# wildltr/ptranking

Hardware: AMD Instinct MI355X
Metric: queries/sec fwd+bwd LambdaRank, MSLR-WEB30K-shaped list_len=128 (higher is better)
Workload: dtype f32

## Files before the change

### include/ptranking_amd.h

```cpp
#ifndef PTRANKING_AMD_H
#define PTRANKING_AMD_H

#include <stddef.h>
#include <stdint.h>

#ifdef __cplusplus
extern "C" {
#endif

#define PTR_ABI_VERSION 8
#define PTR_MAX_LIST_LEN 4096
#define PTR_MAX_CUTOFFS 32
#define PTR_MAX_SUBTOPICS 32
#define PTR_MLP_ACT_LD 112

#define PTR_ERR_INVALID_ARG 1001
#define PTR_ERR_UNSUPPORTED 1002

#define PTR_LAMBDALOSS_NDCG_LOSS1 0
#define PTR_LAMBDALOSS_NDCG_LOSS2 1
#define PTR_LAMBDALOSS_NDCG_LOSS2PP 2

int ptr_abi_version(void);
const char *ptr_last_error(void);

int ptr_ranknet_fwd_bwd(const float *preds, const float *labels, const int32_t *lens, int B, int L, float sigma,
                        float *loss_out, float *loss_q, float *grad, void *stream);

int ptr_lambdarank_fwd_bwd(const float *preds, const float *labels, const int32_t *lens, int B, int L, float sigma,
                           float *loss_out, float *loss_q, float *grad, void *stream);

int ptr_lambdaloss_fwd_bwd(const float *preds, const float *labels, const int32_t *lens, int B, int L, int k,
                           float sigma, float mu, int loss_type, int presort, float *loss_out, float *loss_q,
                           float *grad, void *stream);

int ptr_softrank_fwd_bwd(const float *preds, const float *labels, const int32_t *lens, int B, int L, float delta, int top_k,
                         float *loss_out, float *loss_q, float *grad, void *stream);

int ptr_approxndcg_fwd_bwd(const float *preds, const float *labels, const int32_t *lens, int B, int L, float alpha,
                           int presort, int couple_batch, float grad_scale_override, float *loss_out, float *dcg_q,
                           float *inv_idcg_q, float *scale_out, float *grad, void *stream);

int ptr_listnet_fwd_bwd(const float *preds, const float *labels, const int32_t *lens, int B, int L, float *loss_out,
                        float *loss_q, float *grad, void *stream);

int ptr_stlistnet_fwd_bwd(const float *preds, const float *labels, const float *unif, const int32_t *lens, int B, int L,
                          float temperature, float *loss_out, float *loss_q, float *grad, void *stream);
int ptr_rankmse_fwd_bwd(const float *preds, const float *labels, const int32_t *lens, int B, int L, float *loss_out,
                        float *loss_q, float *grad, void *stream);
int ptr_rankcosine_fwd_bwd(const float *preds, const float *labels, const int32_t *lens, int B, int L, float *loss_out,
                           float *loss_q, float *grad, void *stream);

int ptr_listmle_fwd_bwd(const float *preds, const int64_t *perm, const int32_t *lens, int B, int L, float *loss_out,
                        float *loss_q, float *grad, void *stream);

int ptr_mdprank_fwd_bwd(const float *preds, const float *labels, const int64_t *perm, const int32_t *lens, int B, int L, int top_k,
                        float gamma, float *loss_out, float *loss_q, float *grad, void *stream);

#define PTR_WASS_COST_P1 0
#define PTR_WASS_COST_P2 1
#define PTR_WASS_COST_EG 2
#define PTR_WASS_COST_DG 3
#define PTR_WASS_COST_DDG 4

int ptr_wassrank_fwd_bwd(const float *preds, const float *labels, const int32_t *lens, int B, int L, int cost_type,
                         float gain_base, float non_rele_gap, float var_penalty, float lam, int sh_itr,
                         int scale_by_max_label, float *loss_out, float *loss_q, float *grad, void *stream);

#define PTR_ADCG_TOPK_SUBTOPICS 0
#define PTR_ADCG_TOPK_DOCUMENTS 1
int ptr_alphadcg_fwd_bwd(const float *preds, const float *rele, const int32_t *lens, const int32_t *ntopics, int B, int T, int L, float rt,
                         float alpha, int top_k, int top_k_axis, float *loss_out, float *loss_q, float *grad, void *stream);
int ptr_div_metrics_at_ks(const float *preds, const float *rele, const int32_t *lens, const int32_t *ntopics, int B, int T, int L,
                          const int32_t *ks, int nk, float alpha, float max_label, float *andcg, float *err_ia, float *nerr_ia,
                          int32_t *valid, void *stream);

#define PTR_DIVPROB_ANDCG 0
#define PTR_DIVPROB_ERRIA 1
#define PTR_DIVPROB_PAIRCLS 2
#define PTR_DIVPROB_LAMBDAPAIRCLS 3
int ptr_divprob_fwd_bwd(const float *mus, const float *vars, const float *rele, const int32_t *lens, const int32_t *ntopics, int B, int T, int L,
                        int objective, float beta, int top_k, int top_k_axis, float max_label, int norm, float *loss_out, float *loss_q,
                        float *grad_mu, float *grad_var, void *stream);
int ptr_divprob_expected_ranks(const float *mus, const float *vars, const int32_t *lens, int B, int L, float *ranks, void *stream);

#define PTR_NDEVAL_DEPTH 20
int ptr_ndeval_measures(const float *preds, const float *rele, const int32_t *lens, const int32_t *ntopics, int B, int T, int L,
                        const int32_t *ks, int nk, double alpha, double beta, int depth_m, double *per_k, double *per_q,
                        int32_t *actual_subtopics, int32_t *ideal_order, void *stream);

#define PTR_TREE_PAIRS_ALL 0
#define PTR_TREE_PAIRS_NOTIES 1
#define PTR_TREE_PAIRS_NO00 2
#define PTR_TREE_PAIRS_00 3
#define PTR_TREE_W_NONE 0
#define PTR_TREE_W_DELTA_NDCG 1
#define PTR_TREE_W_DELTA_GAIN 2
#define PTR_TREE_HESS_REFERENCE 0
#define PTR_TREE_HESS_SUM 1
#define PTR_TREE_HESS_CONSTANT 2
#define PTR_TREE_GAIN_POWER 0
#define PTR_TREE_GAIN_LABEL 1
int ptr_tree_pair_grad_hess(const float *preds, const float *labels, const int64_t *offsets, int B, const int32_t *queries, int nq, int max_len,
                            int pair_type, int weighting, float epsilon, int hessian, float *grad, float *hess, void *stream);
int ptr_tree_listnet_grad_hess(const float *preds, const float *labels, const int64_t *offsets, int B, const int32_t *queries, int nq, int max_len,
                               int gain_type, int hessian, float *grad, float *hess, void *stream);

#define PTR_SMOOTH_P 0
#define PTR_SMOOTH_AP 1
#define PTR_SMOOTH_NERR 2
#define PTR_SMOOTH_NDCG 3
int ptr_smoothmetric_fwd_bwd(const float *preds, const float *labels, const int32_t *lens, int B, int L, int metric, int opt_ideal, int top_k,
                             float alpha, float max_label, float *loss_out, float *loss_q, float *valid_q, float *ranks, float *max_label_ws,
                             float *grad, void *stream);

int ptr_gaussmetric_fwd_bwd(const float *mus, const float *vars, const float *labels, const int32_t *lens, int B, int L, int metric,
                            int opt_ideal, int top_k, float const_std, float max_label, float *loss_out, float *loss_q, float *valid_q,
                            float *ranks, int32_t *pos, float *max_label_ws, float *grad_mu, float *grad_var, void *stream);

#define PTR_PL_DIST_PL 0
#define PTR_PL_DIST_STPL 1
int ptr_pl_uniforms(int B, int L, int S, uint64_t seed, int64_t q0, float *unif, void *stream);
int ptr_pl_sample(const float *preds, const int32_t *lens, int B, int L, int S, float temperature, int distribution, uint64_t seed, int64_t q0,
                  const float *unif, int64_t *perm, float *action, void *stream);
int ptr_mdprank_sample_fwd_bwd(const float *preds, const float *labels, const int32_t *lens, int B, int L, int S, int top_k, float gamma,
                               float temperature, int distribution, uint64_t seed, int64_t q0, const float *unif, float *loss_out,
                               float *loss_q, float *grad, int64_t *perm_out, void *stream);

#define PTR_IRGAN_MAX_SAMPLES 64
#define PTR_IRGAN_MAX_DRAWS_PER_POS 64
#define PTR_IRGAN_POINT_D 0
#define PTR_IRGAN_PAIR_D 1
#define PTR_IRGAN_PAIR_G 2
#define PTR_IRGAN_SEL_POINT_D 0
#define PTR_IRGAN_SEL_PAIR_D_SVM 1
#define PTR_IRGAN_SEL_PAIR_D_LOG 2
#define PTR_IRGAN_SEL_PAIR_G_SVM 3
#define PTR_IRGAN_SEL_PAIR_G_LOG 4
int ptr_irgan_sample(const float *preds, const int32_t *lens, const int32_t *num_pos, int B, int L, int S, int mode, float temperature,
                     uint64_t seed, int64_t q0, const float *unif, int64_t *pos_idx, int64_t *neg_idx, int32_t *nsel, void *stream);
int ptr_irgan_point_gen_fwd_bwd(const float *g_preds, const float *d_preds, const int32_t *lens, const int32_t *num_pos, int B, int L,
                                float temperature, float lambda, int draws_per_pos, uint64_t seed, int64_t q0, const float *unif,
                                float *loss_out, float *loss_q, float *valid_q, float *grad, int32_t *counts, void *stream);
int ptr_irgan_sel_fwd_bwd(const float *x, const float *d_sel, const int64_t *neg_idx, const int32_t *nsel, const int32_t *lens, int B, int L,
                          int S, int mode, float temperature, float *loss_out, float *loss_q, float *valid_q, float *grad, void *stream);

#define PTR_IRFGAN_POINT_D 0
#define PTR_IRFGAN_PAIR_D 1
#define PTR_IRFGAN_POINT_G 2
#define PTR_IRFGAN_PAIR_G 3
#define PTR_FDIV_TVAR 0
#define PTR_FDIV_KL 1
#define PTR_FDIV_RKL 2
#define PTR_FDIV_PC 3
#define PTR_FDIV_NC 4
#define PTR_FDIV_SH 5
#define PTR_FDIV_JS 6
#define PTR_FDIV_GAN 7
int ptr_irfgan_point_sample(const float *preds, const int32_t *lens, const int32_t *num_pos, int B, int L, int S, uint64_t seed, int64_t q0,
                            const float *unif, int64_t *pos_idx, int64_t *neg_idx, int32_t *nsel, void *stream);
int ptr_irfgan_pair_sample(const float *preds, const float *labels, const int32_t *lens, const int32_t *num_pos, int B, int L, int S,
                           uint64_t seed, int64_t q0, const float *unif_draw, const float *unif_bern, int64_t *true_head, int64_t *true_tail,
                           int64_t *fake_head, int64_t *fake_tail, int32_t *nsel, int32_t *bern_count, void *stream);
int ptr_irfgan_fwd_bwd(const float *x, const float *d_fake, const int64_t *idx_a, const int64_t *idx_b, const int32_t *nsel, const int32_t *lens,
                       int B, int L, int S, int mode, int f_div, float *loss_out, float *loss_q, float *valid_q, float *grad, void *stream);

int ptr_shuffle_ties_order(const float *labels, const int32_t *lens, int B, int L, uint64_t seed, int64_t *perm,
                           void *stream);

int ptr_sort_desc(const float *preds, const int32_t *lens, int B, int L, float *vals, int64_t *idx, void *stream);

#define PTR_LABEL_MULTILABEL 0
#define PTR_LABEL_PERMUTATION 1
int ptr_metrics_at_ks(const float *preds, const float *labels, const int32_t *lens, int B, int L, const int32_t *ks,
                      int nk, int presort, int label_type, float max_label, float *max_label_ws, float *ndcg, float *nerr,
                      float *ap, float *prec, void *stream);

int ptr_sum_f32(const float *x, int n, float scale, float *out, void *stream);

size_t ptr_mlp_num_params(int F, int NL);
size_t ptr_mlp_backward_ws_floats(int F, int NL);
size_t ptr_mlp_backward_dz_floats(int R, int F, int NL);
size_t ptr_mlp_acts_floats(int R, int NL);
int ptr_mlp_forward(const float *X, const float *params, int R, int F, int NL, int train, float p_drop, uint64_t seed,
                    float *preds, float *acts, void *stream);
int ptr_mlp_backward(const float *X, const float *params, const float *acts, const float *dpreds, int R, int F, int NL,
                     float p_drop, uint64_t seed, float *dz, float *ws, float *grad, void *stream);
#define PTR_OPT_ADAM 1
#define PTR_OPT_ADAGRAD 2
#define PTR_OPT_RMSPROP 3
int ptr_mlp_backward_step(const float *X, float *params, const float *acts, const float *dpreds, int R, int F, int NL, float p_drop,
                          uint64_t seed, float *dz, float *ws, float *grad, int opt_kind, float lr, float hyper1, float hyper2, float eps,
                          float weight_decay, int step, float *state1, float *state2, const float *loss_q, int nq, float *loss_out,
                          void *stream);
int ptr_opt_step_loss(float *params, const float *grad, int64_t n, int opt_kind, float lr, float hyper1, float hyper2, float eps,
                      float weight_decay, int step, float *state1, float *state2, const float *loss_q, int nq, float *loss_out, void *stream);
int ptr_adam_step(float *param, const float *grad, float *exp_avg, float *exp_avg_sq, int64_t n, float lr, float beta1,
                  float beta2, float eps, float weight_decay, int step, void *stream);
int ptr_adagrad_step(float *param, const float *grad, float *state_sum, int64_t n, float lr, float lr_decay, float eps,
                     float weight_decay, int step, void *stream);
int ptr_rmsprop_step(float *param, const float *grad, float *square_avg, int64_t n, float lr, float alpha, float eps,
                     float weight_decay, void *stream);
size_t ptr_mlp_x6_ws_bytes(int F, int NL);
int ptr_mlp_forward_x6(const float *X, const float *params, int R, int F, int NL, int train, float p_drop, uint64_t seed,
                       float *preds, float *acts, void *wimg, void *stream);
#define PTR_LOSS_RANKNET 1
#define PTR_LOSS_LAMBDARANK 2
#define PTR_LOSS_LAMBDALOSS 3
#define PTR_LOSS_LISTNET 4
typedef struct ptr_train_step_desc {
    int32_t struct_bytes;
    int32_t loss_kind;
    int32_t B, L, F, NL;
    int32_t opt_kind, step;
    int32_t loss_i[4];
    float loss_f[4];
    float p_drop, lr, hyper1, hyper2, eps, weight_decay;
    uint64_t seed;
    const float *X, *labels;
    const int32_t *lens;
    float *params, *grad, *state1, *state2;
    float *preds, *acts, *loss_q, *dpreds, *dz, *ws;
    void *wimg;
    float *loss_out;
    void *events[4];
    int32_t wimg_current;
    int32_t reserved;
} ptr_train_step_desc;
int ptr_train_step(const ptr_train_step_desc *d, void *stream);
int ptr_mlp_dropout_mask(int R, int n_feat, int site, float p_drop, uint64_t seed, float *out, void *stream);

#define PTR_LINEAR_NONE 0
#define PTR_LINEAR_RELU 1
#define PTR_LINEAR_RELU_DROPOUT 2
#define PTR_LINEAR_GATE 3
int ptr_linear_forward(const float *X, int ldx, const float *W, const float *bias, int R, int K, int N, int act, float p_drop,
                       uint64_t seed, int site, float *Y, int ldy, void *stream);
int ptr_linear_backward_input(const float *dY, int ldy, const float *W, int R, int K, int N, const float *gate, int ldg, float p_drop,
                              float *dX, int ldx, void *stream);
size_t ptr_linear_backward_weight_ws_floats(int R, int K, int N);
int ptr_linear_backward_weight(const float *X, int ldx, const float *dY, int ldy, int R, int K, int N, float *ws, float *dW, float *db,
                               void *stream);
int ptr_dropout_apply(const float *x, int ldx, int R, int C, float p_drop, uint64_t seed, int site, float *out, int ldo, void *stream);
int ptr_relu_gate(const float *dy, const float *y, int64_t n, float *out, void *stream);

#define PTR_AF_NONE 0
#define PTR_AF_RELU 1
#define PTR_AF_LEAKY 2
#define PTR_AF_ELU 3
#define PTR_AF_SELU 4
#define PTR_AF_GELU 5
#define PTR_AF_SIGMOID 6
#define PTR_AF_TANH 7
size_t ptr_bn_ws_floats(int R, int N, int group_rows);
int ptr_bn_stats(const float *z, int ld, int R, int N, int group_rows, const int32_t *lens, int rows_per_query, float eps, float *ws,
                 float *mean, float *rstd, void *stream);
int ptr_bnact_forward(const float *z, int ld, int R, int N, int group_rows, const int32_t *lens, int rows_per_query, const float *mean,
                      const float *rstd, const float *gamma, const float *beta, int af, float p_drop, uint64_t seed, int site, float *out,
                      void *stream);
int ptr_bnact_backward(const float *z, const float *da, int ld, int R, int N, int group_rows, const int32_t *lens, int rows_per_query,
                       const float *mean, const float *rstd, const float *gamma, const float *beta, int af, float p_drop, uint64_t seed,
                       int site, float *ws, float *dz, float *dgamma, float *dbeta, void *stream);

size_t ptr_bn_slot_floats(int N);
int ptr_bn_stats_partial(const float *z, int ld, int R, int N, int group_rows, const int32_t *lens, int rows_per_query, float *ws,
                         float *slot, void *stream);
int ptr_bn_stats_combine(const float *slots, int W, int slot_stride, int N, float eps, float *mean, float *rstd, float *total_count,
                         void *stream);
int ptr_bnact_backward_sums(const float *z, const float *da, int ld, int R, int N, int group_rows, const int32_t *lens, int rows_per_query,
                            const float *mean, const float *rstd, const float *gamma, const float *beta, int af, float p_drop,
                            uint64_t seed, int site, float *ws, float *sums, void *stream);
int ptr_bnact_backward_apply(const float *z, const float *da, int ld, int R, int N, int group_rows, const int32_t *lens, int rows_per_query,
                             const float *mean, const float *rstd, const float *gamma, const float *beta, int af, float p_drop,
                             uint64_t seed, int site, const float *sums, int W, const float *total_count, float *ws, float *dz,
                             void *stream);

#define PTR_MHSA_MAX_HEAD_DIM 352
int ptr_mhsa_forward(const float *Q, const float *K, const float *V, int ld_qkv, const int32_t *lens, int B, int L, int F,
                     int n_heads, float p_drop, uint64_t seed, int site, float *O, float *lse, void *stream);
int ptr_mhsa_backward(const float *Q, const float *K, const float *V, int ld_qkv, const float *O, const float *dO, const float *lse,
                      const int32_t *lens, int B, int L, int F, int n_heads, float p_drop, uint64_t seed, int site, float *dvec,
                      float *dQ, float *dK, float *dV, float *ds_ws, void *stream);
int ptr_mhsa_dropout_mask(int B, int L, int n_heads, float p_drop, uint64_t seed, int site, float *out, void *stream);
int ptr_layernorm_forward(const float *X, const float *a2, const float *b2, int64_t R, int F, float eps, float *Y, float *stats,
                          void *stream);
size_t ptr_layernorm_backward_ws_floats(int F);
int ptr_layernorm_backward(const float *X, const float *a2, const float *dY, const float *stats, int64_t R, int F, float *ws,
                           float *dX, float *da2, float *db2, void *stream);

int ptr_launch_form(const char *entry, const int64_t *args, int nargs, int32_t *form, int nform);

#define PTR_GBDT_MAX_BIN 256
int ptr_gbdt_bin(const float *X, int64_t n, int F, const float *edges, const int32_t *nbins, int max_bin, int stride, uint8_t *bins,
                 void *stream);
int ptr_gbdt_quantize(const float *g, const float *h, int64_t n, int32_t *qg, int32_t *qh, int32_t *expo, int32_t *flag, uint32_t *state,
                      void *stream);
int ptr_gbdt_histogram(const uint8_t *bins, int stride, int64_t n, const int32_t *qg, const int32_t *qh, const int32_t *rows, int64_t m,
                       int F, int max_bin, int64_t *hist, void *stream);
int ptr_gbdt_hist_sub(const int64_t *parent, const int64_t *child, int F, int max_bin, int64_t *out, void *stream);
int ptr_gbdt_best_split(const int64_t *hist, int nleaf, int F, int max_bin, const int32_t *nbins, const int32_t *expo, double lambda_l2,
                        int64_t min_data_in_leaf, double min_sum_hessian_in_leaf, double min_gain_to_split, int64_t *ws, int64_t *rec,
                        void *stream);
size_t ptr_gbdt_partition_ws_ints(int64_t m);
int ptr_gbdt_partition(const uint8_t *bins, int stride, int64_t n, int F, const int32_t *rows, int64_t m, int feature, int bin,
                       int32_t *out, int32_t *left_count, int32_t *ws, void *stream);
int ptr_gbdt_add_leaf_values(float *scores, int64_t n, const int32_t *rows, const int32_t *offsets, const float *values, int nleaves,
                             int64_t total, void *stream);
int ptr_gbdt_predict(const float *X, int64_t n, int F, const int32_t *feature, const float *threshold, const int32_t *left,
                     const int32_t *right, const float *value, const int32_t *tree_offsets, int ntrees, float *out, void *stream);

int ptr_gbdt_histogram_segments(const uint8_t *bins, int stride, int64_t n, const int32_t *qg, const int32_t *qh, const int32_t *rows,
                                int64_t nrows, const int32_t *segs, int K, const int32_t *items, int n_direct, int n_lds, int F, int max_bin,
                                int64_t *pool, int nslots, void *stream);
int ptr_gbdt_hist_sub_segments(int64_t *pool, int nslots, int F, int max_bin, const int32_t *trips, int K, void *stream);
int ptr_gbdt_best_split_slots(const int64_t *pool, int nslots, const int32_t *slots, int K, int F, int max_bin, const int32_t *nbins,
                              const int32_t *expo, double lambda_l2, int64_t min_data_in_leaf, double min_sum_hessian_in_leaf,
                              double min_gain_to_split, int64_t *ws, int64_t *rec, void *stream);
size_t ptr_gbdt_partition_segments_ws_ints(int64_t nblocks);
int ptr_gbdt_partition_segments(const uint8_t *bins, int stride, int64_t n, int F, const int32_t *rows, int64_t nrows, const int32_t *segs, int K,
                                const int32_t *blocks, int nblocks, int32_t *out, int32_t *left_counts, int32_t *ws, int64_t ws_ints,
                                void *stream);

int ptr_letor_scan(const char *path, int one_indexed, int64_t *n_docs, int32_t *n_features, int64_t *n_queries);
int ptr_letor_load(const char *path, int one_indexed, float missing, int64_t n_docs, int32_t n_features, int64_t n_queries,
                   void *X, int x_is_f64, float *y, int64_t *qids, int64_t *qoff);

#ifdef __cplusplus
}
#endif
#endif
```

### ptranking_amd/_lib.py

```python
import ctypes as C
import os

import torch

_PKG = os.path.dirname(os.path.abspath(__file__))
LIB_PATH = os.environ.get("PTR_LIB") or os.path.join(_PKG, "libptranking_amd.so")

ABI_VERSION = 8
MAX_LIST_LEN = 4096
MAX_CUTOFFS = 32
MAX_SUBTOPICS = 32

_vp, _i, _f, _u64 = C.c_void_p, C.c_int, C.c_float, C.c_uint64

SIGNATURES = {
    "ptr_abi_version": [],
    "ptr_last_error": [],
    "ptr_ranknet_fwd_bwd": [_vp, _vp, _vp, _i, _i, _f, _vp, _vp, _vp, _vp],
    "ptr_lambdarank_fwd_bwd": [_vp, _vp, _vp, _i, _i, _f, _vp, _vp, _vp, _vp],
    "ptr_lambdaloss_fwd_bwd": [_vp, _vp, _vp, _i, _i, _i, _f, _f, _i, _i, _vp, _vp, _vp, _vp],
    "ptr_approxndcg_fwd_bwd": [_vp, _vp, _vp, _i, _i, _f, _i, _i, _f, _vp, _vp, _vp, _vp, _vp, _vp],
    "ptr_softrank_fwd_bwd": [_vp, _vp, _vp, _i, _i, _f, _i, _vp, _vp, _vp, _vp],
    "ptr_listnet_fwd_bwd": [_vp, _vp, _vp, _i, _i, _vp, _vp, _vp, _vp],
    "ptr_mdprank_fwd_bwd": [_vp, _vp, _vp, _vp, _i, _i, _i, _f, _vp, _vp, _vp, _vp],
    "ptr_listmle_fwd_bwd": [_vp, _vp, _vp, _i, _i, _vp, _vp, _vp, _vp],
    "ptr_stlistnet_fwd_bwd": [_vp, _vp, _vp, _vp, _i, _i, _f, _vp, _vp, _vp, _vp],
    "ptr_rankmse_fwd_bwd": [_vp, _vp, _vp, _i, _i, _vp, _vp, _vp, _vp],
    "ptr_rankcosine_fwd_bwd": [_vp, _vp, _vp, _i, _i, _vp, _vp, _vp, _vp],
    "ptr_wassrank_fwd_bwd": [_vp, _vp, _vp, _i, _i, _i, _f, _f, _f, _f, _i, _i, _vp, _vp, _vp, _vp],
    "ptr_alphadcg_fwd_bwd": [_vp, _vp, _vp, _vp, _i, _i, _i, _f, _f, _i, _i, _vp, _vp, _vp, _vp],
    "ptr_div_metrics_at_ks": [_vp, _vp, _vp, _vp, _i, _i, _i, C.POINTER(C.c_int32), _i, _f, _f, _vp, _vp, _vp, _vp, _vp],
    "ptr_divprob_fwd_bwd": [_vp, _vp, _vp, _vp, _vp, _i, _i, _i, _i, _f, _i, _i, _f, _i, _vp, _vp, _vp, _vp, _vp],
    "ptr_divprob_expected_ranks": [_vp, _vp, _vp, _i, _i, _vp, _vp],
    "ptr_ndeval_measures": [_vp, _vp, _vp, _vp, _i, _i, _i, C.POINTER(C.c_int32), _i, C.c_double, C.c_double, _i, _vp, _vp, _vp, _vp, _vp],
    "ptr_tree_pair_grad_hess": [_vp, _vp, _vp, _i, _vp, _i, _i, _i, _i, _f, _i, _vp, _vp, _vp],
    "ptr_tree_listnet_grad_hess": [_vp, _vp, _vp, _i, _vp, _i, _i, _i, _i, _vp, _vp, _vp],
    "ptr_smoothmetric_fwd_bwd": [_vp, _vp, _vp, _i, _i, _i, _i, _i, _f, _f, _vp, _vp, _vp, _vp, _vp, _vp, _vp],
    "ptr_gaussmetric_fwd_bwd": [_vp, _vp, _vp, _vp, _i, _i, _i, _i, _i, _f, _f, _vp, _vp, _vp, _vp, _vp, _vp, _vp, _vp, _vp],
    "ptr_pl_uniforms": [_i, _i, _i, _u64, C.c_int64, _vp, _vp],
    "ptr_pl_sample": [_vp, _vp, _i, _i, _i, _f, _i, _u64, C.c_int64, _vp, _vp, _vp, _vp],
    "ptr_mdprank_sample_fwd_bwd": [_vp, _vp, _vp, _i, _i, _i, _i, _f, _f, _i, _u64, C.c_int64, _vp, _vp, _vp, _vp, _vp, _vp],
    "ptr_irgan_sample": [_vp, _vp, _vp, _i, _i, _i, _i, _f, _u64, C.c_int64, _vp, _vp, _vp, _vp, _vp],
    "ptr_irgan_point_gen_fwd_bwd": [_vp, _vp, _vp, _vp, _i, _i, _f, _f, _i, _u64, C.c_int64, _vp, _vp, _vp, _vp, _vp, _vp, _vp],
    "ptr_irgan_sel_fwd_bwd": [_vp, _vp, _vp, _vp, _vp, _i, _i, _i, _i, _f, _vp, _vp, _vp, _vp, _vp],
    "ptr_irfgan_point_sample": [_vp, _vp, _vp, _i, _i, _i, _u64, C.c_int64, _vp, _vp, _vp, _vp, _vp],
    "ptr_irfgan_pair_sample": [_vp, _vp, _vp, _vp, _i, _i, _i, _u64, C.c_int64, _vp, _vp, _vp, _vp, _vp, _vp, _vp, _vp, _vp],
    "ptr_irfgan_fwd_bwd": [_vp, _vp, _vp, _vp, _vp, _vp, _i, _i, _i, _i, _i, _vp, _vp, _vp, _vp, _vp],
    "ptr_shuffle_ties_order": [_vp, _vp, _i, _i, _u64, _vp, _vp],
    "ptr_sort_desc": [_vp, _vp, _i, _i, _vp, _vp, _vp],
    "ptr_metrics_at_ks": [_vp, _vp, _vp, _i, _i, C.POINTER(C.c_int32), _i, _i, _i, _f, _vp, _vp, _vp, _vp, _vp, _vp],
    "ptr_sum_f32": [_vp, _i, _f, _vp, _vp],
    "ptr_mlp_num_params": [_i, _i],
    "ptr_mlp_backward_ws_floats": [_i, _i],
    "ptr_mlp_backward_dz_floats": [_i, _i, _i],
    "ptr_mlp_acts_floats": [_i, _i],
    "ptr_mlp_forward": [_vp, _vp, _i, _i, _i, _i, _f, _u64, _vp, _vp, _vp],
    "ptr_mlp_backward": [_vp, _vp, _vp, _vp, _i, _i, _i, _f, _u64, _vp, _vp, _vp, _vp],
    "ptr_mlp_backward_step": [_vp, _vp, _vp, _vp, _i, _i, _i, _f, _u64, _vp, _vp, _vp, _i, _f, _f, _f, _f, _f, _i, _vp, _vp, _vp, _i, _vp, _vp],
    "ptr_opt_step_loss": [_vp, _vp, C.c_int64, _i, _f, _f, _f, _f, _f, _i, _vp, _vp, _vp, _i, _vp, _vp],
    "ptr_train_step": [_vp, _vp],
    "ptr_mlp_x6_ws_bytes": [_i, _i],
    "ptr_mlp_forward_x6": [_vp, _vp, _i, _i, _i, _i, _f, _u64, _vp, _vp, _vp, _vp],
    "ptr_adam_step": [_vp, _vp, _vp, _vp, C.c_int64, _f, _f, _f, _f, _f, _i, _vp],
    "ptr_adagrad_step": [_vp, _vp, _vp, C.c_int64, _f, _f, _f, _f, _i, _vp],
    "ptr_rmsprop_step": [_vp, _vp, _vp, C.c_int64, _f, _f, _f, _f, _vp],
    "ptr_mlp_dropout_mask": [_i, _i, _i, _f, _u64, _vp, _vp],
    "ptr_linear_forward": [_vp, _i, _vp, _vp, _i, _i, _i, _i, _f, _u64, _i, _vp, _i, _vp],
    "ptr_linear_backward_input": [_vp, _i, _vp, _i, _i, _i, _vp, _i, _f, _vp, _i, _vp],
    "ptr_linear_backward_weight_ws_floats": [_i, _i, _i],
    "ptr_linear_backward_weight": [_vp, _i, _vp, _i, _i, _i, _i, _vp, _vp, _vp, _vp],
    "ptr_bn_ws_floats": [_i, _i, _i],
    "ptr_bn_stats": [_vp, _i, _i, _i, _i, _vp, _i, _f, _vp, _vp, _vp, _vp],
    "ptr_bnact_forward": [_vp, _i, _i, _i, _i, _vp, _i, _vp, _vp, _vp, _vp, _i, _f, _u64, _i, _vp, _vp],
    "ptr_bnact_backward": [_vp, _vp, _i, _i, _i, _i, _vp, _i, _vp, _vp, _vp, _vp, _i, _f, _u64, _i, _vp, _vp, _vp, _vp, _vp],
    "ptr_bn_slot_floats": [_i],
    "ptr_bn_stats_partial": [_vp, _i, _i, _i, _i, _vp, _i, _vp, _vp, _vp],
    "ptr_bn_stats_combine": [_vp, _i, _i, _i, _f, _vp, _vp, _vp, _vp],
    "ptr_bnact_backward_sums": [_vp, _vp, _i, _i, _i, _i, _vp, _i, _vp, _vp, _vp, _vp, _i, _f, _u64, _i, _vp, _vp, _vp],
    "ptr_bnact_backward_apply": [_vp, _vp, _i, _i, _i, _i, _vp, _i, _vp, _vp, _vp, _vp, _i, _f, _u64, _i, _vp, _i, _vp, _vp, _vp, _vp],
    "ptr_dropout_apply": [_vp, _i, _i, _i, _f, _u64, _i, _vp, _i, _vp],
    "ptr_relu_gate": [_vp, _vp, C.c_int64, _vp, _vp],
    "ptr_mhsa_forward": [_vp, _vp, _vp, _i, _vp, _i, _i, _i, _i, _f, _u64, _i, _vp, _vp, _vp],
    "ptr_mhsa_backward": [_vp, _vp, _vp, _i, _vp, _vp, _vp, _vp, _i, _i, _i, _i, _f, _u64, _i, _vp, _vp, _vp, _vp, _vp, _vp],
    "ptr_mhsa_dropout_mask": [_i, _i, _i, _f, _u64, _i, _vp, _vp],
    "ptr_layernorm_forward": [_vp, _vp, _vp, C.c_int64, _i, _f, _vp, _vp, _vp],
    "ptr_layernorm_backward_ws_floats": [_i],
    "ptr_layernorm_backward": [_vp, _vp, _vp, _vp, C.c_int64, _i, _vp, _vp, _vp, _vp, _vp],
    "ptr_launch_form": [C.c_char_p, C.POINTER(C.c_int64), _i, C.POINTER(C.c_int32), _i],
    "ptr_gbdt_bin": [_vp, C.c_int64, _i, _vp, _vp, _i, _i, _vp, _vp],
    "ptr_gbdt_quantize": [_vp, _vp, C.c_int64, _vp, _vp, _vp, _vp, _vp, _vp],
    "ptr_gbdt_histogram": [_vp, _i, C.c_int64, _vp, _vp, _vp, C.c_int64, _i, _i, _vp, _vp],
    "ptr_gbdt_hist_sub": [_vp, _vp, _i, _i, _vp, _vp],
    "ptr_gbdt_best_split": [_vp, _i, _i, _i, _vp, _vp, C.c_double, C.c_int64, C.c_double, C.c_double, _vp, _vp, _vp],
    "ptr_gbdt_partition_ws_ints": [C.c_int64],
    "ptr_gbdt_partition": [_vp, _i, C.c_int64, _i, _vp, C.c_int64, _i, _i, _vp, _vp, _vp, _vp],
    "ptr_gbdt_add_leaf_values": [_vp, C.c_int64, _vp, _vp, _vp, _i, C.c_int64, _vp],
    "ptr_gbdt_predict": [_vp, C.c_int64, _i, _vp, _vp, _vp, _vp, _vp, _vp, _i, _vp, _vp],
    "ptr_gbdt_histogram_segments": [_vp, _i, C.c_int64, _vp, _vp, _vp, C.c_int64, _vp, _i, _vp, _i, _i, _i, _i, _vp, _i, _vp],
    "ptr_gbdt_hist_sub_segments": [_vp, _i, _i, _i, _vp, _i, _vp],
    "ptr_gbdt_best_split_slots": [_vp, _i, _vp, _i, _i, _i, _vp, _vp, C.c_double, C.c_int64, C.c_double, C.c_double, _vp, _vp, _vp],
    "ptr_gbdt_partition_segments_ws_ints": [C.c_int64],
    "ptr_gbdt_partition_segments": [_vp, _i, C.c_int64, _i, _vp, C.c_int64, _vp, _i, _vp, _i, _vp, _vp, _vp, C.c_int64, _vp],
    "ptr_letor_scan":[C.c_char_p, _i, _vp, _vp, _vp],
    "ptr_letor_load": [C.c_char_p, _i, _f, C.c_int64, C.c_int32, C.c_int64, _vp, _i, _vp, _vp, _vp],
}
_RESTYPES = {"ptr_last_error": C.c_char_p, "ptr_mlp_num_params": C.c_size_t, "ptr_mlp_backward_ws_floats": C.c_size_t,
             "ptr_mlp_backward_dz_floats": C.c_size_t, "ptr_mlp_acts_floats": C.c_size_t, "ptr_mlp_x6_ws_bytes": C.c_size_t, "ptr_linear_backward_weight_ws_floats": C.c_size_t, "ptr_bn_ws_floats": C.c_size_t,
             "ptr_bn_slot_floats": C.c_size_t, "ptr_gbdt_partition_ws_ints": C.c_size_t,
             "ptr_gbdt_partition_segments_ws_ints": C.c_size_t,
             "ptr_layernorm_backward_ws_floats": C.c_size_t}
OPTIONAL = set()

_lib = None


class Loss:

    def __init__(self, entry, kind, params=()):
        self.entry, self.kind, self.params = entry, kind, tuple(params)

    def c_args(self, **values):
        return [C.c_float(float(values[n])) if t is _f else int(values[n]) for n, t in self.params]

    def desc_arrays(self, **values):
        return (tuple(int(values[n]) for n, t in self.params if t is _i), tuple(C.c_float(float(values[n])).value for n, t in self.params if t is _f))


LOSSES = {
    "ranknet": Loss("ptr_ranknet_fwd_bwd", 1, [("sigma", _f)]),
    "lambdarank": Loss("ptr_lambdarank_fwd_bwd", 2, [("sigma", _f)]),
    "lambdaloss": Loss("ptr_lambdaloss_fwd_bwd", 3, [("k", _i), ("sigma", _f), ("mu", _f), ("loss_type", _i), ("presort", _i)]),
    "listnet": Loss("ptr_listnet_fwd_bwd", 4),
}


class TrainStepDesc(C.Structure):
    _fields_ = [("struct_bytes", C.c_int32), ("loss_kind", C.c_int32),
                ("B", C.c_int32), ("L", C.c_int32), ("F", C.c_int32), ("NL", C.c_int32),
                ("opt_kind", C.c_int32), ("step", C.c_int32),
                ("loss_i", C.c_int32 * 4), ("loss_f", C.c_float * 4),
                ("p_drop", C.c_float), ("lr", C.c_float), ("hyper1", C.c_float), ("hyper2", C.c_float), ("eps", C.c_float), ("weight_decay", C.c_float),
                ("seed", C.c_uint64),
                ("X", C.c_void_p), ("labels", C.c_void_p), ("lens", C.c_void_p),
                ("params", C.c_void_p), ("grad", C.c_void_p), ("state1", C.c_void_p), ("state2", C.c_void_p),
                ("preds", C.c_void_p), ("acts", C.c_void_p), ("loss_q", C.c_void_p), ("dpreds", C.c_void_p), ("dz", C.c_void_p), ("ws", C.c_void_p),
                ("wimg", C.c_void_p), ("loss_out", C.c_void_p), ("events", C.c_void_p * 4), ("wimg_current", C.c_int32), ("reserved", C.c_int32)]


class NativeLibraryError(RuntimeError):
    pass


def load():
    global _lib
    if _lib is not None:
        return _lib
    if not os.path.exists(LIB_PATH):
        raise NativeLibraryError(
            f"{LIB_PATH} is missing: build the HIP extension first (python -m ptranking_amd.build, or "
            f"__graft_entry__.build()).  ptranking_amd has no CPU / eager fallback by design.")
    lib = C.CDLL(LIB_PATH, mode=C.RTLD_GLOBAL)
    for name, argtypes in SIGNATURES.items():
        try:
            fn = getattr(lib, name)
        except AttributeError:
            if name in OPTIONAL:
                continue
            raise NativeLibraryError(f"{LIB_PATH} does not export {name}; rebuild it")
        fn.argtypes = argtypes
        fn.restype = _RESTYPES.get(name, C.c_int)
    v = lib.ptr_abi_version()
    if v != ABI_VERSION:
        raise NativeLibraryError(f"ABI version mismatch: library {v}, binding {ABI_VERSION}")
    _lib = lib
    return lib


def has(name):
    return hasattr(load(), name)


TIMING = None


def query(name, *args):
    return getattr(load(), name)(*args)


def call(name, *args):
    lib = load()
    if TIMING is not None:
        ev0, ev1 = torch.cuda.Event(enable_timing=True), torch.cuda.Event(enable_timing=True)
        ev0.record()
        rc = getattr(lib, name)(*args)
        ev1.record()
        TIMING.setdefault(name, []).append((ev0, ev1))
    else:
        rc = getattr(lib, name)(*args)
    if rc != 0:
        msg = lib.ptr_last_error()
        raise RuntimeError(f"{name} failed (code {rc}): {msg.decode() if msg else ''}")


def ptr(t):
    return None if t is None else C.c_void_p(t.data_ptr())


def current_stream(device):
    return C.c_void_p(torch.cuda.current_stream(device).cuda_stream)
```

### ptranking_amd/csrc/optim.hip

```cpp
#include "ptr_mlp.h"
#include "ptr_optim.h"

namespace ptr {

constexpr int kRedElems = 128;
inline unsigned reduce_grid(size_t n, bool loss_block) { return (unsigned)((n + kRedElems - 1) / kRedElems) + (loss_block ? 1u : 0u); }
__global__ void __launch_bounds__(1024)
reduce_partials_kernel(const float *__restrict__ ws, int nblk, int nblk_tail, size_t tail_begin, size_t stride, size_t n,
                       float *__restrict__ grad, OptStep o) {
    __shared__ float part[16][kRedElems];
    const int lane = threadIdx.x & 63, w = threadIdx.x >> 6;
    if (o.loss_out && blockIdx.x == gridDim.x - 1) {
        const float tot = block1024_sum(o.loss_q, o.nq, &part[0][0]);
        if (threadIdx.x == 0) o.loss_out[0] = tot;
        return;
    }
    const size_t ia = (size_t)blockIdx.x * kRedElems + lane, ib = ia + 64;
    const size_t ica = ia < n ? ia : n - 1, icb = ib < n ? ib : n - 1;
    const int nba = ica >= tail_begin ? nblk_tail : nblk, nbb = icb >= tail_begin ? nblk_tail : nblk;
    const int nbc = nba < nbb ? nba : nbb;
    float a0 = 0.f, a1 = 0.f, a2 = 0.f, a3 = 0.f, b0 = 0.f, b1 = 0.f, b2 = 0.f, b3 = 0.f;
    int b = w;
    for (; b + 48 < nbc; b += 64) {
        a0 += ws[(size_t)b * stride + ica];
        a1 += ws[(size_t)(b + 16) * stride + ica];
        a2 += ws[(size_t)(b + 32) * stride + ica];
        a3 += ws[(size_t)(b + 48) * stride + ica];
        b0 += ws[(size_t)b * stride + icb];
        b1 += ws[(size_t)(b + 16) * stride + icb];
        b2 += ws[(size_t)(b + 32) * stride + icb];
        b3 += ws[(size_t)(b + 48) * stride + icb];
    }
    int ba = b, bb = b;
    for (; ba + 48 < nba; ba += 64) {
        a0 += ws[(size_t)ba * stride + ica];
        a1 += ws[(size_t)(ba + 16) * stride + ica];
        a2 += ws[(size_t)(ba + 32) * stride + ica];
        a3 += ws[(size_t)(ba + 48) * stride + ica];
    }
    for (; bb + 48 < nbb; bb += 64) {
        b0 += ws[(size_t)bb * stride + icb];
        b1 += ws[(size_t)(bb + 16) * stride + icb];
        b2 += ws[(size_t)(bb + 32) * stride + icb];
        b3 += ws[(size_t)(bb + 48) * stride + icb];
    }
    for (; ba < nba; ba += 16) a0 += ws[(size_t)ba * stride + ica];
    for (; bb < nbb; bb += 16) b0 += ws[(size_t)bb * stride + icb];
    part[w][lane] = (a0 + a1) + (a2 + a3);
    part[w][64 + lane] = (b0 + b1) + (b2 + b3);
    __syncthreads();
    const int col = 64 * w + lane;
    const size_t i = (size_t)blockIdx.x * kRedElems + col;
    if (w < 2 && i < n) {
        float s = part[0][col];
#pragma unroll
        for (int k = 1; k < 16; ++k) s += part[k][col];
        if (grad) grad[i] = s;
        if (o.kind) {
            const float pn = opt_update(o, i, s);
            if (o.wimg) x6_img_put(o.wimg, o.F, o.NL, i, pn);
        }
    }
}

int launch_reduce_partials(const float *ws, int nblk, int nblk_tail, size_t tail_begin, size_t stride, size_t n, float *grad, const OptStep &o,
                           hipStream_t st, const char *who) {
    hipLaunchKernelGGL(reduce_partials_kernel, dim3(reduce_grid(n, o.loss_out != nullptr)), dim3(1024), 0, st, ws, nblk, nblk_tail, tail_begin,
                       stride, n, grad, o);
    return check_hip(hipGetLastError(), who);
}

__global__ void __launch_bounds__(256)
opt_step_kernel(const float *__restrict__ grad, size_t n, OptStep o) {
    const size_t i = (size_t)blockIdx.x * 256 + threadIdx.x;
    if (i < n) opt_update(o, i, grad[i]);
}

static int opt_step_alone(const char *who, int opt_kind, float *param, const float *grad, float *state1, float *state2, int64_t n, float lr, float hyper1,
                          float hyper2, float eps, float weight_decay, int step, void *stream) {
    if (n < 0 || (n > 0 && (!param || !grad))) { set_error("%s: bad arguments", who); return PTR_ERR_INVALID_ARG; }
    OptStep o;
    if (int rc = make_opt_step(o, who, opt_kind, lr, hyper1, hyper2, eps, weight_decay, step, param, state1, state2, n > 0, nullptr, 0, nullptr)) return rc;
    if (n == 0) return 0;
    hipLaunchKernelGGL(opt_step_kernel, dim3((unsigned)((n + 255) / 256)), dim3(256), 0, as_stream(stream), grad, (size_t)n, o);
    return check_hip(hipGetLastError(), who);
}

}

extern "C" int ptr_adam_step(float *param, const float *grad, float *exp_avg, float *exp_avg_sq, int64_t n, float lr, float beta1,
                             float beta2, float eps, float weight_decay, int step, void *stream) {
    return ptr::opt_step_alone("ptr_adam_step", PTR_OPT_ADAM, param, grad, exp_avg, exp_avg_sq, n, lr, beta1, beta2, eps, weight_decay, step, stream);
}

extern "C" int ptr_adagrad_step(float *param, const float *grad, float *state_sum, int64_t n, float lr, float lr_decay, float eps,
                                float weight_decay, int step, void *stream) {
    return ptr::opt_step_alone("ptr_adagrad_step", PTR_OPT_ADAGRAD, param, grad, state_sum, nullptr, n, lr, lr_decay, 0.0f, eps, weight_decay, step, stream);
}

extern "C" int ptr_rmsprop_step(float *param, const float *grad, float *square_avg, int64_t n, float lr, float alpha, float eps,
                                float weight_decay, void *stream) {
    return ptr::opt_step_alone("ptr_rmsprop_step", PTR_OPT_RMSPROP, param, grad, square_avg, nullptr, n, lr, alpha, 0.0f, eps, weight_decay, 1, stream);
}

extern "C" int ptr_opt_step_loss(float *params, const float *grad, int64_t n, int opt_kind, float lr, float hyper1, float hyper2, float eps,
                                 float weight_decay, int step, float *state1, float *state2, const float *loss_q, int nq, float *loss_out,
                                 void *stream) {
    using namespace ptr;
    const char *who = "ptr_opt_step_loss";
    OptStep o;
    if (int rc = make_opt_step(o, who, opt_kind, lr, hyper1, hyper2, eps, weight_decay, step, params, state1, state2, n > 0, loss_q, nq, loss_out)) return rc;
    if (n < 0 || (n > 0 && (!params || !grad))) { set_error("%s: bad optimiser / loss arguments", who); return PTR_ERR_INVALID_ARG; }
    if (n == 0 && !loss_out) return 0;
    const size_t nn = (size_t)n;
    return launch_reduce_partials(grad, 1, 1, nn, nn, nn, nullptr, o, as_stream(stream), who);
}
```

### ptranking_amd/csrc/ptr_mlp.h

```cpp
#pragma once
#include <stdlib.h>
#include <utility>

#include "ptr_device.h"
#include "ptr_dropout.h"
#include "ptr_x6.h"

namespace ptr {

constexpr int kH = 100;
constexpr int kHP = 112;
constexpr int kMT = 7;
constexpr int kMaxLayers = 8;
constexpr int kAL = 112;
constexpr int kActTile = 16 * kAL;
__host__ __device__ inline int act_row_tiles(int R) { return (R + 15) >> 4; }
__host__ __device__ inline size_t act_layer_floats(int R) { return (size_t)act_row_tiles(R) * kActTile; }
__host__ __device__ inline size_t act_off(int row, int col) {
    return (size_t)(row >> 4) * kActTile + (size_t)(((col >> 4) << 8) + ((row & 15) << 4) + (col & 15));
}

__host__ __device__ inline size_t off_W(int l, int F) { return l == 0 ? 0 : (size_t)kH * F + kH + (size_t)(l - 1) * (kH * kH + kH); }
__host__ __device__ inline size_t off_b(int l, int F) { return off_W(l, F) + (l == 0 ? (size_t)kH * F : (size_t)kH * kH); }
__host__ __device__ inline size_t off_wout(int NL, int F) { return off_W(NL, F); }
__host__ __device__ inline size_t n_params(int NL, int F) { return off_wout(NL, F) + kH + 1; }

struct MlpArgs {
    int R, F, NL;
    float p_drop;
    uint32_t seed_lo, seed_hi;
};

constexpr int kX6Rows = kHP;
constexpr int kX6PlaneBytes = kX6Rows * 32 * 2;
constexpr int kX6SliceBytes = 3 * kX6PlaneBytes;
__host__ __device__ inline int x6_n1(int F) { return (F + 31) / 32; }
__host__ __device__ inline int x6_nslices(int F, int NL) { return x6_n1(F) + 4 * (NL - 1); }
#if defined(__HIPCC__)
__device__ __forceinline__ void x6_img_put(uint8_t *__restrict__ img, int F, int NL, size_t i, float x) {
    const size_t w1 = (size_t)kH * F;
    int sl, row, g, e;
    if (i < w1) {
        row = (int)(i / F);
        const int k = (int)(i - (size_t)row * F), kk = k & 31;
        sl = k >> 5; g = kk >> 3; e = kk & 7;
    } else {
        if (i < w1 + kH) return;
        const size_t jv = i - (w1 + kH);
        const int l = 1 + (int)(jv / (kH * kH + kH));
        if (l > NL - 1) return;
        const int jj = (int)(jv - (size_t)(l - 1) * (kH * kH + kH));
        int k;
        if (jj < kH * kH) { row = jj / kH; k = jj - row * kH; } else { row = jj - kH * kH; k = kH; }
        const int kk = k & 31;
        sl = x6_n1(F) + 4 * (l - 1) + (k >> 5);
        g = (kk & 15) >> 2; e = 4 * (kk >> 4) + (kk & 3);
    }
    uint16_t p1, p2, p3;
    split_pack1(x, p1, p2, p3);
    uint8_t *at = img + (size_t)sl * kX6SliceBytes + (size_t)(row >> 4) * 1024 + g * 256 + (row & 15) * 16 + e * 2;
    *reinterpret_cast<uint16_t *>(at) = p1;
    *reinterpret_cast<uint16_t *>(at + kX6PlaneBytes) = p2;
    *reinterpret_cast<uint16_t *>(at + 2 * kX6PlaneBytes) = p3;
}
#endif

template <int N, class Fn> __device__ __forceinline__ void static_for(Fn &&f) {
    [&]<int... I>(std::integer_sequence<int, I...>) { (f(std::integral_constant<int, I>{}), ...); }(std::make_integer_sequence<int, N>{});
}

bool bwd_fused_supported(int F, int NL, const void *X, const void *acts);
int bwd_fused_grid(int R);
int launch_bwd_fused(const float *X, const float *params, const float *acts, const float *dpreds, const MlpArgs &a, float *ws,
                     hipStream_t st, const char *who);

bool bwd_tail_supported(int NL, const void *acts);
int launch_bwd_tail(const float *params, const float *acts, const float *dpreds, const MlpArgs &a, float *ws, float *dz0, hipStream_t st,
                    const char *who);

bool bwd_x6_supported(int R, int F, int NL, const void *X, const void *acts);
int launch_bwd_x6(const float *X, const float *params, const float *acts, const float *dpreds, const MlpArgs &a, float *ws, hipStream_t st,
                  const char *who);

bool bwd_x6_tail_supported(int R, int NL, const void *acts);
int launch_bwd_x6_tail(const float *params, const float *acts, const float *dpreds, const MlpArgs &a, float *ws, float *dz0, hipStream_t st,
                       const char *who);

bool dw_x6_supported(int R, int K, int lda, const void *A);
int launch_dw_x6(const float *A, int lda, const float *dZ, int K, int ntk, const MlpArgs &a, float *ws, size_t np_stride, size_t w_off, size_t b_off,
                 int nblk, hipStream_t st, const char *who);

int mlp_forward_x6_impl(const float *X, const float *params, int R, int F, int NL, int train, float p_drop, uint64_t seed, float *preds, float *acts,
                        void *wimg, bool prep, void *stream);
int mlp_backward_step_impl(const float *X, float *params, const float *acts, const float *dpreds, int R, int F, int NL, float p_drop, uint64_t seed, float *dz,
                           float *ws, float *grad, int opt_kind, float lr, float hyper1, float hyper2, float eps, float weight_decay, int step, float *state1,
                           float *state2, const float *loss_q, int nq, float *loss_out, void *wimg, void *stream);

}
```

### ptranking_amd/csrc/ptr_optim.h

```cpp
#pragma once
#include <math.h>

#include "ptr_device.h"

namespace ptr {

struct OptStep {
    int kind;
    float lr, h1, h2, eps, wd, bc1, bc2_sqrt;
    float *param, *s1, *s2;
    const float *loss_q; int nq; float *loss_out;
    uint8_t *wimg; int F, NL;
};

inline int make_opt_step(OptStep &o, const char *who, int opt_kind, float lr, float hyper1, float hyper2, float eps, float weight_decay, int step,
                         float *params, float *state1, float *state2, bool need_state, const float *loss_q, int nq, float *loss_out) {
    if (opt_kind < PTR_OPT_ADAM || opt_kind > PTR_OPT_RMSPROP) { set_error("%s: unknown optimiser %d", who, opt_kind); return PTR_ERR_INVALID_ARG; }
    if (step < 1 || nq < 0 || (need_state && (!state1 || (opt_kind == PTR_OPT_ADAM && !state2))) || (loss_out && nq > 0 && !loss_q)) {
        set_error("%s: bad optimiser / loss arguments", who);
        return PTR_ERR_INVALID_ARG;
    }
    o = OptStep{};
    o.kind = opt_kind; o.lr = lr; o.h1 = hyper1; o.h2 = hyper2; o.eps = eps; o.wd = weight_decay;
    o.param = params; o.s1 = state1; o.s2 = state2; o.loss_q = loss_q; o.nq = nq; o.loss_out = loss_out;
    if (opt_kind == PTR_OPT_ADAM) { o.bc1 = 1.0f - powf(hyper1, (float)step); o.bc2_sqrt = sqrtf(1.0f - powf(hyper2, (float)step)); }
    else if (opt_kind == PTR_OPT_ADAGRAD) o.lr = lr / (1.0f + (float)(step - 1) * hyper1);
    return 0;
}

int launch_reduce_partials(const float *ws, int nblk, int nblk_tail, size_t tail_begin, size_t stride, size_t n, float *grad, const OptStep &o,
                           hipStream_t st, const char *who);

#if defined(__HIPCC__)
__device__ __forceinline__ float opt_update(const OptStep &o, size_t i, float g) {
    const float pi = o.param[i];
    const float gi = g + o.wd * pi;
    float upd;
    if (o.kind == PTR_OPT_ADAM) {
        const float mi = o.h1 * o.s1[i] + (1.0f - o.h1) * gi;
        const float vi = o.h2 * o.s2[i] + (1.0f - o.h2) * gi * gi;
        o.s1[i] = mi; o.s2[i] = vi;
        const float denom = sqrtf(vi) / o.bc2_sqrt + o.eps;
        upd = (o.lr / o.bc1) * (mi / denom);
    } else {
        const float si = o.kind == PTR_OPT_ADAGRAD ? o.s1[i] + gi * gi : o.h1 * o.s1[i] + (1.0f - o.h1) * gi * gi;
        o.s1[i] = si;
        upd = o.lr * (gi / (sqrtf(si) + o.eps));
    }
    const float pn = pi - upd;
    o.param[i] = pn;
    return pn;
}
#endif

}
```

### ptranking_amd/csrc/scorer.hip

```cpp
#include "ptr_mlp.h"
#include "ptr_optim.h"

namespace ptr {

__host__ __device__ inline int ld_w1(int F) { return (F + 3) / 4 * 4 + 4; }


constexpr int kTailNone = 0, kTailSpread = 1, kTailReplicate = 2;
__device__ __forceinline__ void stage_matrix(float *dst, int ld, const float *src, int rows, int cols, bool transpose, int tid, int nthr,
                                             int tail = kTailNone) {
    constexpr int U = 8;
    const int n = rows * cols;
    const bool vec = ((cols & 3) == 0) && ((reinterpret_cast<uintptr_t>(src) & 15) == 0);
    const int reps = tail == kTailReplicate ? 4 : 1;
    if (vec) {
        const int n4 = n >> 2;
        for (int base = tid; base < n4; base += U * nthr) {
            f32x4 v[U];
#pragma unroll
            for (int u = 0; u < U; ++u) {
                const int i4 = base + u * nthr;
                v[u] = *reinterpret_cast<const f32x4 *>(src + 4 * (size_t)(i4 < n4 ? i4 : n4 - 1));
            }
#pragma unroll
            for (int u = 0; u < U; ++u) {
                const int i4 = base + u * nthr;
                if (i4 < n4) {
                    const int idx = 4 * i4, r = idx / cols, c = idx - r * cols;
                    if (!transpose) {
                        for (int rep = 0; rep < (r >= 96 ? reps : 1); ++rep) *reinterpret_cast<f32x4 *>(dst + (size_t)(r + 4 * rep) * ld + c) = v[u];
                    } else {
#pragma unroll
                        for (int e = 0; e < 4; ++e) dst[(size_t)(c + e) * ld + r] = v[u][e];
                    }
                }
            }
        }
    } else {
        for (int base = tid; base < n; base += U * nthr) {
            float v[U];
#pragma unroll
            for (int u = 0; u < U; ++u) { const int idx = base + u * nthr; v[u] = src[idx < n ? idx : n - 1]; }
#pragma unroll
            for (int u = 0; u < U; ++u) {
                const int idx = base + u * nthr;
                if (idx < n) {
                    const int r = idx / cols, c = idx - r * cols;
                    if (transpose) dst[(size_t)c * ld + r] = v[u];
                    else for (int rep = 0; rep < (r >= 96 ? reps : 1); ++rep) dst[(size_t)(r + 4 * rep) * ld + c] = v[u];
                }
            }
        }
    }
    const int vr = transpose ? cols : rows, vc = transpose ? rows : cols;
    for (int idx = tid; idx < kHP * ld; idx += nthr) {
        const int r = idx / ld, c = idx - r * ld;
        const bool real_row = (tail == kTailReplicate && r >= 96) ? 96 + ((r - 96) & 3) < vr : r < vr;
        if (!real_row || c >= vc) dst[idx] = 0.0f;
    }
}
__device__ __forceinline__ void stage_vector(float *dst, const float *src, int n, int tid, int nthr, int tail = kTailNone) {
    for (int i = tid; i < kHP; i += nthr) {
        if (tail != kTailSpread || i < 96) dst[i] = i < n ? src[i] : 0.0f;
        else dst[i] = (((i - 96) & 3) == 0 && 96 + ((i - 96) >> 2) < n) ? src[96 + ((i - 96) >> 2)] : 0.0f;
    }
}

constexpr int kSlabK = 48, kSlabLd = kSlabK + 4;
__host__ __device__ inline size_t fwd_lds_floats(int F, int NL, int w1_mode) {
    const size_t w1 = w1_mode == 0 ? (size_t)kHP * ld_w1(F) : (w1_mode == 2 ? (size_t)2 * kHP * kSlabLd : 0);
    return w1 + (size_t)(NL - 1) * kHP * kH + (size_t)NL * kHP + kHP + 16;
}
__host__ __device__ inline int fwd_w1_mode(int F, int NL) {
    if (fwd_lds_floats(F, NL, 0) * sizeof(float) <= 160 * 1024) return 0;
    return fwd_lds_floats(F, NL, 2) * sizeof(float) <= 160 * 1024 ? 2 : 1;
}

#ifdef PTR_FWD_TRACE
#define FWD_STAMP(i) do { if (blockIdx.x == 0 && lane == 0 && ntile_done < 8) { unsigned long long *tr_ = reinterpret_cast<unsigned long long *>(preds + ((R + 3) & ~3) + 4) + (ntile_done * 16 + wave) * 8; tr_[(i)] = clock64(); if ((i) == 0) tr_[4] = wall_clock64(); if ((i) == 3) tr_[5] = wall_clock64(); } } while (0)
#else
#define FWD_STAMP(i) do { } while (0)
#endif

template <int RT, int NTHR, bool TRAIN, bool VEC, int W1G>
__global__ void __launch_bounds__(NTHR)
mlp_fwd_kernel(const float *__restrict__ X, const float *__restrict__ P, MlpArgs a, float *__restrict__ preds,
               float *__restrict__ acts) {
    extern __shared__ __attribute__((aligned(16))) float smem[];
    const int F = a.F, NL = a.NL, R = a.R, ld1 = ld_w1(F), R16 = act_row_tiles(a.R) * 16;
    float *W1s = smem;
    float *Wh = W1s + (W1G == 0 ? (size_t)kHP * ld1 : (W1G == 2 ? (size_t)2 * kHP * kSlabLd : 0));
    float *Bs = Wh + (size_t)(NL - 1) * kHP * kH;
    float *Wo = Bs + (size_t)NL * kHP;
    const int tid = threadIdx.x, nthr = blockDim.x;
    if constexpr (W1G == 0) stage_matrix(W1s, ld1, P + off_W(0, F), kH, F, false, tid, nthr, kTailReplicate);
    for (int l = 1; l < NL; ++l) stage_matrix(Wh + (size_t)(l - 1) * kHP * kH, kH, P + off_W(l, F), kH, kH, false, tid, nthr, kTailReplicate);
    for (int l = 0; l < NL; ++l) stage_vector(Bs + (size_t)l * kHP, P + off_b(l, F), kH, tid, nthr);
    stage_vector(Wo, P + off_wout(NL, F), kH, tid, nthr, kTailSpread);
    if (tid < 16) Wo[kHP + tid] = tid == 0 ? P[off_wout(NL, F) + kH] : 0.0f;
    __syncthreads();
    const float b_out = Wo[kHP];

    const int lane = tid & 63, j = lane & 15, g = lane >> 4;
    const int wpb = nthr >> 6, wave = tid >> 6;
    const int rows_per_tile = 16 * RT;
    const int ntiles = (R + rows_per_tile - 1) / rows_per_tile;
    const uint32_t thr = drop_thr(a.p_drop);
    const float scale = TRAIN ? 1.0f / (1.0f - a.p_drop) : 1.0f;
    const int nS1 = (F + 15) >> 4;

    int ntile_done = 0;
    (void)ntile_done;
    auto prefetch_first = [&](int t, f32x4 (&xb)[RT]) {
        const int tt = t < ntiles ? t : ntiles - 1;
        const int k0 = 4 * g;
#pragma unroll
        for (int rt = 0; rt < RT; ++rt) {
            const int r = tt * rows_per_tile + 16 * rt + j;
            const float *xr = X + (size_t)(r < R ? r : R - 1) * F;
            if constexpr (VEC) {
                xb[rt] = *reinterpret_cast<const f32x4 *>(xr + (k0 < F ? k0 : 0));
            } else {
#pragma unroll
                for (int c = 0; c < 4; ++c) xb[rt][c] = xr[k0 + c < F ? k0 + c : 0];
            }
        }
    };
    f32x4 xpre[RT];
    constexpr bool kQueue = W1G != 2;
    const int tiles_per_block = (ntiles + gridDim.x - 1) / gridDim.x;
    const int tile_lo = kQueue ? blockIdx.x * tiles_per_block : 0, tile_hi = kQueue ? min(ntiles, tile_lo + tiles_per_block) : ntiles;
    int *queue = reinterpret_cast<int *>(Wo + kHP + 8);
    int tile = blockIdx.x * wpb + wave;
    if constexpr (kQueue) {
        if (tid == 0) *queue = tile_lo + wpb;
        __syncthreads();
        tile = tile_lo + wave;
    }
    constexpr int kSlabV = kHP * (kSlabK / 4);
    constexpr int kSlabU = (kSlabV + NTHR - 1) / NTHR;
    f32x4 slab_r[W1G == 2 ? kSlabU : 1];
    int slab_buf = 0;
    auto slab_load = [&](int sl) {
        if constexpr (W1G == 2) {
#pragma unroll
            for (int u = 0; u < kSlabU; ++u) {
                const int i4 = tid + u * NTHR, r = i4 / (kSlabK / 4), c = 4 * (i4 - r * (kSlabK / 4));
                const int wr = r < 96 ? r : 96 + ((r - 96) & 3), k = kSlabK * sl + c;
                slab_r[u] = *reinterpret_cast<const f32x4 *>(P + (size_t)(wr < kHP ? wr : 0) * F + (k < F ? k : 0));
            }
        }
    };
    auto slab_store = [&](int sl, int buf) {
        if constexpr (W1G == 2) {
#pragma unroll
            for (int u = 0; u < kSlabU; ++u) {
                const int i4 = tid + u * NTHR, r = i4 / (kSlabK / 4), c = 4 * (i4 - r * (kSlabK / 4));
                const bool real = kSlabK * sl + c < F;
                f32x4 v = slab_r[u];
                if (!real) v = f32x4{0.f, 0.f, 0.f, 0.f};
                if (i4 < kSlabV) *reinterpret_cast<f32x4 *>(W1s + (size_t)buf * kHP * kSlabLd + (size_t)r * kSlabLd + c) = v;
            }
        }
    };
    if constexpr (W1G == 2) { slab_load(0); slab_store(0, 0); }
    prefetch_first(tile, xpre);
    for (; (kQueue ? tile : tile - wave) < tile_hi; ++ntile_done) {
        int next_tile = tile_hi;
        auto advance = [&]() {
            if constexpr (kQueue) {
                int nxt = 0;
                if (lane == 0) nxt = atomicAdd(queue, 1);
                next_tile = __builtin_amdgcn_readfirstlane(nxt);
            } else {
                next_tile = tile + gridDim.x * wpb;
            }
            prefetch_first(next_tile, xpre);
        };
        const int row0 = tile * rows_per_tile;
        const bool tile_full = row0 + rows_per_tile <= R;
        int row[RT];
#pragma unroll
        for (int rt = 0; rt < RT; ++rt) row[rt] = row0 + 16 * rt + j;
        FWD_STAMP(0);

        const float *xrow[RT];
        bool rok[RT];
#pragma unroll
        for (int rt = 0; rt < RT; ++rt) {
            rok[rt] = row[rt] < R;
            xrow[rt] = X + (size_t)(rok[rt] ? row[rt] : R - 1) * F;
        }
        auto load_raw = [&](int S, f32x4 (&xb)[RT]) {
            const int k0 = 16 * S + 4 * g;
#pragma unroll
            for (int rt = 0; rt < RT; ++rt) {
                if constexpr (VEC) {
                    xb[rt] = *reinterpret_cast<const f32x4 *>(xrow[rt] + (k0 < F ? k0 : 0));
                } else {
#pragma unroll
                    for (int c = 0; c < 4; ++c) xb[rt][c] = xrow[rt][k0 + c < F ? k0 + c : 0];
                }
            }
        };
        auto finish_x = [&](int S, f32x4 (&xb)[RT]) {
            const int k0 = 16 * S + 4 * g;
#pragma unroll
            for (int rt = 0; rt < RT; ++rt) {
                f32x4 v = xb[rt];
                if (16 * S + 16 > F || !tile_full) {
#pragma unroll
                    for (int c = 0; c < 4; ++c) v[c] *= ((k0 + c < F) && rok[rt]) ? 1.0f : 0.0f;
                }
                if constexpr (TRAIN) {
                    uint32_t w0, w1;
                    drop_bits(a.seed_lo, a.seed_hi, 0, row[rt], k0 >> 2, w0, w1);
                    v = drop4(v, w0, w1, thr, scale);
                }
                xb[rt] = v;
            }
        };

        auto tail_store = [&](float v, float ones) -> f32x4 {
            const float h1 = __shfl(v, j + 16, 64), h2 = __shfl(v, j + 32, 64), h3 = __shfl(v, j + 48, 64);
            f32x4 o = f32x4{g == 1 ? ones : 0.0f, 0.0f, 0.0f, 0.0f};
            if (g == 0) o = f32x4{v, h1, h2, h3};
            return o;
        };
        auto mma = [&](auto mt_, float aop, float bop, f32x4 c) -> f32x4 {
            if constexpr (decltype(mt_)::value == kMT - 1) return __builtin_amdgcn_mfma_f32_4x4x1f32(aop, bop, c, 0, 0, 0);
            else return __builtin_amdgcn_mfma_f32_16x16x4f32(aop, bop, c, 0, 0, 0);
        };
        f32x4 acc[kMT][RT];
        auto tile6_finish = [&]() {
#pragma unroll
            for (int rt = 0; rt < RT; ++rt) {
                f32x4 t = acc[kMT - 1][rt];
#pragma unroll
                for (int c = 0; c < 4; ++c) { t[c] += __shfl_xor(t[c], 16, 64); t[c] += __shfl_xor(t[c], 32, 64); }
                acc[kMT - 1][rt][0] = g == 0 ? t[0] : (g == 1 ? t[1] : (g == 2 ? t[2] : t[3]));
            }
        };
        auto mma_tiles = [&](const f32x4 (&wa)[kMT], const f32x4 (&b)[RT], int nc) {
            auto one = [&]<int MT>(std::integral_constant<int, MT> mt_, int c) {
#pragma unroll
                for (int rt = 0; rt < RT; ++rt) acc[MT][rt] = mma(mt_, wa[MT][c], b[rt][c], acc[MT][rt]);
            };
            using std::integral_constant;
#pragma unroll
            for (int c = 0; c < 4; ++c) if (c < nc) { one(integral_constant<int, 0>{}, c); one(integral_constant<int, 1>{}, c); }
#pragma unroll
            for (int c = 0; c < 4; ++c) if (c < nc) { one(integral_constant<int, 2>{}, c); one(integral_constant<int, 3>{}, c); }
#pragma unroll
            for (int c = 0; c < 4; ++c) if (c < nc) { one(integral_constant<int, 4>{}, c); one(integral_constant<int, 5>{}, c); one(integral_constant<int, 6>{}, c); }
        };
        auto bias_init = [&](const float *b) {
#pragma unroll
            for (int mt = 0; mt < kMT; ++mt) {
                f32x4 b4 = *reinterpret_cast<const f32x4 *>(b + (mt < kMT - 1 ? 16 * mt + 4 * g : 96));
                if (mt == kMT - 1) { const float on = g == 0 ? 1.0f : 0.0f; b4 = b4 * on; }
#pragma unroll
                for (int rt = 0; rt < RT; ++rt) acc[mt][rt] = b4;
            }
        };
        bias_init(Bs);
        f32x4 xa[RT], xb[RT], xc[RT];
#pragma unroll
        for (int rt = 0; rt < RT; ++rt) xa[rt] = xpre[rt];
        if (NL == 1) advance();
        finish_x(0, xa);
        auto read_w1 = [&](int S, int sin, int mt) -> f32x4 {
            const int k0 = 16 * S + 4 * g;
            if constexpr (W1G == 2) {
                return *reinterpret_cast<const f32x4 *>(W1s + (size_t)slab_buf * kHP * kSlabLd + (size_t)(16 * mt + j) * kSlabLd + 16 * sin + 4 * g);
            } else if constexpr (W1G == 1) {
                const int wr = mt < kMT - 1 ? 16 * mt + j : 96 + (j & 3);
                return *reinterpret_cast<const f32x4 *>(P + (size_t)wr * F + (k0 < F ? k0 : 0));
            } else {
                return *reinterpret_cast<const f32x4 *>(W1s + (size_t)(16 * mt + j) * ld1 + k0);
            }
        };
        auto l1_step = [&](int S, int sin, f32x4 (&cur)[RT], f32x4 (&nxt)[RT], f32x4 (&nn)[RT]) {
            load_raw(S + 2 < nS1 ? S + 2 : 0, nn);
            __builtin_amdgcn_sched_barrier(0);
            f32x4 wa[kMT];
#pragma unroll
            for (int mt = 0; mt < kMT; ++mt) wa[mt] = read_w1(S, sin, mt);
            if constexpr (RT > 1) __builtin_amdgcn_sched_barrier(0);
            mma_tiles(wa, cur, 4);
            finish_x(S + 1, nxt);
        };
        auto slab_enter = [&](int S) {
            if constexpr (W1G == 2) {
                __syncthreads();
                slab_load(S + 3 < nS1 ? S / 3 + 1 : 0);
            }
        };
        auto slab_leave = [&](int S) {
            if constexpr (W1G == 2) {
                slab_store(S + 3 < nS1 ? S / 3 + 1 : 0, slab_buf ^ 1);
                slab_buf ^= 1;
            }
        };
        load_raw(nS1 > 1 ? 1 : 0, xb);
        int S1 = 0;
        for (; S1 + 3 <= nS1; S1 += 3) {
            slab_enter(S1);
            l1_step(S1, 0, xa, xb, xc);
            l1_step(S1 + 1, 1, xb, xc, xa);
            l1_step(S1 + 2, 2, xc, xa, xb);
            slab_leave(S1);
        }
        const int left = nS1 - S1;
        if (left == 0) {
        } else if (left == 1) {
            slab_enter(S1);
            l1_step(S1, 0, xa, xb, xc);
            slab_leave(S1);
        } else {
            slab_enter(S1);
            l1_step(S1, 0, xa, xb, xc);
            l1_step(S1 + 1, 1, xb, xc, xa);
            slab_leave(S1);
        }
        tile6_finish();

        FWD_STAMP(1);
        for (int l = 1; l < NL; ++l) {
            f32x4 hin[kMT][RT];
#pragma unroll
            for (int mt = 0; mt < kMT; ++mt)
#pragma unroll
                for (int rt = 0; rt < RT; ++rt) {
                    f32x4 h = acc[mt][rt];
#pragma unroll
                    for (int c = 0; c < 4; ++c) h[c] = fmaxf(h[c], 0.0f);
                    if constexpr (TRAIN) {
                        if (mt < kMT - 1) {
                            uint32_t w0, w1;
                            drop_bits(a.seed_lo, a.seed_hi, l, row[rt], 4 * mt + g, w0, w1);
                            h = drop4(h, w0, w1, thr, scale);
                        } else {
                            h[0] *= drop_keep1(a.seed_lo, a.seed_hi, l, row[rt], 96 + g, thr) ? scale : 0.0f;
                        }
                    }
                    hin[mt][rt] = h;
                }
            if (l == NL - 1) advance();
            const float *Wl = Wh + (size_t)(l - 1) * kHP * kH;
            bias_init(Bs + (size_t)l * kHP);
#pragma unroll
            for (int S = 0; S < kMT; ++S) {
                constexpr int kLast = kMT - 1;
                f32x4 wa[kMT];
#pragma unroll
                for (int mt = 0; mt < kMT; ++mt) {
                    const float *wp = Wl + (size_t)(16 * mt + j) * kH;
                    if (S < kLast) wa[mt] = *reinterpret_cast<const f32x4 *>(wp + 16 * S + 4 * g);
                    else wa[mt] = f32x4{wp[96 + g], 0.0f, 0.0f, 0.0f};
                }
                if constexpr (RT > 1) __builtin_amdgcn_sched_barrier(0);
                if constexpr (TRAIN) {
#pragma unroll
                    for (int rt = 0; rt < RT; ++rt) {
                        if (row[rt] < R16) {
                            float *arow = acts + (size_t)(l - 1) * act_layer_floats(R) + act_off(row[rt], 0);
                            *reinterpret_cast<f32x4 *>(arow + 256 * S + 4 * g) = S < kLast ? hin[S][rt] : tail_store(hin[S][rt][0], 1.0f);
                        }
                    }
                    if constexpr (RT > 1) __builtin_amdgcn_sched_barrier(0);
                }
                mma_tiles(wa, hin[S], S < kLast ? 4 : 1);
            }
            tile6_finish();
        }

        FWD_STAMP(2);
        float sc[RT];
#pragma unroll
        for (int rt = 0; rt < RT; ++rt) sc[rt] = 0.0f;
#pragma unroll
        for (int mt = 0; mt < kMT; ++mt) {
            const f32x4 w4 = *reinterpret_cast<const f32x4 *>(Wo + 16 * mt + 4 * g);
#pragma unroll
            for (int rt = 0; rt < RT; ++rt) {
                f32x4 h = acc[mt][rt];
#pragma unroll
                for (int c = 0; c < (mt == kMT - 1 ? 1 : 4); ++c) { h[c] = fmaxf(h[c], 0.0f); sc[rt] = fmaf(h[c], w4[c], sc[rt]); }
                if constexpr (TRAIN) {
                    if (row[rt] < R16) {
                        float *arow = acts + (size_t)(NL - 1) * act_layer_floats(R) + act_off(row[rt], 0);
                        *reinterpret_cast<f32x4 *>(arow + 256 * mt + 4 * g) = mt < kMT - 1 ? h : tail_store(h[0], 0.0f);
                    }
                }
            }
        }
#pragma unroll
        for (int rt = 0; rt < RT; ++rt) {
            float s = sc[rt];
            s += __shfl_xor(s, 16, 64);
            s += __shfl_xor(s, 32, 64);
            if (g == 0 && row[rt] < R) preds[row[rt]] = s + b_out;
        }
        FWD_STAMP(3);
        tile = next_tile;
    }
}

__host__ __device__ inline size_t dz_lds_floats(int NL) { return (size_t)(NL - 1) * kHP * kH + (kHP + 16) + 16 * (kHP + 16); }

template <int RT, int NTHR>
__global__ void __launch_bounds__(NTHR)
mlp_bwd_dz_kernel(const float *__restrict__ P, const float *__restrict__ acts, const float *__restrict__ dpreds, MlpArgs a,
                  float *__restrict__ dz, float *__restrict__ ws, size_t np_stride, size_t wout_off) {
    extern __shared__ __attribute__((aligned(16))) float smem[];
    const int F = a.F, NL = a.NL, R = a.R;
    float *WT = smem;
    float *Wo = WT + (size_t)(NL - 1) * kHP * kH;
    float *wrow = Wo + kHP + 16;
    const int tid = threadIdx.x, nthr = blockDim.x;
    for (int l = 1; l < NL; ++l) stage_matrix(WT + (size_t)(l - 1) * kHP * kH, kH, P + off_W(l, F), kH, kH, true, tid, nthr);
    stage_vector(Wo, P + off_wout(NL, F), kH, tid, nthr);
    if (tid < 16) Wo[kHP + tid] = 0.0f;
    __syncthreads();

    const int lane = tid & 63, j = lane & 15, g = lane >> 4;
    const int wpb = nthr >> 6, wave = tid >> 6;
    const int rows_per_tile = 16 * RT;
    const int ntiles = (R + rows_per_tile - 1) / rows_per_tile;
    const float inv_keep = a.p_drop > 0.0f ? 1.0f / (1.0f - a.p_drop) : 1.0f;

    f32x4 dwo[kMT];
#pragma unroll
    for (int mt = 0; mt < kMT; ++mt) dwo[mt] = f32x4{0.f, 0.f, 0.f, 0.f};
    float dbo = 0.0f;

    f32x4 hpf[kMT][RT];
    float dspf[RT];
    auto prefetch_top = [&](int tile) {
#pragma unroll
        for (int rt = 0; rt < RT; ++rt) {
            const int r = tile * rows_per_tile + 16 * rt + j;
            const int rc = r < R ? r : R - 1;
            dspf[rt] = dpreds[rc];
#pragma unroll
            for (int mt = 0; mt < kMT; ++mt)
                hpf[mt][rt] = *reinterpret_cast<const f32x4 *>(acts + (size_t)(NL - 1) * act_layer_floats(R) + act_off(rc, 16 * mt + 4 * g));
        }
    };
    const int tile_first = blockIdx.x * wpb + wave, tile_step = gridDim.x * wpb;
    if (tile_first < ntiles) prefetch_top(tile_first);
    for (int tile = tile_first; tile < ntiles; tile += tile_step) {
        const int row0 = tile * rows_per_tile;
        int row[RT];
        float ds[RT];
        f32x4 htop[kMT][RT];
#pragma unroll
        for (int rt = 0; rt < RT; ++rt) {
            row[rt] = row0 + 16 * rt + j;
            ds[rt] = dspf[rt] * (row[rt] < R ? 1.0f : 0.0f);
            if (g == 0) dbo += ds[rt];
#pragma unroll
            for (int mt = 0; mt < kMT; ++mt) htop[mt][rt] = hpf[mt][rt];
        }
        if (tile + tile_step < ntiles) prefetch_top(tile + tile_step);
        f32x4 cur[kMT][RT];
#pragma unroll
        for (int mt = 0; mt < kMT; ++mt) {
            const f32x4 w4 = *reinterpret_cast<const f32x4 *>(Wo + 16 * mt + 4 * g);
#pragma unroll
            for (int rt = 0; rt < RT; ++rt) {
                const bool ok = row[rt] < R;
                const size_t o = ((size_t)(NL - 1) * R + row[rt]) * kAL + 16 * mt + 4 * g;
                f32x4 h = htop[mt][rt];
                const float okf = ok ? 1.0f : 0.0f;
#pragma unroll
                for (int c = 0; c < 4; ++c) h[c] *= okf;
                f32x4 d;
#pragma unroll
                for (int c = 0; c < 4; ++c) { d[c] = (ds[rt] * w4[c]) * (h[c] > 0.0f ? 1.0f : 0.0f); dwo[mt][c] = fmaf(h[c], ds[rt], dwo[mt][c]); }
                if (ok) *reinterpret_cast<f32x4 *>(dz + o) = d;
                cur[mt][rt] = d;
            }
        }
        for (int l = NL - 1; l >= 1; --l) {
            const float *Wl = WT + (size_t)(l - 1) * kHP * kH;
            f32x4 gate[kMT][RT];
#pragma unroll
            for (int mt = 0; mt < kMT; ++mt)
#pragma unroll
                for (int rt = 0; rt < RT; ++rt) {
                    const bool ok = row[rt] < R;
                    const size_t o = (size_t)(l - 1) * act_layer_floats(R) + act_off(row[rt], 16 * mt + 4 * g);
                    gate[mt][rt] = *reinterpret_cast<const f32x4 *>(acts + (ok ? o : 0));
                }
            f32x4 acc[kMT][RT];
#pragma unroll
            for (int mt = 0; mt < kMT; ++mt)
#pragma unroll
                for (int rt = 0; rt < RT; ++rt) acc[mt][rt] = f32x4{0.f, 0.f, 0.f, 0.f};
#pragma unroll
            for (int S = 0; S < kMT; ++S) {
                f32x4 wa[kMT];
#pragma unroll
                for (int mt = 0; mt < kMT; ++mt) wa[mt] = *reinterpret_cast<const f32x4 *>(Wl + (size_t)(16 * mt + j) * kH + 16 * S + 4 * g);
                auto group = [&](int m0, int m1) {
#pragma unroll
                    for (int c = 0; c < 4; ++c)
#pragma unroll
                        for (int mt = m0; mt < m1; ++mt)
#pragma unroll
                            for (int rt = 0; rt < RT; ++rt)
                                acc[mt][rt] = __builtin_amdgcn_mfma_f32_16x16x4f32(wa[mt][c], cur[S][rt][c], acc[mt][rt], 0, 0, 0);
                };
                group(0, 2); group(2, 4); group(4, kMT);
            }
#pragma unroll
            for (int mt = 0; mt < kMT; ++mt)
#pragma unroll
                for (int rt = 0; rt < RT; ++rt) {
                    const bool ok = row[rt] < R;
                    const size_t o = ((size_t)(l - 1) * R + row[rt]) * kAL + 16 * mt + 4 * g;
                    f32x4 d;
#pragma unroll
                    for (int c = 0; c < 4; ++c) d[c] = acc[mt][rt][c] * ((ok && gate[mt][rt][c] > 0.0f) ? inv_keep : 0.0f);
                    if (ok) *reinterpret_cast<f32x4 *>(dz + o) = d;
                    cur[mt][rt] = d;
                }
        }
    }
#pragma unroll
    for (int mt = 0; mt < kMT; ++mt)
#pragma unroll
        for (int c = 0; c < 4; ++c) {
            float v = dwo[mt][c];
            v += __shfl_xor(v, 1, 64); v += __shfl_xor(v, 2, 64); v += __shfl_xor(v, 4, 64); v += __shfl_xor(v, 8, 64);
            if (j == 0) wrow[(size_t)wave * (kHP + 16) + 16 * mt + 4 * g + c] = v;
        }
    {
        float v = dbo;
        v += __shfl_xor(v, 1, 64); v += __shfl_xor(v, 2, 64); v += __shfl_xor(v, 4, 64); v += __shfl_xor(v, 8, 64);
        if (lane == 0) wrow[(size_t)wave * (kHP + 16) + kHP] = v;
    }
    __syncthreads();
    for (int i = tid; i < kH + 1; i += nthr) {
        const int src = i < kH ? i : kHP;
        float s = 0.0f;
        for (int w = 0; w < wpb; ++w) s += wrow[(size_t)w * (kHP + 16) + src];
        ws[(size_t)blockIdx.x * np_stride + wout_off + i] = s;
    }
}

template <int NTW, bool SITE0, int NWV>
__global__ void __launch_bounds__(NWV * 64)
mlp_bwd_dw_kernel(const float *__restrict__ A, int lda, const float *__restrict__ dZ, int K, int nt_base, MlpArgs a,
                  float *__restrict__ ws, size_t np_stride, size_t w_off, size_t b_off) {
    const int R = a.R;
    const int tid = threadIdx.x, lane = tid & 63, j = lane & 15, g = lane >> 4, wave = tid >> 6;
    constexpr int U = 4;
    const int chunk = ((R + gridDim.x - 1) / gridDim.x + 4 * U - 1) / (4 * U) * (4 * U);
    const int r_begin = blockIdx.x * chunk, r_end = min(R, r_begin + chunk);
    const uint32_t thr = drop_thr(a.p_drop);
    const float scale = (SITE0 && a.p_drop > 0.0f) ? 1.0f / (1.0f - a.p_drop) : 1.0f;
    const int ntk = (K + 15) >> 4;
    (void)ntk;

    f32x4 acc[NTW][kMT];
#pragma unroll
    for (int t = 0; t < NTW; ++t)
#pragma unroll
        for (int mt = 0; mt < kMT; ++mt) acc[t][mt] = f32x4{0.f, 0.f, 0.f, 0.f};
    float dbv[kMT];
#pragma unroll
    for (int mt = 0; mt < kMT; ++mt) dbv[mt] = 0.0f;

    int fa[kMT], kb[NTW];
    bool fa_ok[kMT], kb_ok[NTW];
#pragma unroll
    for (int mt = 0; mt < kMT; ++mt) { const int f = 16 * mt + j; fa_ok[mt] = true; fa[mt] = f; }
#pragma unroll
    for (int t = 0; t < NTW; ++t) { const int k = 16 * (nt_base + wave + NWV * t) + j; kb_ok[t] = k < K; kb[t] = kb_ok[t] ? k : 0; }
    float av[U][kMT], bv[U][NTW], avn[U][kMT], bvn[U][NTW];
    auto load = [&](int r0, bool guard, float (&pa)[U][kMT], float (&pb)[U][NTW]) {
#pragma unroll
        for (int u = 0; u < U; ++u) {
            const int r = r0 + 4 * u + g;
            const bool rok = !guard || r < r_end;
            const int rc = rok ? r : r_end - 1;
            const float *dzr = dZ + (size_t)rc * kAL;
            const float *ar = SITE0 ? A + (size_t)rc * lda : A + act_off(rc, 0);
#pragma unroll
            for (int mt = 0; mt < kMT; ++mt) pa[u][mt] = dzr[fa[mt]] * ((rok & fa_ok[mt]) ? 1.0f : 0.0f);
#pragma unroll
            for (int t = 0; t < NTW; ++t) {
                float v = SITE0 ? ar[kb[t]] : ar[((kb[t] >> 4) << 8) + (kb[t] & 15)];
                bool keep = rok & kb_ok[t];
                if constexpr (SITE0) keep = keep & drop_keep1(a.seed_lo, a.seed_hi, 0, rc, kb[t], thr);
                pb[u][t] = v * (keep ? scale : 0.0f);
            }
        }
    };
    auto mma = [&]() {
#pragma unroll
        for (int u = 0; u < U; ++u) {
#pragma unroll
            for (int mt = 0; mt < kMT; ++mt) dbv[mt] += av[u][mt];
#pragma unroll
            for (int t = 0; t < NTW; ++t)
#pragma unroll
                for (int mt = 0; mt < kMT; ++mt)
                    acc[t][mt] = __builtin_amdgcn_mfma_f32_16x16x4f32(av[u][mt], bv[u][t], acc[t][mt], 0, 0, 0);
        }
    };
    const int n_full = r_end > r_begin ? (r_end - r_begin) / (4 * U) : 0;
    int r0 = r_begin;
    if (n_full > 0) {
        load(r0, false, av, bv);
        for (int it = 0; it < n_full; ++it, r0 += 4 * U) {
            if (it + 1 < n_full) load(r0 + 4 * U, false, avn, bvn);
            mma();
#pragma unroll
            for (int u = 0; u < U; ++u) {
#pragma unroll
                for (int mt = 0; mt < kMT; ++mt) av[u][mt] = avn[u][mt];
#pragma unroll
                for (int t = 0; t < NTW; ++t) bv[u][t] = bvn[u][t];
            }
        }
    }
    if (r0 < r_end) { load(r0, true, av, bv); mma(); }
    float *out = ws + (size_t)blockIdx.x * np_stride + w_off;
    float *outb = ws + (size_t)blockIdx.x * np_stride + b_off;
#pragma unroll
    for (int t = 0; t < NTW; ++t) {
        const int nt = nt_base + wave + NWV * t, k = 16 * nt + j;
#pragma unroll
        for (int mt = 0; mt < kMT; ++mt)
#pragma unroll
            for (int c = 0; c < 4; ++c) {
                const int o = 16 * mt + 4 * g + c;
                if (nt < ntk && k < K && o < kH) out[(size_t)o * K + k] = acc[t][mt][c];
            }
    }
    if (wave == 0 && nt_base == 0) {
#pragma unroll
        for (int mt = 0; mt < kMT; ++mt) {
            float v = dbv[mt];
            v += __shfl_xor(v, 16, 64);
            v += __shfl_xor(v, 32, 64);
            const int f = 16 * mt + j;
            if (g == 0 && f < kH) outb[f] = v;
        }
    }
}

template <int NTW, bool SITE0, int RB>
__global__ void __launch_bounds__(256)
mlp_bwd_dw_lds_kernel(const float *__restrict__ A, int lda, const float *__restrict__ dZ, int K, int nt_base, MlpArgs a,
                      float *__restrict__ ws, size_t np_stride, size_t w_off, size_t b_off) {
    constexpr int WA4 = 16 * NTW;
    constexpr int LDA = 64 * NTW + 16;
    constexpr int LDZ = kAL;
    constexpr int SA = RB * WA4 / 256;
    constexpr int SZ = (RB * (kAL / 4) + 255) / 256;
    extern __shared__ __attribute__((aligned(16))) float smem[];
    auto zb = [&](int b) -> float * { return smem + b * (RB * LDZ); };
    auto ab = [&](int b) -> float * { return smem + 2 * RB * LDZ + b * (RB * LDA); };

    const int R = a.R;
    const int tid = threadIdx.x, lane = tid & 63, j = lane & 15, g = lane >> 4, wave = tid >> 6;
    const int chunk = ((R + gridDim.x - 1) / gridDim.x + RB - 1) / RB * RB;
    const int r_begin = blockIdx.x * chunk, r_end = min(R, r_begin + chunk);
    const uint32_t thr = drop_thr(a.p_drop);
    const float scale = (SITE0 && a.p_drop > 0.0f) ? 1.0f / (1.0f - a.p_drop) : 1.0f;
    const int col0 = 16 * nt_base;

    int a_row[SA], a_col[SA], z_row[SZ], z_col[SZ];
    bool a_ok[SA], z_ok[SZ];
#pragma unroll
    for (int s_ = 0; s_ < SA; ++s_) {
        const int idx = s_ * 256 + tid;
        a_row[s_] = idx / WA4;
        a_col[s_] = col0 + 4 * (idx % WA4);
        a_ok[s_] = a_col[s_] < K;
    }
#pragma unroll
    for (int s_ = 0; s_ < SZ; ++s_) {
        const int idx = s_ * 256 + tid;
        z_ok[s_] = idx < RB * (kAL / 4);
        z_row[s_] = z_ok[s_] ? idx / (kAL / 4) : 0;
        z_col[s_] = z_ok[s_] ? 4 * (idx % (kAL / 4)) : 0;
    }
    f32x4 ra[SA], rz[SZ];
    auto gload = [&](int r0) {
#pragma unroll
        for (int s_ = 0; s_ < SA; ++s_) {
            const int r = r0 + a_row[s_];
            const int rc = r < r_end ? r : r_end - 1;
            const int cc = a_ok[s_] ? a_col[s_] : 0;
            ra[s_] = *reinterpret_cast<const f32x4 *>(SITE0 ? A + (size_t)rc * lda + cc : A + act_off(rc, cc));
        }
#pragma unroll
        for (int s_ = 0; s_ < SZ; ++s_) {
            const int r = r0 + z_row[s_];
            const int rc = r < r_end ? r : r_end - 1;
            rz[s_] = *reinterpret_cast<const f32x4 *>(dZ + (size_t)rc * kAL + z_col[s_]);
        }
    };
    auto lstore = [&](int buf, int r0) {
#pragma unroll
        for (int s_ = 0; s_ < SA; ++s_) {
            const int r = r0 + a_row[s_];
            const bool rok = r < r_end;
            f32x4 v = ra[s_];
            if constexpr (SITE0) {
                uint32_t w0, w1;
                drop_bits(a.seed_lo, a.seed_hi, 0, rok ? r : r_end - 1, a_col[s_] >> 2, w0, w1);
                v = drop4(v, w0, w1, thr, scale);
            }
            const float okf = (rok & a_ok[s_]) ? 1.0f : 0.0f;
#pragma unroll
            for (int c = 0; c < 4; ++c) v[c] *= okf;
            *reinterpret_cast<f32x4 *>(ab(buf) + a_row[s_] * LDA + (a_col[s_] - col0)) = v;
        }
#pragma unroll
        for (int s_ = 0; s_ < SZ; ++s_) {
            if (z_ok[s_]) {
                const float okf = (r0 + z_row[s_] < r_end) ? 1.0f : 0.0f;
                f32x4 v = rz[s_];
#pragma unroll
                for (int c = 0; c < 4; ++c) v[c] *= okf;
                *reinterpret_cast<f32x4 *>(zb(buf) + z_row[s_] * LDZ + z_col[s_]) = v;
            }
        }
    };

    f32x4 acc[NTW][kMT];
#pragma unroll
    for (int t = 0; t < NTW; ++t)
#pragma unroll
        for (int mt = 0; mt < kMT; ++mt) acc[t][mt] = f32x4{0.f, 0.f, 0.f, 0.f};
    float dbv[kMT];
#pragma unroll
    for (int mt = 0; mt < kMT; ++mt) dbv[mt] = 0.0f;

    if (r_begin < r_end) {
        gload(r_begin);
        lstore(0, r_begin);
    }
    __syncthreads();
    int buf = 0;
    for (int r0 = r_begin; r0 < r_end; r0 += RB, buf ^= 1) {
        const bool more = r0 + RB < r_end;
        if (more) gload(r0 + RB);
        const float *zs = zb(buf), *as = ab(buf);
#pragma unroll
        for (int u = 0; u < RB / 4; ++u) {
            float av[kMT], bv[NTW];
#pragma unroll
            for (int mt = 0; mt < kMT; ++mt) { av[mt] = zs[(4 * u + g) * LDZ + 16 * mt + j]; dbv[mt] += av[mt]; }
#pragma unroll
            for (int t = 0; t < NTW; ++t) bv[t] = as[(4 * u + g) * LDA + 16 * (wave + 4 * t) + j];
#pragma unroll
            for (int t = 0; t < NTW; ++t)
#pragma unroll
                for (int mt = 0; mt < kMT; ++mt)
                    acc[t][mt] = __builtin_amdgcn_mfma_f32_16x16x4f32(av[mt], bv[t], acc[t][mt], 0, 0, 0);
        }
        if (more) lstore(buf ^ 1, r0 + RB);
        __syncthreads();
    }
    float *out = ws + (size_t)blockIdx.x * np_stride + w_off;
    float *outb = ws + (size_t)blockIdx.x * np_stride + b_off;
#pragma unroll
    for (int t = 0; t < NTW; ++t) {
        const int k = col0 + 16 * (wave + 4 * t) + j;
#pragma unroll
        for (int mt = 0; mt < kMT; ++mt)
#pragma unroll
            for (int c = 0; c < 4; ++c) {
                const int o = 16 * mt + 4 * g + c;
                if (k < K && o < kH) out[(size_t)o * K + k] = acc[t][mt][c];
            }
    }
    if (wave == 0 && nt_base == 0) {
#pragma unroll
        for (int mt = 0; mt < kMT; ++mt) {
            float v = dbv[mt];
            v += __shfl_xor(v, 16, 64);
            v += __shfl_xor(v, 32, 64);
            const int f = 16 * mt + j;
            if (g == 0 && f < kH) outb[f] = v;
        }
    }
}
__host__ __device__ constexpr size_t dw_lds_bytes(int NTW, int RB) { return (size_t)(2 * RB * kAL + 2 * RB * (64 * NTW + 16)) * sizeof(float); }

__global__ void __launch_bounds__(256)
dropout_mask_kernel(MlpArgs a, int site, int n_feat, float *__restrict__ out) {
    const size_t i = (size_t)blockIdx.x * 256 + threadIdx.x;
    if (i >= (size_t)a.R * n_feat) return;
    const int row = (int)(i / n_feat), k = (int)(i % n_feat);
    out[i] = drop_keep1(a.seed_lo, a.seed_hi, site, row, k, drop_thr(a.p_drop)) ? 1.0f : 0.0f;
}

static int check_mlp(const char *who, int R, int F, int NL, float p) {
    if (R < 0 || F <= 0 || NL < 1 || NL > kMaxLayers) { set_error("%s: bad shape R=%d F=%d NL=%d", who, R, F, NL); return PTR_ERR_INVALID_ARG; }
    if (!(p >= 0.0f && p < 1.0f)) { set_error("%s: dropout p=%g out of [0,1)", who, (double)p); return PTR_ERR_INVALID_ARG; }
    const int w1g = fwd_w1_mode(F, NL);
    if (fwd_lds_floats(F, NL, w1g) * sizeof(float) > 160 * 1024 || (w1g && F % 4 != 0) || (F + 15) / 16 > 48) {
        set_error("%s: F=%d with %d hidden layers is outside the fused scorer's range (LDS %zu KB, max 160; F %% 4 == 0 needed "
                  "above ~157 features; F <= 768)", who, F, NL, fwd_lds_floats(F, NL, w1g) * sizeof(float) / 1024);
        return PTR_ERR_UNSUPPORTED;
    }
    return 0;
}

constexpr int kDwBlocksPerCu = 2;
constexpr int kDwRB = 16;

}

extern "C" size_t ptr_mlp_num_params(int F, int NL) { return ptr::n_params(NL, F); }

extern "C" size_t ptr_mlp_backward_ws_floats(int F, int NL) {
    return (size_t)ptr::kDwBlocksPerCu * ptr::num_cus() * ptr::n_params(NL, F);
}

extern "C" size_t ptr_mlp_acts_floats(int R, int NL) { return R > 0 && NL > 0 ? (size_t)NL * ptr::act_layer_floats(R) : 0; }
extern "C" size_t ptr_mlp_backward_dz_floats(int R, int F, int NL) {
    return ptr::bwd_fused_supported(F, NL, nullptr, nullptr) ? 0 : (size_t)NL * (size_t)R * ptr::kAL;
}

extern "C" int ptr_mlp_forward(const float *X, const float *params, int R, int F, int NL, int train, float p_drop, uint64_t seed,
                               float *preds, float *acts, void *stream) {
    using namespace ptr;
    const char *who = "ptr_mlp_forward";
    if (int rc = check_mlp(who, R, F, NL, p_drop)) return rc;
    if (R > 0 && (!X || !params || !preds || (train && !acts))) { set_error("%s: NULL pointer", who); return PTR_ERR_INVALID_ARG; }
    if (R == 0) return 0;
    MlpArgs a{R, F, NL, train ? p_drop : 0.0f, (uint32_t)seed, (uint32_t)(seed >> 32)};
    const int w1g = fwd_w1_mode(F, NL);
    const size_t lds = fwd_lds_floats(F, NL, w1g) * sizeof(float);
    const bool vec = (F % 4 == 0) && ((reinterpret_cast<uintptr_t>(X) & 15) == 0);
    const bool wide = train && !w1g;
    const int rows_per_tile = wide ? 16 : 32, wpb = wide ? 16 : 8;
    const int ntiles = (R + rows_per_tile - 1) / rows_per_tile;
    const int grid = ntiles < num_cus() ? ntiles : num_cus();
    auto launch = [&](auto kern) -> int {
        if (int e = allow_lds(kern, lds)) return e;
        hipLaunchKernelGGL(kern, dim3(grid > 0 ? grid : 1), dim3(wpb * 64), lds, as_stream(stream), X, params, a, preds, acts);
        return check_hip(hipGetLastError(), who);
    };
    if (w1g) {
        if (!vec) { set_error("%s: X must be 16-byte aligned for F=%d", who, F); return PTR_ERR_INVALID_ARG; }
        if (w1g == 2 && !env_int("PTR_FWD_W1_STREAM", 0))
            return train ? launch(mlp_fwd_kernel<2, 512, true, true, 2>) : launch(mlp_fwd_kernel<2, 512, false, true, 2>);
        return train ? launch(mlp_fwd_kernel<2, 512, true, true, 1>) : launch(mlp_fwd_kernel<2, 512, false, true, 1>);
    }
    if (wide) return vec ? launch(mlp_fwd_kernel<1, 1024, true, true, 0>) : launch(mlp_fwd_kernel<1, 1024, true, false, 0>);
    return vec ? launch(mlp_fwd_kernel<2, 512, false, true, 0>) : launch(mlp_fwd_kernel<2, 512, false, false, 0>);
}

namespace ptr {
int mlp_backward_impl(const char *who, const float *X, const float *params, const float *acts, const float *dpreds, int R, int F, int NL,
                             float p_drop, uint64_t seed, float *dz, float *ws, float *grad, void *stream, const OptStep &opt);
}
extern "C" int ptr_mlp_backward(const float *X, const float *params, const float *acts, const float *dpreds, int R, int F, int NL,
                                float p_drop, uint64_t seed, float *dz, float *ws, float *grad, void *stream) {
    return ptr::mlp_backward_impl("ptr_mlp_backward", X, params, acts, dpreds, R, F, NL, p_drop, seed, dz, ws, grad, stream, ptr::OptStep{});
}

extern "C" int ptr_mlp_backward_step(const float *X, float *params, const float *acts, const float *dpreds, int R, int F, int NL, float p_drop,
                                     uint64_t seed, float *dz, float *ws, float *grad, int opt_kind, float lr, float hyper1, float hyper2,
                                     float eps, float weight_decay, int step, float *state1, float *state2, const float *loss_q, int nq,
                                     float *loss_out, void *stream) {
    return ptr::mlp_backward_step_impl(X, params, acts, dpreds, R, F, NL, p_drop, seed, dz, ws, grad, opt_kind, lr, hyper1, hyper2, eps, weight_decay, step, state1,
                                       state2, loss_q, nq, loss_out, nullptr, stream);
}

int ptr::mlp_backward_step_impl(const float *X, float *params, const float *acts, const float *dpreds, int R, int F, int NL, float p_drop, uint64_t seed,
                                float *dz, float *ws, float *grad, int opt_kind, float lr, float hyper1, float hyper2, float eps, float weight_decay, int step,
                                float *state1, float *state2, const float *loss_q, int nq, float *loss_out, void *wimg, void *stream) {
    using namespace ptr;
    const char *who = "ptr_mlp_backward_step";
    OptStep o;
    if (int rc = make_opt_step(o, who, opt_kind, lr, hyper1, hyper2, eps, weight_decay, step, params, state1, state2, true, loss_q, nq, loss_out)) return rc;
    o.wimg = reinterpret_cast<uint8_t *>(wimg); o.F = F; o.NL = NL;
    return mlp_backward_impl(who, X, params, acts, dpreds, R, F, NL, p_drop, seed, dz, ws, grad, stream, o);
}

int ptr::mlp_backward_impl(const char *who, const float *X, const float *params, const float *acts, const float *dpreds, int R, int F, int NL,
                                  float p_drop, uint64_t seed, float *dz, float *ws, float *grad, void *stream, const OptStep &opt) {
    using namespace ptr;
    if (int rc = check_mlp(who, R, F, NL, p_drop)) return rc;
    if (!X || !params || !acts || !dpreds || !ws || !grad) { set_error("%s: NULL pointer", who); return PTR_ERR_INVALID_ARG; }
    hipStream_t st = as_stream(stream);
    MlpArgs a{R, F, NL, p_drop, (uint32_t)seed, (uint32_t)(seed >> 32)};
    if (R > 0 && bwd_fused_supported(F, NL, X, acts)) {
        if (int e = bwd_x6_supported(R, F, NL, X, acts) ? launch_bwd_x6(X, params, acts, dpreds, a, ws, st, who)
                                                        : launch_bwd_fused(X, params, acts, dpreds, a, ws, st, who)) return e;
        const int nb = bwd_fused_grid(R);
        const size_t NPf = n_params(NL, F);
        return launch_reduce_partials(ws, nb, nb, NPf, NPf, NPf, grad, opt, st, who);
    }
    if (!dz) { set_error("%s: dz scratch is required for this configuration (ptr_mlp_backward_dz_floats)", who); return PTR_ERR_INVALID_ARG; }
    const int ncu = num_cus();
    const int nblk = kDwBlocksPerCu * ncu;
    const size_t NP = n_params(NL, F);
    constexpr int wpb = 8;
    const int ntiles = (R + 15) / 16;
    int grid_dz = ntiles < wpb * ncu ? (ntiles + wpb - 1) / wpb : ncu;
    if (grid_dz < 1) grid_dz = 1;
    const bool tail = R > 0 && bwd_tail_supported(NL, acts);
    if (tail) {
        if (int e = bwd_x6_tail_supported(R, NL, acts) ? launch_bwd_x6_tail(params, acts, dpreds, a, ws, dz, st, who)
                                                       : launch_bwd_tail(params, acts, dpreds, a, ws, dz, st, who)) return e;
    } else {
        const size_t lds = dz_lds_floats(NL) * sizeof(float);
        auto go = [&](auto kern) -> int {
            if (int e = allow_lds(kern, lds)) return e;
            hipLaunchKernelGGL(kern, dim3(grid_dz), dim3(wpb * 64), lds, st, params, acts, dpreds, a, dz, ws, NP, off_wout(NL, F));
            return check_hip(hipGetLastError(), who);
        };
        if (int e = go(mlp_bwd_dz_kernel<1, 512>)) return e;
    }
    for (int l = 0; l < (tail ? 1 : NL); ++l) {
        const int K = l == 0 ? F : kH;
        const float *A = l == 0 ? X : acts + (size_t)(l - 1) * act_layer_floats(R);
        const int lda = l == 0 ? F : kAL;
        const float *dZ = dz + (size_t)l * R * kAL;
        const int ntk = (K + 15) / 16;
        auto go = [&](auto kern, int nt_base) -> int {
            hipLaunchKernelGGL(kern, dim3(nblk), dim3(256), 0, st, A, lda, dZ, K, nt_base, a, ws, NP, off_W(l, F), off_b(l, F));
            return check_hip(hipGetLastError(), who);
        };
        auto go_lds = [&](auto kern, int ntw, int nt_base) -> int {
            if (int e0 = allow_lds(kern, dw_lds_bytes(ntw, kDwRB))) return e0;
            hipLaunchKernelGGL(kern, dim3(nblk), dim3(256), dw_lds_bytes(ntw, kDwRB), st, A, lda, dZ, K, nt_base, a, ws, NP, off_W(l, F),
                               off_b(l, F));
            return check_hip(hipGetLastError(), who);
        };
        const bool aligned = (lda % 4 == 0) && ((reinterpret_cast<uintptr_t>(A) & 15) == 0);
        int e = 0;
        if (l == 0) {
            if (aligned) {
                if (ntk <= 12) e = go_lds(mlp_bwd_dw_lds_kernel<3, true, kDwRB>, 3, 0);
                else if (dw_x6_supported(R, K, lda, A))
                    e = launch_dw_x6(A, lda, dZ, K, ntk, a, ws, NP, off_W(l, F), off_b(l, F), nblk, st, who);
                else for (int base = 0; base < ntk && !e; base += 24) e = go_lds(mlp_bwd_dw_lds_kernel<6, true, kDwRB>, 6, base);
            } else if (ntk <= 12) e = go(mlp_bwd_dw_kernel<3, true, 4>, 0);
            else if (ntk <= 24) e = go(mlp_bwd_dw_kernel<6, true, 4>, 0);
            else if (ntk <= 48) { e = go(mlp_bwd_dw_kernel<6, true, 4>, 0); if (!e) e = go(mlp_bwd_dw_kernel<6, true, 4>, 24); }
            else { set_error("%s: F=%d not supported by the dW kernel", who, F); return PTR_ERR_UNSUPPORTED; }
        } else {
            if (!aligned) e = go(mlp_bwd_dw_kernel<2, false, 4>, 0);
            else e = go_lds(mlp_bwd_dw_lds_kernel<2, false, kDwRB>, 2, 0);
        }
        if (e) return e;
    }
    return launch_reduce_partials(ws, nblk, tail ? bwd_fused_grid(R) : grid_dz, tail ? off_W(1, F) : off_wout(NL, F), NP, NP, grad, opt, st, who);
}

extern "C" int ptr_mlp_dropout_mask(int R, int n_feat, int site, float p_drop, uint64_t seed, float *out, void *stream) {
    using namespace ptr;
    if (R < 0 || n_feat <= 0 || !out) { set_error("ptr_mlp_dropout_mask: bad arguments"); return PTR_ERR_INVALID_ARG; }
    MlpArgs a{R, n_feat, 1, p_drop, (uint32_t)seed, (uint32_t)(seed >> 32)};
    const size_t n = (size_t)R * n_feat;
    if (n == 0) return 0;
    hipLaunchKernelGGL(dropout_mask_kernel, dim3((unsigned)((n + 255) / 256)), dim3(256), 0, as_stream(stream), a, site, n_feat, out);
    return check_hip(hipGetLastError(), "ptr_mlp_dropout_mask");
}
```

### ptranking_amd/csrc/scorer_bwd_x6.hip

```cpp
#include "ptr_mlp.h"

namespace ptr {

constexpr int kB6S = 32;
constexpr int kB6ZRS = 224, kB6ZPL = kB6S * kB6ZRS, kB6ZIMG = 3 * kB6ZPL;
constexpr int kB6XRS = 288, kB6XPL = kB6S * kB6XRS, kB6XIMG = 3 * kB6XPL;
constexpr int kB6STG = kB6S * kAL * 4;
constexpr int kB6_ZA = 0, kB6_ZB = kB6ZIMG, kB6_A1 = 2 * kB6ZIMG, kB6_A2 = 3 * kB6ZIMG, kB6_XI = 4 * kB6ZIMG, kB6_ST = kB6_XI + kB6XIMG;
constexpr int kB6_WO = kB6_ST + 3 * kB6STG;
constexpr int kB6Lds = kB6_WO + 512;
static_assert(kB6Lds <= 160 * 1024, "LDS budget");

using b6_srd = __attribute__((ext_vector_type(4))) int;
using b6_rsrc = __amdgpu_buffer_rsrc_t;
__device__ __forceinline__ b6_srd b6_make_srd(const void *p, uint32_t bytes) {
    const uint64_t a = reinterpret_cast<uint64_t>(p);
    return b6_srd{(int)(uint32_t)a, (int)((uint32_t)(a >> 32) & 0xffffu), (int)bytes, 0x00020000};
}
__device__ __forceinline__ void b6_bdma16(b6_srd srd, uint32_t voff, uint32_t soff, uint32_t lds_dst) {
    unsigned keep;
    asm volatile("s_mov_b32 %0, m0\n\ts_mov_b32 m0, %4\n\ts_nop 0\n\tbuffer_load_dwordx4 %1, %2, %3 offen lds\n\ts_mov_b32 m0, %0"
                 : "=&s"(keep) : "v"(voff), "s"(srd), "s"(soff), "s"(lds_dst) : "memory");
}
__device__ __forceinline__ uint32_t b6_opaque(uint32_t x) { asm volatile("" : "+s"(x)); return x; }

template <int NT1>
__global__ void __launch_bounds__(512, 2)
mlp_bwd_x6_kernel(const float *__restrict__ X, const float *__restrict__ P, const float *__restrict__ acts, const float *__restrict__ dpreds,
                  MlpArgs a, float *__restrict__ ws, size_t np_stride, float *__restrict__ dz0) {
    static_assert(NT1 == 9 || NT1 == 0, "the X image is laid out for nine in-feature tiles; NT1 = 0 is the TAIL form");
    constexpr bool TAIL = NT1 == 0;
    extern __shared__ __attribute__((aligned(16))) uint8_t smem_b6[];
    constexpr int NL = 3;
    const int F = a.F, R = a.R;
    const int tid = threadIdx.x, lane = tid & 63, j = lane & 15, g = lane >> 4, W = __builtin_amdgcn_readfirstlane(tid >> 6);
    const uint32_t lds0 = lds_byte_addr(smem_b6);
#ifdef PTR_B6_TRACE_EDGE
    unsigned long long *etrace = reinterpret_cast<unsigned long long *>(ws + (size_t)gridDim.x * np_stride) + 8 * 256 + W * 16;
    int nedge = 0;
#define B6_EDGE() do { if (blockIdx.x == 0 && lane == 0 && nedge < 16) etrace[nedge++] = clock64(); } while (0)
#else
#define B6_EDGE() do { } while (0)
#endif
    B6_EDGE();
    const int nslabs = (R + kB6S - 1) / kB6S;
    const uint32_t thr = a.p_drop > 0.0f ? drop_thr(a.p_drop) : 0u;
    const float scale = a.p_drop > 0.0f ? 1.0f / (1.0f - a.p_drop) : 1.0f;
    const bool chain = W < 7;
    B6_EDGE();

    f32x4 st[39];
#pragma unroll
    for (int i = 0; i < 39; ++i) st[i] = f32x4{0.0f, 0.0f, 0.0f, 0.0f};
    if (chain) {
#pragma unroll
        for (int c = 0; c < 2; ++c) {
            const float *Wl = P + off_W(2 - c, F);
            const int ri = 16 * W + j;
#pragma unroll
            for (int s = 0; s < 3; ++s) {
                float v[8];
#pragma unroll
                for (int e = 0; e < 8; ++e) {
                    const int k = 32 * s + 8 * g + e;
                    v[e] = ri < kH ? Wl[(size_t)k * kH + ri] : 0.0f;
                }
                Frag pl[3];
#pragma unroll
                for (int d = 0; d < 4; ++d) split_pack2(v[2 * d], v[2 * d + 1], pl[0].u[d], pl[1].u[d], pl[2].u[d]);
#pragma unroll
                for (int p = 0; p < 3; ++p) st[18 + 3 * (3 * c + s) + p] = __builtin_bit_cast(f32x4, pl[p].q);
            }
            {
                float v[4];
#pragma unroll
                for (int e = 0; e < 4; ++e) { const int k = 96 + 4 * g + e; v[e] = (ri < kH && k < kH) ? Wl[(size_t)k * kH + ri] : 0.0f; }
                uint32_t t0[3], t1[3];
                split_pack2(v[0], v[1], t0[0], t0[1], t0[2]);
                split_pack2(v[2], v[3], t1[0], t1[1], t1[2]);
#pragma unroll
                for (int p = 0; p < 3; ++p) {
                    const int d = 2 * (3 * c + p);
                    st[36 + d / 4][d % 4] = __uint_as_float(t0[p]);
                    st[36 + d / 4][d % 4 + 1] = __uint_as_float(t1[p]);
                }
            }
        }
    }
    B6_EDGE();
    if (tid < kHP) reinterpret_cast<float *>(smem_b6 + kB6_WO)[tid] = tid < kH ? P[off_wout(NL, F) + tid] : 0.0f;
    float awo[4] = {0.0f, 0.0f, 0.0f, 0.0f}, abo = 0.0f;

    const uint32_t swz = (uint32_t)((j >> 2) & 1);
    const uint32_t wr_z = (uint32_t)(j * kB6ZRS) + 8u * ((uint32_t)g ^ (2u * swz));
    const uint32_t wr_x = (uint32_t)(j * kB6XRS) + 8u * ((uint32_t)g ^ (2u * swz));
    const uint32_t rd_b = (uint32_t)(j * kB6ZRS + 32 * (g >> 1)) + 16u * (((uint32_t)g & 1u) ^ swz);
    const uint32_t tr_z = (uint32_t)((4 * g + (j >> 2)) * kB6ZRS) + 8u * (((uint32_t)j & 3u) ^ (2u * ((uint32_t)g & 1u)));
    const uint32_t tr_x = (uint32_t)((4 * g + (j >> 2)) * kB6XRS) + 8u * (((uint32_t)j & 3u) ^ (2u * ((uint32_t)g & 1u)));

    auto mma6w = [&](f32x4 &c, int w0, const Frag (&bf)[3]) __attribute__((always_inline)) {
        Frag af[3];
#pragma unroll
        for (int p = 0; p < 3; ++p) af[p].q = __builtin_bit_cast(u32x4, st[w0 + p]);
        mma6(c, af, bf);
    };
    auto mma6t = [&](f32x4 &c, int cl, const u32x2 (&bt)[3]) __attribute__((always_inline)) {
        i16x4 at[3], bb[3];
#pragma unroll
        for (int p = 0; p < 3; ++p) {
            const int d = 2 * (3 * cl + p);
            at[p] = __builtin_bit_cast(i16x4, u32x2{__float_as_uint(st[36 + d / 4][d % 4]), __float_as_uint(st[36 + d / 4][d % 4 + 1])});
            bb[p] = __builtin_bit_cast(i16x4, bt[p]);
        }
#pragma unroll
        for (int q = 0; q < 6; ++q) c = __builtin_amdgcn_mfma_f32_16x16x16bf16_1k(at[kSixA[q]], bb[kSixB[q]], c, 0, 0, 0);
    };
    auto dw_row = [&](auto nn_, auto pipe_, int acc0, uint32_t zimg, int mo, uint32_t aimg_lane, int a_plane, int a_row, int n0) __attribute__((always_inline)) {
        constexpr int NN = decltype(nn_)::value;
        constexpr bool PIPE = decltype(pipe_)::value;
        Frag za[3];
        read_tr(za, zimg + tr_z + (uint32_t)(32 * mo), kB6ZPL, kB6ZRS, 0);
        if constexpr (PIPE && NN > 1) {
            Frag ab[2][3];
            read_tr(ab[0], aimg_lane, a_plane, a_row, n0);
#pragma unroll
            for (int n = 0; n < NN; ++n) {
                if (n + 1 < NN) read_tr(ab[(n + 1) & 1], aimg_lane, a_plane, a_row, n0 + n + 1);
                __builtin_amdgcn_sched_barrier(0);
                mma6(st[acc0 + n], za, ab[n & 1]);
                __builtin_amdgcn_sched_barrier(0);
            }
        } else {
#pragma unroll
            for (int n = 0; n < NN; ++n) {
                Frag ab[3];
                read_tr(ab, aimg_lane, a_plane, a_row, n0 + n);
                mma6(st[acc0 + n], za, ab);
                __builtin_amdgcn_sched_barrier(0);
            }
        }
    };

    f32x4 xr[2][2];
    float dsv[2];
    const b6_rsrc xsrd = __builtin_amdgcn_make_buffer_rsrc(const_cast<float *>(X), 0, TAIL ? 0 : (int)((uint32_t)R * (uint32_t)(F * 4)), 0x00020000);
    const b6_rsrc zsrd = __builtin_amdgcn_make_buffer_rsrc(dz0, 0, TAIL ? (int)((uint32_t)R * (uint32_t)(kAL * 4)) : 0, 0x00020000);
    const b6_rsrc dsrd = __builtin_amdgcn_make_buffer_rsrc(const_cast<float *>(dpreds), 0, (int)((uint32_t)R * 4u), 0x00020000);
    const b6_srd asrd = b6_make_srd(acts, (uint32_t)NL * (uint32_t)(act_layer_floats(R) * 4));
    uint32_t jx = (uint32_t)j * (uint32_t)(F * 4) + (uint32_t)g * 16, j4 = (uint32_t)j * 4, l16 = (uint32_t)lane * 16;
    asm volatile("" : "+v"(jx), "+v"(j4), "+v"(l16));
    auto load_x = [&](int slab) __attribute__((always_inline)) {
        const int row0 = slab * kB6S;
#pragma unroll
        for (int dt = 0; dt < 2; ++dt)
#pragma unroll
            for (int sl = 0; sl < 2; ++sl) {
                const int t = chain ? W : 7 + sl;
                if (!(chain && sl == 1))
                    xr[sl][dt] = __builtin_bit_cast(f32x4, __builtin_amdgcn_raw_buffer_load_b128(xsrd, (int)jx, (int)((uint32_t)(row0 + 16 * dt) * (uint32_t)(F * 4) + (uint32_t)(64 * t)), 0));
            }
    };
    uint32_t jk = (uint32_t)j * kDropRowMul + (uint32_t)g * kDropFgMul + a.seed_lo;
    asm volatile("" : "+v"(jk));
    auto stage_x_tile = [&](int row0, int t_, const f32x4 (&x2)[2]) __attribute__((always_inline)) {
        const int t = (int)b6_opaque((uint32_t)t_);
        int col = 16 * t + 4 * g;
        asm volatile("" : "+v"(col));
#pragma unroll
        for (int dt = 0; dt < 2; ++dt) {
            uint32_t w0, w1;
            drop_bits_key(jk + ((uint32_t)(row0 + 16 * dt) * kDropRowMul + (uint32_t)(4 * t) * kDropFgMul), a.seed_hi, w0, w1);
            f32x4 v = drop4(x2[dt], w0, w1, thr, scale);
#pragma unroll
            for (int r = 0; r < 4; ++r) v[r] = col + r < F ? v[r] : (col + r == F ? 1.0f : 0.0f);
            split_write4(b6_opaque(lds0 + kB6_XI + (uint32_t)(32 * t)) + wr_x + (uint32_t)(16 * dt * kB6XRS), kB6XPL, v);
        }
    };
    auto stage_x = [&](int slab) __attribute__((always_inline)) {
        if (chain) stage_x_tile(slab * kB6S, W, xr[0]);
        else { stage_x_tile(slab * kB6S, 7, xr[0]); stage_x_tile(slab * kB6S, 8, xr[1]); }
    };
    auto prefetch = [&](int slab) __attribute__((always_inline)) {
        const int row0 = slab * kB6S;
#pragma unroll
        for (int q = 0; q < 6; ++q) {
            const int k = chain ? W + 7 * q : 3 * 14;
            if (k < 3 * 14) {
                const int layer = k / 14, ch = k - 14 * layer;
                b6_bdma16(asrd, l16, (uint32_t)layer * (uint32_t)(act_layer_floats(R) * 4) + (uint32_t)row0 * (kAL * 4) + (uint32_t)ch * 1024,
                          __builtin_amdgcn_readfirstlane(lds0 + (uint32_t)(kB6_ST + layer * kB6STG + ch * 1024)));
            }
        }
#pragma unroll
        for (int dt = 0; dt < 2; ++dt)
            dsv[dt] = __builtin_bit_cast(float, __builtin_amdgcn_raw_buffer_load_b32(dsrd, (int)j4, (int)((uint32_t)(row0 + 16 * dt) * 4u), 0));
    };
    uint32_t m2 = 0u, m1 = 0u;
    auto staging = [&](uint32_t zdst) __attribute__((always_inline)) {
        m2 = 0u; m1 = 0u;
        if (chain) {
            const f32x4 wo4 = *reinterpret_cast<lds_f32x4 *>((uintptr_t)(b6_opaque(lds0 + (uint32_t)(kB6_WO + 64 * W)) + (uint32_t)(16 * g)));
#pragma unroll
            for (int dt = 0; dt < 2; ++dt) {
                const uint32_t so = b6_opaque(lds0 + (uint32_t)(kB6_ST + 1024 * W)) + (uint32_t)(j * 64 + 16 * g) + (uint32_t)(dt * kActTile * 4);
                const f32x4 a1 = *reinterpret_cast<lds_f32x4 *>((uintptr_t)so);
                const f32x4 a2 = *reinterpret_cast<lds_f32x4 *>((uintptr_t)(so + kB6STG));
                const f32x4 a3 = *reinterpret_cast<lds_f32x4 *>((uintptr_t)(so + 2 * kB6STG));
                const float ds = dsv[dt];
                f32x4 z3;
#pragma unroll
                for (int r = 0; r < 4; ++r) {
                    z3[r] = a3[r] > 0.0f ? ds * wo4[r] : 0.0f;
                    awo[r] = fmaf(ds, a3[r], awo[r]);
                    m2 |= (a2[r] > 0.0f ? 1u : 0u) << (4 * dt + r);
                    m1 |= (a1[r] > 0.0f ? 1u : 0u) << (4 * dt + r);
                }
                if (W == 0 && g == 0) abo += ds;
                const uint32_t wo = wr_z + b6_opaque(lds0 + (uint32_t)(32 * W)) + (uint32_t)(16 * dt * kB6ZRS);
                split_write4(wo + b6_opaque(zdst), kB6ZPL, z3);
                split_write4(wo + kB6_A2, kB6ZPL, a2);
                split_write4(wo + kB6_A1, kB6ZPL, a1);
            }
        }
    };
    const int slab0 = blockIdx.x;
    prefetch(slab0 < nslabs ? slab0 : nslabs - 1);
    asm volatile("s_waitcnt vmcnt(0)" ::: "memory");
    __syncthreads();
    B6_EDGE();

#ifdef PTR_B6_TRACE
    unsigned long long *trace = reinterpret_cast<unsigned long long *>(ws + (size_t)gridDim.x * np_stride) + W * 256;
    int nstamp = 0;
#define B6_STAMP() do { if (blockIdx.x == 0 && lane == 0 && nstamp < 256) trace[nstamp++] = clock64(); } while (0)
#else
#define B6_STAMP() do { } while (0)
#endif
#if defined(PTR_B6_TRACE) && defined(PTR_B6_TRACE2)
#define B6_STAMP2() B6_STAMP()
#else
#define B6_STAMP2() do { } while (0)
#endif
    uint32_t zi = kB6_ZA, zo = kB6_ZB;
    staging(zi);
    wg_barrier();
    {
        const int nxt = slab0 + (int)gridDim.x;
        prefetch(nxt < nslabs ? nxt : nslabs - 1);
    }
    for (int slab = slab0; slab < nslabs; slab += gridDim.x) {
        B6_STAMP();
#pragma unroll
        for (int c = 0; c < 2; ++c) {
            if constexpr (!TAIL) { if (c == 1) load_x(slab); }
            const uint32_t zin = b6_opaque(lds0 + (c == 0 ? zi : zo)), zout = b6_opaque(lds0 + (c == 0 ? zo : zi) + (uint32_t)(32 * W));
            const uint32_t aim = b6_opaque(lds0 + (c == 0 ? kB6_A2 : kB6_A1));
            if (chain) {
              auto chain_part = [&]() __attribute__((always_inline)) {
                f32x4 cc[2] = {f32x4{0.f, 0.f, 0.f, 0.f}, f32x4{0.f, 0.f, 0.f, 0.f}};
                auto read_b = [&](Frag (&b)[3], int u) __attribute__((always_inline)) {
#pragma unroll
                    for (int p = 0; p < 3; ++p)
                        b[p].q = *reinterpret_cast<lds_u32x4 *>((uintptr_t)(zin + rd_b + (uint32_t)(p * kB6ZPL + 16 * (u & 1) * kB6ZRS + 64 * (u >> 1))));
                };
                u32x2 bt[2][3];
                auto read_bt = [&]() __attribute__((always_inline)) {
#pragma unroll
                    for (int dt = 0; dt < 2; ++dt)
#pragma unroll
                        for (int p = 0; p < 3; ++p)
                            bt[dt][p] = *reinterpret_cast<lds_u32x2 *>((uintptr_t)(zin + wr_z + (uint32_t)(192 + p * kB6ZPL + 16 * dt * kB6ZRS)));
                };
                if (c == 0) {
                    Frag b[2][3];
                    read_b(b[0], 0);
#pragma unroll
                    for (int u = 0; u < 6; ++u) {
                        if (u + 1 < 6) read_b(b[(u + 1) & 1], u + 1);
                        else read_bt();
                        __builtin_amdgcn_sched_barrier(0);
                        mma6w(cc[u & 1], 18 + 3 * (3 * c + (u >> 1)), b[u & 1]);
                        __builtin_amdgcn_sched_barrier(0);
                    }
                } else {
#pragma unroll
                    for (int u = 0; u < 6; ++u) {
                        Frag b[3];
                        read_b(b, u);
                        if (u == 5) read_bt();
                        mma6w(cc[u & 1], 18 + 3 * (3 * c + (u >> 1)), b);
                        __builtin_amdgcn_sched_barrier(0);
                    }
                }
#pragma unroll
                for (int dt = 0; dt < 2; ++dt) {
                    mma6t(cc[dt], c, bt[dt]);
                    __builtin_amdgcn_sched_barrier(0);
                }
                B6_STAMP2();
                const uint32_t m = c == 0 ? m2 : m1;
#pragma unroll
                for (int dt = 0; dt < 2; ++dt) {
                    f32x4 dz;
#pragma unroll
                    for (int r = 0; r < 4; ++r) dz[r] = (m >> (4 * dt + r)) & 1u ? cc[dt][r] * scale : 0.0f;
                    if (TAIL && c == 1) {
                        const uint32_t row = (uint32_t)(slab * kB6S + 16 * dt + j);
                        __builtin_amdgcn_raw_buffer_store_b128(__builtin_bit_cast(u32x4, dz), zsrd, (int)(row < (uint32_t)R ? row * (kAL * 4) + (uint32_t)(64 * W + 16 * g) : 0xFFFFF000u), 0, 0);
                    } else {
                        split_write4(zout + wr_z + (uint32_t)(16 * dt * kB6ZRS), kB6ZPL, dz);
                    }
                }
                B6_STAMP2();
              };
              auto dw_part = [&]() __attribute__((always_inline)) {
                if (c == 0) dw_row(std::integral_constant<int, 5>{}, std::true_type{}, 0, zin, W, aim + tr_z, kB6ZPL, kB6ZRS, 0);
                else dw_row(std::integral_constant<int, 5>{}, std::false_type{}, 5, zin, W, aim + tr_z, kB6ZPL, kB6ZRS, 0);
              };
              chain_part();
              dw_part();
            } else {
                B6_STAMP2(); B6_STAMP2();
                constexpr int ZD = 2;
                Frag ab5[3], ab6[3], zr[ZD][3];
                read_tr(zr[0], zin + tr_z, kB6ZPL, kB6ZRS, 0);
                read_tr(ab5, aim + tr_z, kB6ZPL, kB6ZRS, 5);
                read_tr(ab6, aim + tr_z, kB6ZPL, kB6ZRS, 6);
#pragma unroll
                for (int d = 1; d < ZD - 1; ++d) read_tr(zr[d], zin + tr_z + (uint32_t)(32 * d), kB6ZPL, kB6ZRS, 0);
#pragma unroll
                for (int mo = 0; mo < 7; ++mo) {
                    if (mo + ZD - 1 < 7) read_tr(zr[(mo + ZD - 1) % ZD], zin + tr_z + (uint32_t)(32 * (mo + ZD - 1)), kB6ZPL, kB6ZRS, 0);
                    __builtin_amdgcn_sched_barrier(0);
                    mma6(st[14 * c + 2 * mo], zr[mo % ZD], ab5);
                    mma6(st[14 * c + 2 * mo + 1], zr[mo % ZD], ab6);
                    __builtin_amdgcn_sched_barrier(0);
                }
            }
            if constexpr (!TAIL) { if (c == 1) stage_x(slab); }
            if (c == 0 && slab != slab0) {
                const int nxt = slab + (int)gridDim.x;
                prefetch(nxt < nslabs ? nxt : nslabs - 1);
            }
            if (c == 1) asm volatile("s_waitcnt vmcnt(0)" ::: "memory");
            B6_STAMP();
            wg_barrier();
            B6_STAMP();
        }
        const bool more = slab + (int)gridDim.x < nslabs;
        if constexpr (TAIL) {
            if (more) staging(zo);
        } else {
            const uint32_t za = b6_opaque(lds0 + zi), xi = b6_opaque(lds0 + kB6_XI) + tr_x;
            if (more) staging(zo);
            __builtin_amdgcn_sched_barrier(0);
            B6_STAMP2();
            if (chain) {
                dw_row(std::integral_constant<int, 8>{}, std::true_type{}, 10, za, W, xi, kB6XPL, kB6XRS, 0);
            } else {
                Frag xb[3], zr[2][3];
                read_tr(zr[0], za + tr_z, kB6ZPL, kB6ZRS, 0);
                read_tr(xb, xi, kB6XPL, kB6XRS, 8);
#pragma unroll
                for (int mo = 0; mo < 7; ++mo) {
                    if (mo + 1 < 7) read_tr(zr[(mo + 1) & 1], za + tr_z + (uint32_t)(32 * (mo + 1)), kB6ZPL, kB6ZRS, 0);
                    __builtin_amdgcn_sched_barrier(0);
                    mma6(st[28 + mo], zr[mo & 1], xb);
                    __builtin_amdgcn_sched_barrier(0);
                }
            }
        }
        B6_STAMP();
        wg_barrier();
        B6_STAMP();
        const uint32_t tz = zi; zi = zo; zo = tz;
    }
    asm volatile("s_waitcnt vmcnt(0)" ::: "memory");
    B6_EDGE();

    float *out = ws + (size_t)blockIdx.x * np_stride;
    auto store_tile = [&](const f32x4 &c, int layer, int mo, int ni) __attribute__((always_inline)) {
        const int K = layer == 0 ? F : kH;
        const int in = 16 * ni + j;
#pragma unroll
        for (int r = 0; r < 4; ++r) {
            const int o = 16 * mo + 4 * g + r;
            if (o < kH) {
                if (in < K) out[off_W(layer, F) + (size_t)o * K + in] = c[r];
                else if (in == K) out[off_b(layer, F) + o] = c[r];
            }
        }
    };
    if (chain) {
#pragma unroll
        for (int n = 0; n < 5; ++n) { store_tile(st[n], 2, W, n); store_tile(st[5 + n], 1, W, n); }
        if constexpr (!TAIL) {
#pragma unroll
            for (int n = 0; n < 8; ++n) store_tile(st[10 + n], 0, W, n);
        }
#pragma unroll
        for (int r = 0; r < 4; ++r) {
            float v = awo[r];
#pragma unroll
            for (int m = 1; m < 16; m <<= 1) v += __shfl_xor(v, m, 64);
            const int f = 16 * W + 4 * g + r;
            if (j == 0 && f < kH) out[off_wout(NL, F) + f] = v;
        }
        if (W == 0) {
            float v = abo;
#pragma unroll
            for (int m = 1; m < 16; m <<= 1) v += __shfl_xor(v, m, 64);
            if (lane == 0) out[off_wout(NL, F) + kH] = v;
        }
    } else {
#pragma unroll
        for (int mo = 0; mo < 7; ++mo) {
#pragma unroll
            for (int q = 0; q < 2; ++q) { store_tile(st[2 * mo + q], 2, mo, 5 + q); store_tile(st[14 + 2 * mo + q], 1, mo, 5 + q); }
            if constexpr (!TAIL) store_tile(st[28 + mo], 0, mo, 8);
        }
    }
#ifdef PTR_B6_TRACE_EDGE
    asm volatile("s_waitcnt vmcnt(0)" ::: "memory");
    B6_EDGE();
#endif
}

bool bwd_x6_supported(int R, int F, int NL, const void *X, const void *acts) {
    if (!env_int("PTR_BWD_X6", 1)) return false;
    const int NT1 = (F + 15) / 16;
    if ((uint64_t)NL * (uint64_t)act_layer_floats(R) * 4 >= 0xFFFFF000ull || (uint64_t)R * (uint64_t)F * 4 >= 0xFFFFF000ull) return false;
    return NL == 3 && NT1 == 9 && F % 4 == 0 && F < 16 * NT1 && (reinterpret_cast<uintptr_t>(X) & 15) == 0 && (reinterpret_cast<uintptr_t>(acts) & 15) == 0;
}
int launch_bwd_x6(const float *X, const float *params, const float *acts, const float *dpreds, const MlpArgs &a, float *ws, hipStream_t st,
                  const char *who) {
    const int grid = bwd_fused_grid(a.R);
    const size_t NP = n_params(a.NL, a.F);
    auto kern = mlp_bwd_x6_kernel<9>;
    if (int e = allow_lds(kern, kB6Lds)) return e;
    hipLaunchKernelGGL(kern, dim3(grid), dim3(512), kB6Lds, st, X, params, acts, dpreds, a, ws, NP, (float *)nullptr);
    return check_hip(hipGetLastError(), who);
}

bool bwd_x6_tail_supported(int R, int NL, const void *acts) {
    if (!env_int("PTR_BWD_X6", 1)) return false;
    if ((uint64_t)NL * (uint64_t)act_layer_floats(R) * 4 >= 0xFFFFF000ull || (uint64_t)R * (kAL * 4) >= 0xFFFFF000ull) return false;
    return NL == 3 && (reinterpret_cast<uintptr_t>(acts) & 15) == 0;
}
int launch_bwd_x6_tail(const float *params, const float *acts, const float *dpreds, const MlpArgs &a, float *ws, float *dz0, hipStream_t st,
                       const char *who) {
    const int grid = bwd_fused_grid(a.R);
    const size_t NP = n_params(a.NL, a.F);
    auto kern = mlp_bwd_x6_kernel<0>;
    if (int e = allow_lds(kern, kB6Lds)) return e;
    hipLaunchKernelGGL(kern, dim3(grid), dim3(512), kB6Lds, st, (const float *)nullptr, params, acts, dpreds, a, ws, NP, dz0);
    return check_hip(hipGetLastError(), who);
}

}
```

### ptranking_amd/csrc/train_step.hip

```cpp
#include "ptr_mlp.h"

extern "C" int ptr_train_step(const ptr_train_step_desc *d, void *stream) {
    using namespace ptr;
    const char *who = "ptr_train_step";
    if (!d) { set_error("%s: NULL descriptor", who); return PTR_ERR_INVALID_ARG; }
    if (d->struct_bytes != (int32_t)sizeof(ptr_train_step_desc)) {
        set_error("%s: descriptor of %d bytes, this library expects %d (ABI v%d)", who, (int)d->struct_bytes, (int)sizeof(ptr_train_step_desc), PTR_ABI_VERSION);
        return PTR_ERR_INVALID_ARG;
    }
    if (d->B < 0 || d->L <= 0 || (int64_t)d->B * d->L > 0x7fffffffll) { set_error("%s: bad shape B=%d L=%d", who, d->B, d->L); return PTR_ERR_INVALID_ARG; }
    if (d->loss_kind < PTR_LOSS_RANKNET || d->loss_kind > PTR_LOSS_LISTNET) { set_error("%s: unknown loss %d", who, d->loss_kind); return PTR_ERR_INVALID_ARG; }
    if (!d->loss_q || !d->dpreds || !d->preds) { set_error("%s: NULL scratch pointer", who); return PTR_ERR_INVALID_ARG; }
    const int R = d->B * d->L;
    hipStream_t st = as_stream(stream);
    auto mark = [&](int k) -> int { return d->events[k] ? check_hip(hipEventRecord(reinterpret_cast<hipEvent_t>(d->events[k]), st), who) : 0; };
    if (int rc = mark(0)) return rc;
    if (int rc = d->wimg ? mlp_forward_x6_impl(d->X, d->params, R, d->F, d->NL, 1, d->p_drop, d->seed, d->preds, d->acts, d->wimg, d->wimg_current == 0, stream)
                         : ptr_mlp_forward(d->X, d->params, R, d->F, d->NL, 1, d->p_drop, d->seed, d->preds, d->acts, stream)) return rc;
    if (int rc = mark(1)) return rc;
    int rc = 0;
    switch (d->loss_kind) {
    case PTR_LOSS_RANKNET: rc = ptr_ranknet_fwd_bwd(d->preds, d->labels, d->lens, d->B, d->L, d->loss_f[0], nullptr, d->loss_q, d->dpreds, stream); break;
    case PTR_LOSS_LAMBDARANK: rc = ptr_lambdarank_fwd_bwd(d->preds, d->labels, d->lens, d->B, d->L, d->loss_f[0], nullptr, d->loss_q, d->dpreds, stream); break;
    case PTR_LOSS_LAMBDALOSS:
        rc = ptr_lambdaloss_fwd_bwd(d->preds, d->labels, d->lens, d->B, d->L, d->loss_i[0], d->loss_f[0], d->loss_f[1], d->loss_i[1], d->loss_i[2], nullptr,
                                    d->loss_q, d->dpreds, stream);
        break;
    default: rc = ptr_listnet_fwd_bwd(d->preds, d->labels, d->lens, d->B, d->L, nullptr, d->loss_q, d->dpreds, stream); break;
    }
    if (rc) return rc;
    if (int rc2 = mark(2)) return rc2;
    if (int rc3 = mlp_backward_step_impl(d->X, d->params, d->acts, d->dpreds, R, d->F, d->NL, d->p_drop, d->seed, d->dz, d->ws, d->grad, d->opt_kind, d->lr, d->hyper1,
                                         d->hyper2, d->eps, d->weight_decay, d->step, d->state1, d->state2, d->loss_q, d->B, d->loss_out, d->wimg, stream)) return rc3;
    return mark(3);
}
```

### ptranking_amd/rankers.py

```python
import copy
import ctypes as C
import math
import os

import torch

from . import _lib
from . import dp
from . import functional as F_
from .host import DeviceEvaluator, DeviceTrainLoop, PointScorerRanker, is_multilabel
from .listsf import FusedListScorerMixin
from .scorer import (FLAT_OPTIMIZERS, FlatOptimizer, FusedPointScorer, FusedScorerMixin, alloc_acts, mlp_forward, opt_step_c_values, x6_wimg_for,
                     x6_image_tag, x6_set_image_tag)

RANKER_NAMES = ("RankNet", "LambdaRank", "LambdaLoss", "ApproxNDCG", "ListNet", "ListMLE", "STListNet", "RankCosine", "RankMSE", "SoftRank",
                "WassRank")
EXTRA_RANKER_NAMES = ("DASALC", "MDPRank")
METRIC_RANKER_NAMES = ("SmoothMetric",)
PROB_RANKER_NAMES = ("ProbSmoothMetric",)
PROB_SORT_IDS = ('ExpRele', 'RiskAware', 'RERAR')

DEFAULT_PARAS = {
    "RankNet": dict(model_id="RankNet", sigma=1.0),
    "LambdaRank": dict(model_id="LambdaRank", sigma=1.0),
    "LambdaLoss": dict(model_id="LambdaLoss", k=5, sigma=1.0, mu=5.0, loss_type="NDCG_Loss2"),
    "ApproxNDCG": dict(model_id="ApproxNDCG", alpha=10),
    "ListNet": dict(model_id="ListNet"),
    "ListMLE": dict(model_id="ListMLE"),
    "STListNet": dict(model_id="STListNet", temperature=1.0),
    "RankCosine": dict(model_id="RankCosine"),
    "RankMSE": dict(model_id="RankMSE"),
    "SoftRank": dict(model_id="SoftRank", delta=2.0, metric='nDCG', top_k=None),
    "DASALC": dict(model_id="DASALC"),
    "MDPRank": dict(model_id="MDPRank", temperature=1.0, gamma=1.0, top_k=10, distribution='PL'),
    "WassRank": dict(model_id="WassRank", mode='SinkhornOT', sh_itr=20, lam=0.1, smooth_type='ST', norm_type='BothST',
                     cost_type='eg', non_rele_gap=100, var_penalty=math.e, gain_base=4),
    "SmoothMetric": dict(model_id="SmoothMetric", metric='nDCG', alpha=10, top_k=None, opt_ideal=True),
    "ProbSmoothMetric": dict(model_id="ProbSmoothMetric", metric='nDCG', top_k=None, opt_ideal=True, limit_delta=0.01, const_std=None,
                             sort_id='ExpRele'),
}


class FusedStepMixin:

    data_parallel = True
    _grad_bucket = None
    _dp_single = None

    use_direct_step = True
    fuse_optimizer_step = True
    single_call_step = True
    reuse_weight_image = True
    _direct_loss = None
    _direct_owner = None

    def _direct_check(self, kwargs):
        """The reference's asserts of the loss (run on the direct path too)."""

    def _loss_values(self, kwargs):
        return {}

    def _direct_train_op(self, X, Y, kwargs):
        spec = self._direct_loss
        sf = getattr(self, "point_sf", None)
        if (spec is None or not self.use_direct_step or not isinstance(sf, FusedPointScorer) or not isinstance(self.optimizer, FlatOptimizer)
                or type(self).custom_loss_function is not self._direct_owner.custom_loss_function or not sf.training
                or not torch.is_grad_enabled() or not (X.is_cuda and X.dim() == 3 and X.dtype == torch.float32 and X.is_contiguous())
                or not (Y.is_cuda and Y.dtype == torch.float32 and Y.is_contiguous() and Y.shape == X.shape[:2])
                or X.size(2) != sf.num_features or len(self.optimizer.param_groups) != 1):
            return None
        od = self.optimizer.__dict__
        if 'zero_grad' in od or ('step' in od and not getattr(od['step'], '_wrapped_by_lr_sched', False)):
            return None
        self._direct_check(kwargs)
        lens = kwargs.get('lens')
        B, L, Fd = X.shape
        if L > _lib.MAX_LIST_LEN or (lens is not None and not (lens.is_cuda and lens.dtype == torch.int32 and lens.is_contiguous()
                                                               and lens.shape == (B,))):
            return None
        R, NL, dev = B * L, sf.num_layers, X.device
        cache = self.__dict__.setdefault("_direct_buffers", {})
        buf = cache.get((B, L))
        if buf is None:
            if len(cache) >= 4:
                cache.pop(next(iter(cache)))
            ndz = _lib.query("ptr_mlp_backward_dz_floats", R, Fd, NL)
            buf = dict(preds=torch.empty((B, L), device=dev), acts=alloc_acts(R, NL, dev),
                       loss_q=torch.empty(max(B, 1), device=dev), dpreds=torch.empty((B, L), device=dev),
                       ws=torch.empty(_lib.query("ptr_mlp_backward_ws_floats", Fd, NL), device=dev),
                       dz=torch.empty(ndz, device=dev) if ndz else None)
            cache[(B, L)] = buf
        flat = sf.flat
        if flat.grad is None or flat.grad.shape != flat.shape or not flat.grad.is_contiguous():
            flat.grad = torch.empty_like(flat)
        p = sf.dropout
        seed = int(torch.randint(0, 2 ** 62, (1,)).item()) if p > 0.0 else 0
        if p > 0.0:
            seed = dp.local_dropout_seed(seed, R, local_queries=B)
        dp.end_step()
        loss = torch.empty(1, device=dev)
        values = self._loss_values(kwargs)
        distributed = self.data_parallel and dp.is_distributed()
        fuse_step = self.fuse_optimizer_step and not distributed and type(self.optimizer) in FLAT_OPTIMIZERS.values()
        if fuse_step and self.single_call_step:
            return self._single_call_step(X, Y, lens, buf, flat, B, L, Fd, NL, R, p, seed, spec, values, kwargs, loss, dev)
        with torch.cuda.device(dev):
            st = _lib.current_stream(dev)
            mlp_forward(X, flat, R, Fd, NL, 1, p, seed, buf["preds"], buf["acts"], dev)
            stop_training = False
            if 'epoch_k' in kwargs and kwargs['epoch_k'] % self.stop_check_freq == 0:
                stop_training = self.stop_training(buf["preds"])
            dp_fused = distributed and self.fuse_optimizer_step and type(self.optimizer) in FLAT_OPTIMIZERS.values()
            _lib.call(spec.entry, _lib.ptr(buf["preds"]), _lib.ptr(Y), _lib.ptr(lens), B, L, *spec.c_args(**values),
                      None if (fuse_step or dp_fused) else _lib.ptr(loss), _lib.ptr(buf["loss_q"]), _lib.ptr(buf["dpreds"]), st)
            if fuse_step:
                opt = opt_step_c_values(self.optimizer.fused_step_args(flat)).values()
                try:
                    _lib.call("ptr_mlp_backward_step", _lib.ptr(X), _lib.ptr(flat), _lib.ptr(buf["acts"]), _lib.ptr(buf["dpreds"]), R, Fd, NL, C.c_float(p),
                              C.c_uint64(seed), _lib.ptr(buf["dz"]), _lib.ptr(buf["ws"]), _lib.ptr(flat.grad), *opt, _lib.ptr(buf["loss_q"]), B, _lib.ptr(loss), st)
                except Exception:
                    self.optimizer.undo_step(flat)
                    raise
            else:
                _lib.call("ptr_mlp_backward", _lib.ptr(X), _lib.ptr(flat), _lib.ptr(buf["acts"]), _lib.ptr(buf["dpreds"]), R, Fd, NL, C.c_float(p),
                          C.c_uint64(seed), _lib.ptr(buf["dz"]), _lib.ptr(buf["ws"]), _lib.ptr(flat.grad), st)
                if distributed:
                    dp.all_reduce_sum(flat.grad)
                if dp_fused:
                    opt = opt_step_c_values(self.optimizer.fused_step_args(flat)).values()
                    try:
                        _lib.call("ptr_opt_step_loss", _lib.ptr(flat), _lib.ptr(flat.grad), C.c_int64(flat.numel()), *opt, _lib.ptr(buf["loss_q"]), B,
                                  _lib.ptr(loss), st)
                    except Exception:
                        self.optimizer.undo_step(flat)
                        raise
                else:
                    self.optimizer.step_flat(flat)
        return loss.reshape(()), stop_training

    def _single_call_step(self, X, Y, lens, buf, flat, B, L, Fd, NL, R, p, seed, spec, values, kwargs, loss, dev):
        d = buf.get("desc")
        if d is None:
            d = buf["desc"] = _lib.TrainStepDesc()
            d.struct_bytes = C.sizeof(_lib.TrainStepDesc)
            d.loss_kind = spec.kind
            d.B, d.L, d.F, d.NL = B, L, Fd, NL
            for k in ("preds", "acts", "loss_q", "dpreds", "dz", "ws"):
                setattr(d, k, None if buf[k] is None else buf[k].data_ptr())
        li, lf = spec.desc_arrays(**values)
        d.loss_i[:len(li)], d.loss_f[:len(lf)] = li, lf
        wimg = x6_wimg_for(X, R, Fd, NL, True, dev)
        d.wimg = None if wimg is None else wimg.data_ptr()
        d.X, d.labels, d.lens = X.data_ptr(), Y.data_ptr(), (None if lens is None else lens.data_ptr())
        st_ = self.optimizer.state.get(flat)
        step_before = int(st_["step"]) if st_ else 0
        d.wimg_current = int(wimg is not None and self.reuse_weight_image and os.environ.get("PTR_REUSE_IMG", "1") != "0" and
                             x6_image_tag(dev, Fd, NL) == (flat.data_ptr(), flat._version, step_before, wimg.data_ptr()))
        timing = _lib.TIMING
        evs = None
        if timing is not None:
            evs = [torch.cuda.Event(enable_timing=True) for _ in range(4)]
            for k, ev in enumerate(evs):
                ev.record()
                d.events[k] = ev.cuda_event
        else:
            for k in range(4):
                d.events[k] = None
        opt = opt_step_c_values(self.optimizer.fused_step_args(flat))
        for name, v in opt.items():
            setattr(d, name, v)
        step = opt["step"]
        d.p_drop, d.seed = p, seed
        d.params, d.grad = flat.data_ptr(), flat.grad.data_ptr()
        d.loss_out = loss.data_ptr()
        if wimg is not None:
            x6_set_image_tag(dev, Fd, NL, None)
        try:
            with torch.cuda.device(dev):
                _lib.TIMING = None
                try:
                    _lib.call("ptr_train_step", C.addressof(d), _lib.current_stream(dev))
                finally:
                    _lib.TIMING = timing
        except Exception:
            self.optimizer.undo_step(flat)
            raise
        if wimg is not None:
            x6_set_image_tag(dev, Fd, NL, (flat.data_ptr(), flat._version, step, wimg.data_ptr()))
        if evs is not None:
            timing.setdefault("ptr_mlp_forward_x6" if wimg is not None else "ptr_mlp_forward", []).append((evs[0], evs[1]))
            timing.setdefault(spec.entry, []).append((evs[1], evs[2]))
            timing.setdefault("ptr_mlp_backward_step", []).append((evs[2], evs[3]))
        stop_training = False
        if 'epoch_k' in kwargs and kwargs['epoch_k'] % self.stop_check_freq == 0:
            stop_training = self.stop_training(buf["preds"])
        return loss.reshape(()), stop_training

    def _bucket(self, extra=0):
        if self._grad_bucket is None or self._grad_bucket.extra != extra:
            if hasattr(self.optimizer, "grad_bucket"):
                self._grad_bucket = self.optimizer.grad_bucket(extra)
            else:
                self._grad_bucket = dp.FlatGradBucket(list(self.get_parameters()), extra=extra)
        return self._grad_bucket

    def _fused_step(self, loss):
        if self.data_parallel and dp.is_distributed():
            if self._dp_single is None:
                ps = [p for p in self.get_parameters() if p.requires_grad]
                self._dp_single = ps[0] if len(ps) == 1 else False
            if self._dp_single is not False:
                self.optimizer.zero_grad()
                loss.backward()
                if self._dp_single.grad is None:
                    self._dp_single.grad = torch.zeros_like(self._dp_single)
                stack = getattr(self.optimizer, "stack", None)
                if stack is not None:
                    stack.reattach_grads()
                dp.all_reduce_sum(self._dp_single.grad)
            else:
                bucket = self._bucket()
                bucket.zero()
                loss.backward()
                bucket.all_reduce()
        else:
            self.optimizer.zero_grad()
            loss.backward()
        self.optimizer.step()
        dp.end_step()
        return loss

    def _batch_mean_step(self, loss, b_local):
        if not (self.data_parallel and dp.is_distributed()):
            return self._fused_step(loss)
        b_local = float(b_local)
        bucket = self._bucket(extra=2)
        bucket.zero()
        loss.backward()
        bucket.flat[:bucket.numel].mul_(b_local)
        bucket.extras[0] = b_local
        bucket.extras[1] = loss.detach() * b_local
        bucket.all_reduce()
        b_global = bucket.extras[0].clone()
        bucket.flat[:bucket.numel].div_(b_global)
        self.optimizer.step()
        return bucket.extras[1] / b_global


class RankNetLoss(FusedStepMixin):
    _direct_loss = _lib.LOSSES["ranknet"]

    def _loss_values(self, kwargs):
        return dict(sigma=self.sigma)

    def custom_loss_function(self, batch_preds, batch_std_labels, **kwargs):
        return self._fused_step(F_.ranknet_loss(batch_preds, batch_std_labels, sigma=self.sigma, lens=kwargs.get('lens')))


class LambdaRankLoss(FusedStepMixin):
    _direct_loss = _lib.LOSSES["lambdarank"]

    def _loss_values(self, kwargs):
        return dict(sigma=self.sigma)

    def _direct_check(self, kwargs):
        assert 'label_type' in kwargs and is_multilabel(kwargs['label_type'])
        assert 'presort' in kwargs and kwargs['presort'] is True

    def custom_loss_function(self, batch_preds, batch_std_labels, **kwargs):
        self._direct_check(kwargs)
        return self._fused_step(F_.lambdarank_loss(batch_preds, batch_std_labels, sigma=self.sigma, lens=kwargs.get('lens')))


class LambdaLossLoss(FusedStepMixin):
    _direct_loss = _lib.LOSSES["lambdaloss"]

    def _loss_values(self, kwargs):
        return dict(k=self.k, sigma=self.sigma, mu=getattr(self, 'mu', 5.0), loss_type=F_.LAMBDALOSS_TYPES[self.loss_type],
                    presort=bool('presort' in kwargs and kwargs['presort']))

    def _direct_check(self, kwargs):
        assert is_multilabel(kwargs['label_type'])
        if self.loss_type not in F_.LAMBDALOSS_TYPES:
            raise NotImplementedError(f"LambdaLoss type {self.loss_type!r} (supported: {sorted(F_.LAMBDALOSS_TYPES)})")

    def custom_loss_function(self, batch_preds, batch_std_labels, **kwargs):
        self._direct_check(kwargs)
        presort = bool('presort' in kwargs and kwargs['presort'])
        loss = F_.lambdaloss_loss(batch_preds, batch_std_labels, k=self.k, sigma=self.sigma, mu=getattr(self, 'mu', 5.0),
                                  loss_type=self.loss_type, presort=presort, lens=kwargs.get('lens'))
        return self._fused_step(loss)


class ApproxNDCGLoss(FusedStepMixin):
    couple_batch = True

    def uniform_eval_setting(self, **kwargs):
        eval_dict = kwargs['eval_dict']
        if eval_dict["do_validation"] and not eval_dict['vali_metric'] == 'nDCG':
            eval_dict['vali_metric'] = "nDCG"

    def custom_loss_function(self, batch_preds, batch_std_labels, **kwargs):
        assert is_multilabel(kwargs['label_type'])
        presort = bool('presort' in kwargs and kwargs['presort'])
        if not (self.data_parallel and dp.is_distributed() and self.couple_batch):
            loss = F_.approxndcg_loss(batch_preds, batch_std_labels, alpha=self.alpha, presort=presort,
                                      couple_batch=self.couple_batch, lens=kwargs.get('lens'))
            return self._fused_step(loss)
        loss1, parts = F_.approxndcg_loss(batch_preds, batch_std_labels, alpha=self.alpha, presort=presort,
                                          couple_batch=True, grad_scale_override=1.0, return_parts=True, lens=kwargs.get('lens'))
        bucket = self._bucket(extra=2)
        bucket.zero()
        loss1.backward()
        bucket.extras[0] = parts["scale"][1]
        bucket.extras[1] = -loss1.detach()
        bucket.all_reduce()
        S, D = bucket.extras[0].clone(), bucket.extras[1].clone()
        bucket.flat[:bucket.numel].mul_(S)
        self.optimizer.step()
        return -(D * S)


class SoftRankLoss(FusedStepMixin):
    def custom_loss_function(self, batch_preds, batch_std_labels, **kwargs):
        assert 'presort' in kwargs and kwargs['presort'] is True
        assert 'nDCG' == self.metric
        assert is_multilabel(kwargs['label_type'])
        return self._fused_step(F_.softrank_loss(batch_preds, batch_std_labels, delta=self.delta_value, top_k=self.top_k,
                                                 lens=kwargs.get('lens')))


class SmoothMetricLoss(FusedStepMixin):
    max_label = None

    def uniform_eval_setting(self, **kwargs):
        eval_dict = kwargs['eval_dict']
        if eval_dict["do_validation"] and not eval_dict['vali_metric'] == self.metric:
            eval_dict['vali_metric'] = self.metric

    def custom_loss_function(self, batch_preds, batch_std_labels, **kwargs):
        assert 'presort' in kwargs and kwargs['presort'] is True
        assert 'label_type' in kwargs and is_multilabel(kwargs['label_type'])
        if self.metric == 'nERR' and self.max_label is None and self.data_parallel and dp.is_distributed():
            raise ValueError("SmoothMetric nERR under data parallelism needs model_para_dict['max_label']: the batch maximum is rank-local")
        return self._fused_step(F_.smooth_metric_objective(batch_preds, batch_std_labels, self.metric, alpha=self.alpha, top_k=self.top_k,
                                                           opt_ideal=self.opt_ideal, max_label=self.max_label, lens=kwargs.get('lens')))


class ProbSmoothMetricLoss(FusedStepMixin):
    max_label = None
    const_std = None
    limit_delta = 0.01
    sort_id = 'ExpRele'
    risk_b = 0.1

    def uniform_eval_setting(self, **kwargs):
        eval_dict = kwargs['eval_dict']
        if eval_dict["do_validation"] and not eval_dict['vali_metric'] == self.metric:
            eval_dict['vali_metric'] = self.metric

    def _head(self, batch_components):
        if self.const_std is not None:
            return batch_components, None
        to_var = torch.exp if self.limit_delta is None else (lambda s: torch.sigmoid(s) * self.limit_delta)
        return batch_components[:, :, 0], to_var(batch_components[:, :, 1])

    def _sort_scores(self, batch_mus, batch_vars, lens=None):
        if 'ExpRele' == self.sort_id:
            return batch_mus
        if batch_vars is None:
            batch_vars = torch.full_like(batch_mus, float(self.const_std) ** 2)
        if 'RiskAware' == self.sort_id:
            return batch_mus - self.risk_b * batch_vars
        ranks = F_.expected_ranks(batch_mus.contiguous(), batch_vars.contiguous(), lens=lens)
        return torch.where(ranks > 0, 1.0 / ranks, torch.zeros_like(ranks))

    def forward(self, batch_q_doc_vectors):
        B, L = batch_q_doc_vectors.size(0), batch_q_doc_vectors.size(1)
        out = self.point_sf(batch_q_doc_vectors)
        return out.view(B, L) if self.const_std is not None else out.view(B, L, 2)

    def predict(self, batch_q_doc_vectors, lens=None):
        if lens is None:
            lens = getattr(self, '_batch_lens', None)
        return self._sort_scores(*self._head(self.forward(batch_q_doc_vectors)), lens=lens)

    def custom_loss_function(self, batch_preds, batch_std_labels, **kwargs):
        assert 'presort' in kwargs and kwargs['presort'] is True
        assert 'label_type' in kwargs and is_multilabel(kwargs['label_type'])
        if self.metric == 'nERR' and self.max_label is None and self.data_parallel and dp.is_distributed():
            raise ValueError("ProbSmoothMetric nERR under data parallelism needs model_para_dict['max_label']: the batch maximum is rank-local")
        batch_mus, batch_vars = self._head(batch_preds)
        return self._fused_step(F_.gaussian_metric_objective(batch_mus, batch_vars, batch_std_labels, self.metric, top_k=self.top_k,
                                                             opt_ideal=self.opt_ideal, max_label=self.max_label, lens=kwargs.get('lens'),
                                                             const_std=self.const_std))


class MDPRankLoss(FusedStepMixin):
    sampler = "torch"
    samples_per_query = 1
    _pl_seed = 137
    _pl_calls = 0

    def _query_offset(self, B, kwargs):
        if kwargs.get('q0') is not None:
            return int(kwargs['q0'])
        if not (self.data_parallel and dp.is_distributed()) or dp.world_size() == 1:
            return 0
        if dp.QUERY_SHARD is not None and dp.QUERY_SHARD[1] == B:
            return int(dp.QUERY_SHARD[0])
        return dp.rank() * B

    def _device_sampled_step(self, batch_preds, batch_std_labels, lens, kwargs):
        if self.distribution not in F_.PL_DISTRIBUTIONS:
            raise NotImplementedError
        self._pl_calls += 1
        loss = F_.mdprank_sampled_loss(batch_preds, batch_std_labels, top_k=self.top_k, gamma=self.gamma, temperature=self.temperature,
                                       distribution=self.distribution, samples=self.samples_per_query,
                                       seed=self._pl_seed * 0x9E3779B1 + self._pl_calls, q0=self._query_offset(batch_preds.size(0), kwargs),
                                       lens=lens)
        return self._fused_step(loss)

    def custom_loss_function(self, batch_preds, batch_std_labels, **kwargs):
        assert 'presort' in kwargs and kwargs['presort'] is True
        lens = kwargs.get('lens')
        if self.sampler == 'device':
            return self._device_sampled_step(batch_preds, batch_std_labels, lens, kwargs)
        with torch.no_grad():
            det = batch_preds.detach()
            if lens is not None:
                pad = torch.arange(det.size(1), device=det.device)[None, :] >= lens[:, None].to(det.device)
                det = det.masked_fill(pad, -1e30)
            if 'PL' == self.distribution:
                t = det / self.temperature if 1.0 != self.temperature else det
                probs = torch.exp(t - torch.max(t, dim=1, keepdim=True)[0]).clamp_min(1e-38)
                perm = torch.multinomial(probs, num_samples=det.size(1), replacement=False)
                if lens is not None:
                    is_pad = (perm >= lens[:, None].to(perm.device)).to(torch.int8)
                    perm = torch.gather(perm, 1, torch.sort(is_pad, dim=1, stable=True)[1])
                noise = None
            elif 'STPL' == self.distribution:
                unif = torch.rand(det.size(), device=det.device)
                noise = -torch.log(-torch.log(unif + 1e-20) + 1e-20)
                logits = det + noise if 1.0 == self.temperature else (det + noise) / self.temperature
                perm = torch.sort(logits, dim=1, descending=True)[1]
            else:
                raise NotImplementedError
        if noise is None:
            action_preds = batch_preds
        else:
            action_preds = batch_preds + noise if 1.0 == self.temperature else (batch_preds + noise) / self.temperature
        loss = F_.mdprank_loss(action_preds, batch_std_labels, perm, top_k=self.top_k, gamma=self.gamma, lens=lens)
        return self._fused_step(loss)


class ListNetLoss(FusedStepMixin):
    _direct_loss = _lib.LOSSES["listnet"]

    def custom_loss_function(self, batch_preds, batch_std_labels, **kwargs):
        return self._fused_step(F_.listnet_loss(batch_preds, batch_std_labels, lens=kwargs.get('lens')))


class STListNetLoss(FusedStepMixin):
    def custom_loss_function(self, batch_preds, batch_std_labels, **kwargs):
        unif = torch.rand(batch_preds.size(), device=batch_preds.device)
        return self._fused_step(F_.stlistnet_loss(batch_preds, batch_std_labels, temperature=self.temperature, unif=unif,
                                                  lens=kwargs.get('lens')))


class RankCosineLoss(FusedStepMixin):
    def custom_loss_function(self, batch_preds, batch_std_labels, **kwargs):
        return self._fused_step(F_.rankcosine_loss(batch_preds, batch_std_labels, lens=kwargs.get('lens')))


class RankMSELoss(FusedStepMixin):
    def custom_loss_function(self, batch_preds, batch_std_labels, **kwargs):
        loss = F_.rankmse_loss(batch_preds, batch_std_labels, lens=kwargs.get('lens'))
        return self._batch_mean_step(loss, batch_preds.size(0))


class WassRankLoss(FusedStepMixin):
    def custom_loss_function(self, batch_preds, batch_std_labels, **kwargs):
        wd = self.wass_para_dict
        loss = F_.wassrank_loss(batch_preds, batch_std_labels, cost_type=wd['cost_type'], lam=wd['lam'], sh_itr=wd['sh_itr'],
                                gain_base=wd['gain_base'], non_rele_gap=wd['non_rele_gap'], var_penalty=wd['var_penalty'],
                                scale_by_max_label=self.TL_AF in ('S', 'ST'), lens=kwargs.get('lens'))
        return self._batch_mean_step(loss, batch_preds.size(0))


class ListMLELoss(FusedStepMixin):
    tie_shuffle = "device"
    _tie_seed = 137
    _tie_calls = 0

    def _shuffle_ties(self, batch_std_labels, lens=None):
        if self.tie_shuffle == "device" or lens is not None:
            self._tie_calls += 1
            return F_.shuffle_ties_order(batch_std_labels, seed=self._tie_seed * 0x9E3779B1 + self._tie_calls, lens=lens)
        B, L = batch_std_labels.shape
        dev = batch_std_labels.device
        if B > 1:
            rperms = torch.stack([torch.randperm(L, device=dev) for _ in range(B)], dim=0)
        else:
            rperms = torch.randperm(L, device=dev).view(1, -1)
        shuffled = torch.gather(batch_std_labels, dim=1, index=rperms)
        desc = torch.argsort(shuffled, descending=True)
        return torch.gather(rperms, dim=1, index=desc)

    def custom_loss_function(self, batch_preds, batch_std_labels, **kwargs):
        lens = kwargs.get('lens')
        perm = self._shuffle_ties(batch_std_labels, lens)
        return self._fused_step(F_.listmle_loss(batch_preds, perm, lens=lens))


for _cls in (RankNetLoss, LambdaRankLoss, LambdaLossLoss, ListNetLoss):
    _cls._direct_owner = _cls


def make_ranker_classes(base=PointScorerRanker):

    class RankNet(RankNetLoss, FusedScorerMixin, FusedListScorerMixin, DeviceTrainLoop, DeviceEvaluator, base):
        def __init__(self, sf_para_dict=None, model_para_dict=None, gpu=False, device=None):
            base.__init__(self, id='RankNet', sf_para_dict=sf_para_dict, gpu=gpu, device=device)
            self.sigma = model_para_dict['sigma']

    class LambdaRank(LambdaRankLoss, FusedScorerMixin, FusedListScorerMixin, DeviceTrainLoop, DeviceEvaluator, base):
        def __init__(self, sf_para_dict=None, model_para_dict=None, gpu=False, device=None):
            base.__init__(self, id='LambdaRank', sf_para_dict=sf_para_dict, gpu=gpu, device=device)
            self.sigma = model_para_dict['sigma']

    class LambdaLoss(LambdaLossLoss, FusedScorerMixin, FusedListScorerMixin, DeviceTrainLoop, DeviceEvaluator, base):
        def __init__(self, sf_para_dict=None, model_para_dict=None, gpu=False, device=None):
            base.__init__(self, id='LambdaLoss', sf_para_dict=sf_para_dict, gpu=gpu, device=device)
            self.lambdaloss_dict = model_para_dict
            self.k, self.sigma, self.loss_type = model_para_dict['k'], model_para_dict['sigma'], model_para_dict['loss_type']
            if 'NDCG_Loss2++' == self.loss_type:
                self.mu = model_para_dict['mu']
            if self.loss_type not in F_.LAMBDALOSS_TYPES:
                raise NotImplementedError(f"loss_type {self.loss_type!r}")

    class ApproxNDCG(ApproxNDCGLoss, FusedScorerMixin, FusedListScorerMixin, DeviceTrainLoop, DeviceEvaluator, base):
        def __init__(self, sf_para_dict=None, model_para_dict=None, gpu=False, device=None):
            base.__init__(self, id='ApproxNDCG', sf_para_dict=sf_para_dict, gpu=gpu, device=device)
            self.alpha = model_para_dict['alpha']

    class ListNet(ListNetLoss, FusedScorerMixin, FusedListScorerMixin, DeviceTrainLoop, DeviceEvaluator, base):
        def __init__(self, sf_para_dict=None, gpu=False, device=None):
            base.__init__(self, id='ListNet', sf_para_dict=sf_para_dict, gpu=gpu, device=device)

    class ListMLE(ListMLELoss, FusedScorerMixin, FusedListScorerMixin, DeviceTrainLoop, DeviceEvaluator, base):
        def __init__(self, sf_para_dict=None, model_para_dict=None, gpu=False, device=None):
            base.__init__(self, id='ListMLE', sf_para_dict=sf_para_dict, gpu=gpu, device=device)

    class STListNet(STListNetLoss, FusedScorerMixin, FusedListScorerMixin, DeviceTrainLoop, DeviceEvaluator, base):
        def __init__(self, sf_para_dict=None, model_para_dict=None, gpu=False, device=None):
            base.__init__(self, id='STListNet', sf_para_dict=sf_para_dict, gpu=gpu, device=device)
            self.temperature = model_para_dict['temperature']

    class RankCosine(RankCosineLoss, FusedScorerMixin, FusedListScorerMixin, DeviceTrainLoop, DeviceEvaluator, base):
        def __init__(self, sf_para_dict=None, gpu=False, device=None):
            base.__init__(self, id='RankCosine', sf_para_dict=sf_para_dict, gpu=gpu, device=device)

    class RankMSE(RankMSELoss, FusedScorerMixin, FusedListScorerMixin, DeviceTrainLoop, DeviceEvaluator, base):
        def __init__(self, sf_para_dict=None, gpu=False, device=None):
            base.__init__(self, id='RankMSE', sf_para_dict=sf_para_dict, gpu=gpu, device=device)

    class SoftRank(SoftRankLoss, FusedScorerMixin, FusedListScorerMixin, DeviceTrainLoop, DeviceEvaluator, base):
        def __init__(self, sf_para_dict=None, model_para_dict=None, gpu=False, device=None):
            base.__init__(self, id='SoftRank', sf_para_dict=sf_para_dict, gpu=gpu, device=device)
            self.delta_value = float(model_para_dict['delta'])
            self.delta = torch.tensor([self.delta_value], device=self.device)
            self.top_k = model_para_dict['top_k']
            self.metric = model_para_dict['metric']

    class DASALC(ListNetLoss, FusedScorerMixin, FusedListScorerMixin, DeviceTrainLoop, DeviceEvaluator, base):

        def __init__(self, sf_para_dict=None, gpu=False, device=None):
            base.__init__(self, id='DASALC', sf_para_dict=sf_para_dict, gpu=gpu, device=device)
            assert 'listsf' == sf_para_dict['sf_id']

    class MDPRank(MDPRankLoss, FusedScorerMixin, FusedListScorerMixin, DeviceTrainLoop, DeviceEvaluator, base):
        def __init__(self, sf_para_dict=None, model_para_dict=None, gpu=False, device=None):
            base.__init__(self, id='MDPRank', sf_para_dict=sf_para_dict, gpu=gpu, device=device)
            self.gamma = model_para_dict['gamma']
            self.top_k = model_para_dict['top_k']
            self.temperature = model_para_dict['temperature']
            self.distribution = model_para_dict['distribution']
            self.sampler = model_para_dict.get('sampler', 'torch')
            self.samples_per_query = int(model_para_dict.get('samples_per_query', 1))
            if self.sampler not in ('torch', 'device'):
                raise ValueError(f"MDPRank sampler {self.sampler!r} (supported: 'torch', 'device')")
            if self.samples_per_query < 1 or (self.sampler == 'torch' and self.samples_per_query != 1):
                raise ValueError("MDPRank samples_per_query must be >= 1, and 1 with sampler='torch'")
            self.pg_checking = False

    class WassRank(WassRankLoss, FusedScorerMixin, FusedListScorerMixin, DeviceTrainLoop, DeviceEvaluator, base):

        def __init__(self, sf_para_dict, wass_para_dict=None, dict_cost_mats=None, dict_std_dists=None, gpu=False, device=None):
            base.__init__(self, id='WassRank', sf_para_dict=sf_para_dict, gpu=gpu, device=device)
            self.TL_AF = self.get_tl_af()
            self.wass_para_dict = dict(DEFAULT_PARAS['WassRank']) if wass_para_dict is None else wass_para_dict
            if dict_cost_mats is not None:
                self.dict_cost_mats = dict_cost_mats
            if dict_std_dists is not None:
                self.dict_std_dists = dict_std_dists
            wd = self.wass_para_dict
            if wd['mode'] != 'SinkhornOT':
                raise NotImplementedError(f"WassRank mode {wd['mode']!r}: only mode='SinkhornOT' is served")
            if wd['smooth_type'] != 'ST':
                raise NotImplementedError(f"WassRank smooth_type {wd['smooth_type']!r}: only smooth_type='ST' is served")
            if wd.get('norm_type', 'BothST') != 'BothST':
                raise NotImplementedError(f"WassRank norm_type {wd['norm_type']!r}: only norm_type='BothST' is served")
            if wd['cost_type'] not in F_.WASS_COST_TYPES:
                raise NotImplementedError(f"WassRank cost_type {wd['cost_type']!r} (supported: {sorted(F_.WASS_COST_TYPES)})")

    class SmoothMetric(SmoothMetricLoss, FusedScorerMixin, FusedListScorerMixin, DeviceTrainLoop, DeviceEvaluator, base):

        def __init__(self, sf_para_dict=None, model_para_dict=None, gpu=False, device=None):
            base.__init__(self, id='SmoothMetric', sf_para_dict=sf_para_dict, gpu=gpu, device=device)
            self.metric = model_para_dict['metric']
            if self.metric not in ('P', 'AP', 'nERR', 'nDCG'):
                raise NotImplementedError(f"metric {self.metric!r} (supported: 'P', 'AP', 'nERR', 'nDCG')")
            self.alpha = model_para_dict['alpha']
            self.top_k = model_para_dict['top_k']
            self.opt_ideal = bool(model_para_dict['opt_ideal'])
            self.max_label = model_para_dict.get('max_label')

    class ProbSmoothMetric(ProbSmoothMetricLoss, FusedScorerMixin, DeviceTrainLoop, DeviceEvaluator, base):

        def __init__(self, sf_para_dict=None, model_para_dict=None, gpu=False, device=None):
            sf_id = sf_para_dict['sf_id']
            if sf_id != 'pointsf':
                raise NotImplementedError(f"ProbSmoothMetric with sf_id={sf_id!r}: the point scorer (sf_id='pointsf') only")
            self.metric = model_para_dict['metric']
            if self.metric not in ('P', 'AP', 'nERR', 'nDCG'):
                raise NotImplementedError(f"metric {self.metric!r} (supported: 'P', 'AP', 'nERR', 'nDCG')")
            self.sort_id = model_para_dict.get('sort_id', 'ExpRele')
            if self.sort_id not in PROB_SORT_IDS:
                raise ValueError(f"sort_id {self.sort_id!r} (supported: {PROB_SORT_IDS})")
            self.const_std = model_para_dict.get('const_std')
            if self.const_std is not None and not float(self.const_std) > 0.0:
                raise ValueError(f"const_std must be > 0 (got {self.const_std!r})")
            sf_para_dict = copy.deepcopy(sf_para_dict)
            sf_para_dict[sf_id]['out_dim'] = 1 if self.const_std is not None else 2
            base.__init__(self, id='ProbSmoothMetric', sf_para_dict=sf_para_dict, gpu=gpu, device=device)
            self.top_k = model_para_dict['top_k']
            self.opt_ideal = bool(model_para_dict['opt_ideal'])
            self.max_label = model_para_dict.get('max_label')
            self.limit_delta = model_para_dict.get('limit_delta', 0.01)

    out = dict(RankNet=RankNet, LambdaRank=LambdaRank, LambdaLoss=LambdaLoss, ApproxNDCG=ApproxNDCG, ListNet=ListNet,
               ListMLE=ListMLE, STListNet=STListNet, RankCosine=RankCosine, RankMSE=RankMSE, SoftRank=SoftRank, WassRank=WassRank,
               DASALC=DASALC, MDPRank=MDPRank, SmoothMetric=SmoothMetric, ProbSmoothMetric=ProbSmoothMetric)
    for name, cls in out.items():
        cls.__name__ = cls.__qualname__ = name
        cls.__module__ = __name__
    return out


_standalone = make_ranker_classes(PointScorerRanker)
RankNet, LambdaRank, LambdaLoss = _standalone["RankNet"], _standalone["LambdaRank"], _standalone["LambdaLoss"]
ApproxNDCG, ListNet, ListMLE = _standalone["ApproxNDCG"], _standalone["ListNet"], _standalone["ListMLE"]
STListNet, RankCosine, RankMSE = _standalone["STListNet"], _standalone["RankCosine"], _standalone["RankMSE"]
SoftRank, DASALC, MDPRank = _standalone["SoftRank"], _standalone["DASALC"], _standalone["MDPRank"]
WassRank = _standalone["WassRank"]
SmoothMetric = _standalone["SmoothMetric"]
ProbSmoothMetric = _standalone["ProbSmoothMetric"]
```

Baseline: 5.554 million.

## Cache split-bf16 backward weight image, refreshed by fused optimizer step

Adds a persistent pre-split bf16x3 image of the hidden-layer weights for the x6 backward kernel. The optimizer epilogue writes it alongside the updated parameters, so the backward kernel no longer gathers and splits the weights on every step. A tag check skips re-preparing the image when parameters are unchanged. The optimizer reduction kernel also loads param and state values before the reduction to hide their latency. This costs extra scattered 2-byte stores in the optimizer and adds staleness-tracking complexity.

```diff
diff --git a/include/ptranking_amd.h b/include/ptranking_amd.h
--- a/include/ptranking_amd.h
+++ b/include/ptranking_amd.h
@@ -228,6 +228,11 @@
     int32_t reserved;
 } ptr_train_step_desc;
 int ptr_train_step(const ptr_train_step_desc *d, void *stream);
+size_t ptr_mlp_bwd_x6_img_bytes(int F, int NL);
+int ptr_mlp_bwd_x6_img_prep(const float *params, int F, int NL, void *bimg, void *stream);
+int ptr_mlp_backward_x6_img(const float *X, const float *params, const float *acts, const float *dpreds, int R, int F, int NL,
+                            float p_drop, uint64_t seed, float *dz, float *ws, float *grad, const void *bimg, void *stream);
+int ptr_train_step_img(const ptr_train_step_desc *d, void *bimg, int bimg_current, void *stream);
 int ptr_mlp_dropout_mask(int R, int n_feat, int site, float p_drop, uint64_t seed, float *out, void *stream);
 
 #define PTR_LINEAR_NONE 0
diff --git a/ptranking_amd/_lib.py b/ptranking_amd/_lib.py
--- a/ptranking_amd/_lib.py
+++ b/ptranking_amd/_lib.py
@@ -59,6 +59,10 @@
     "ptr_mlp_backward_step": [_vp, _vp, _vp, _vp, _i, _i, _i, _f, _u64, _vp, _vp, _vp, _i, _f, _f, _f, _f, _f, _i, _vp, _vp, _vp, _i, _vp, _vp],
     "ptr_opt_step_loss": [_vp, _vp, C.c_int64, _i, _f, _f, _f, _f, _f, _i, _vp, _vp, _vp, _i, _vp, _vp],
     "ptr_train_step": [_vp, _vp],
+    "ptr_mlp_bwd_x6_img_bytes": [_i, _i],
+    "ptr_mlp_bwd_x6_img_prep": [_vp, _i, _i, _vp, _vp],
+    "ptr_mlp_backward_x6_img": [_vp, _vp, _vp, _vp, _i, _i, _i, _f, _u64, _vp, _vp, _vp, _vp, _vp],
+    "ptr_train_step_img": [_vp, _vp, _i, _vp],
     "ptr_mlp_x6_ws_bytes": [_i, _i],
     "ptr_mlp_forward_x6": [_vp, _vp, _i, _i, _i, _i, _f, _u64, _vp, _vp, _vp, _vp],
     "ptr_adam_step": [_vp, _vp, _vp, _vp, C.c_int64, _f, _f, _f, _f, _f, _i, _vp],
@@ -105,7 +109,7 @@
     "ptr_letor_load": [C.c_char_p, _i, _f, C.c_int64, C.c_int32, C.c_int64, _vp, _i, _vp, _vp, _vp],
 }
 _RESTYPES = {"ptr_last_error": C.c_char_p, "ptr_mlp_num_params": C.c_size_t, "ptr_mlp_backward_ws_floats": C.c_size_t,
-             "ptr_mlp_backward_dz_floats": C.c_size_t, "ptr_mlp_acts_floats": C.c_size_t, "ptr_mlp_x6_ws_bytes": C.c_size_t, "ptr_linear_backward_weight_ws_floats": C.c_size_t, "ptr_bn_ws_floats": C.c_size_t,
+             "ptr_mlp_backward_dz_floats": C.c_size_t, "ptr_mlp_acts_floats": C.c_size_t, "ptr_mlp_x6_ws_bytes": C.c_size_t, "ptr_mlp_bwd_x6_img_bytes": C.c_size_t, "ptr_linear_backward_weight_ws_floats": C.c_size_t, "ptr_bn_ws_floats": C.c_size_t,
              "ptr_bn_slot_floats": C.c_size_t, "ptr_gbdt_partition_ws_ints": C.c_size_t,
              "ptr_gbdt_partition_segments_ws_ints": C.c_size_t,
              "ptr_layernorm_backward_ws_floats": C.c_size_t}
diff --git a/ptranking_amd/csrc/optim.hip b/ptranking_amd/csrc/optim.hip
--- a/ptranking_amd/csrc/optim.hip
+++ b/ptranking_amd/csrc/optim.hip
@@ -19,6 +19,11 @@
     const size_t ica = ia < n ? ia : n - 1, icb = ib < n ? ib : n - 1;
     const int nba = ica >= tail_begin ? nblk_tail : nblk, nbb = icb >= tail_begin ? nblk_tail : nblk;
     const int nbc = nba < nbb ? nba : nbb;
+    const int col = 64 * w + lane;
+    const size_t i = (size_t)blockIdx.x * kRedElems + col;
+    const bool mine = w < 2 && i < n;
+    float pi = 0.f, s1i = 0.f, s2i = 0.f;
+    if (mine && o.kind) { pi = o.param[i]; s1i = o.s1[i]; if (o.kind == PTR_OPT_ADAM) s2i = o.s2[i]; }
     float a0 = 0.f, a1 = 0.f, a2 = 0.f, a3 = 0.f, b0 = 0.f, b1 = 0.f, b2 = 0.f, b3 = 0.f;
     int b = w;
     for (; b + 48 < nbc; b += 64) {
@@ -49,16 +54,15 @@
     part[w][lane] = (a0 + a1) + (a2 + a3);
     part[w][64 + lane] = (b0 + b1) + (b2 + b3);
     __syncthreads();
-    const int col = 64 * w + lane;
-    const size_t i = (size_t)blockIdx.x * kRedElems + col;
-    if (w < 2 && i < n) {
+    if (mine) {
         float s = part[0][col];
 #pragma unroll
         for (int k = 1; k < 16; ++k) s += part[k][col];
         if (grad) grad[i] = s;
         if (o.kind) {
-            const float pn = opt_update(o, i, s);
+            const float pn = opt_update_loaded(o, i, s, pi, s1i, s2i);
             if (o.wimg) x6_img_put(o.wimg, o.F, o.NL, i, pn);
+            if (o.bimg) b6_img_put(o.bimg, o.F, i, pn);
         }
     }
 }
diff --git a/ptranking_amd/csrc/ptr_b6img.h b/ptranking_amd/csrc/ptr_b6img.h
--- /dev/null
+++ b/ptranking_amd/csrc/ptr_b6img.h
@@ -0,0 +1,30 @@
+#pragma once
+
+#if defined(__HIPCC__)
+#define PTR_B6_HD __host__ __device__
+#else
+#define PTR_B6_HD
+#endif
+
+namespace ptr {
+
+constexpr int kB6ImgSlots = 21, kB6ImgBytes = kB6ImgSlots * 7 * 1024;
+
+PTR_B6_HD inline int b6_img_off(int l, int k, int ri, int p) {
+    const int c = 2 - l, W = ri >> 4, j = ri & 15;
+    int slot, g, byte;
+    if (k < 96) {
+        const int s = k >> 5, e = k & 7;
+        g = (k & 31) >> 3;
+        slot = 3 * (3 * c + s) + p;
+        byte = 2 * e;
+    } else {
+        const int e = (k - 96) & 3, d = 2 * (3 * c + p) + (e >> 1);
+        g = (k - 96) >> 2;
+        slot = 18 + d / 4;
+        byte = 4 * (d % 4) + 2 * (e & 1);
+    }
+    return (slot * 7 + W) * 1024 + (16 * g + j) * 16 + byte;
+}
+
+}
diff --git a/ptranking_amd/csrc/ptr_mlp.h b/ptranking_amd/csrc/ptr_mlp.h
--- a/ptranking_amd/csrc/ptr_mlp.h
+++ b/ptranking_amd/csrc/ptr_mlp.h
@@ -5,6 +5,7 @@
 #include "ptr_device.h"
 #include "ptr_dropout.h"
 #include "ptr_x6.h"
+#include "ptr_b6img.h"
 
 namespace ptr {
 
@@ -65,6 +66,20 @@
 }
 #endif
 
+#if defined(__HIPCC__)
+__device__ __forceinline__ void b6_img_put(uint8_t *__restrict__ img, int F, size_t i, float x) {
+    const size_t w2 = off_W(1, F);
+    if (i < w2 || i >= w2 + 2 * (size_t)(kH * kH + kH)) return;
+    const int jj = (int)(i - w2), l = 1 + jj / (kH * kH + kH), q = jj - (l - 1) * (kH * kH + kH);
+    if (q >= kH * kH) return;
+    const int k = q / kH, ri = q - k * kH;
+    uint16_t p[3];
+    split_pack1(x, p[0], p[1], p[2]);
+#pragma unroll
+    for (int pl = 0; pl < 3; ++pl) *reinterpret_cast<uint16_t *>(img + b6_img_off(l, k, ri, pl)) = p[pl];
+}
+#endif
+
 template <int N, class Fn> __device__ __forceinline__ void static_for(Fn &&f) {
     [&]<int... I>(std::integer_sequence<int, I...>) { (f(std::integral_constant<int, I>{}), ...); }(std::make_integer_sequence<int, N>{});
 }
@@ -79,12 +94,14 @@
                     const char *who);
 
 bool bwd_x6_supported(int R, int F, int NL, const void *X, const void *acts);
-int launch_bwd_x6(const float *X, const float *params, const float *acts, const float *dpreds, const MlpArgs &a, float *ws, hipStream_t st,
-                  const char *who);
+int launch_bwd_x6(const float *X, const float *params, const float *acts, const float *dpreds, const MlpArgs &a, float *ws, const void *bimg,
+                  hipStream_t st, const char *who);
 
 bool bwd_x6_tail_supported(int R, int NL, const void *acts);
-int launch_bwd_x6_tail(const float *params, const float *acts, const float *dpreds, const MlpArgs &a, float *ws, float *dz0, hipStream_t st,
-                       const char *who);
+int launch_bwd_x6_tail(const float *params, const float *acts, const float *dpreds, const MlpArgs &a, float *ws, float *dz0, const void *bimg,
+                       hipStream_t st, const char *who);
+size_t bwd_x6_img_bytes(int F, int NL);
+int launch_b6_prep(const float *params, int F, void *bimg, hipStream_t st, const char *who);
 
 bool dw_x6_supported(int R, int K, int lda, const void *A);
 int launch_dw_x6(const float *A, int lda, const float *dZ, int K, int ntk, const MlpArgs &a, float *ws, size_t np_stride, size_t w_off, size_t b_off,
@@ -94,6 +111,6 @@
                         void *wimg, bool prep, void *stream);
 int mlp_backward_step_impl(const float *X, float *params, const float *acts, const float *dpreds, int R, int F, int NL, float p_drop, uint64_t seed, float *dz,
                            float *ws, float *grad, int opt_kind, float lr, float hyper1, float hyper2, float eps, float weight_decay, int step, float *state1,
-                           float *state2, const float *loss_q, int nq, float *loss_out, void *wimg, void *stream);
+                           float *state2, const float *loss_q, int nq, float *loss_out, void *wimg, void *bimg, void *stream);
 
 }
diff --git a/ptranking_amd/csrc/ptr_optim.h b/ptranking_amd/csrc/ptr_optim.h
--- a/ptranking_amd/csrc/ptr_optim.h
+++ b/ptranking_amd/csrc/ptr_optim.h
@@ -11,6 +11,7 @@
     float *param, *s1, *s2;
     const float *loss_q; int nq; float *loss_out;
     uint8_t *wimg; int F, NL;
+    uint8_t *bimg;
 };
 
 inline int make_opt_step(OptStep &o, const char *who, int opt_kind, float lr, float hyper1, float hyper2, float eps, float weight_decay, int step,
@@ -32,18 +33,17 @@
                            hipStream_t st, const char *who);
 
 #if defined(__HIPCC__)
-__device__ __forceinline__ float opt_update(const OptStep &o, size_t i, float g) {
-    const float pi = o.param[i];
+__device__ __forceinline__ float opt_update_loaded(const OptStep &o, size_t i, float g, float pi, float s1i, float s2i) {
     const float gi = g + o.wd * pi;
     float upd;
     if (o.kind == PTR_OPT_ADAM) {
-        const float mi = o.h1 * o.s1[i] + (1.0f - o.h1) * gi;
-        const float vi = o.h2 * o.s2[i] + (1.0f - o.h2) * gi * gi;
+        const float mi = o.h1 * s1i + (1.0f - o.h1) * gi;
+        const float vi = o.h2 * s2i + (1.0f - o.h2) * gi * gi;
         o.s1[i] = mi; o.s2[i] = vi;
         const float denom = sqrtf(vi) / o.bc2_sqrt + o.eps;
         upd = (o.lr / o.bc1) * (mi / denom);
     } else {
-        const float si = o.kind == PTR_OPT_ADAGRAD ? o.s1[i] + gi * gi : o.h1 * o.s1[i] + (1.0f - o.h1) * gi * gi;
+        const float si = o.kind == PTR_OPT_ADAGRAD ? s1i + gi * gi : o.h1 * s1i + (1.0f - o.h1) * gi * gi;
         o.s1[i] = si;
         upd = o.lr * (gi / (sqrtf(si) + o.eps));
     }
@@ -51,6 +51,9 @@
     o.param[i] = pn;
     return pn;
 }
+__device__ __forceinline__ float opt_update(const OptStep &o, size_t i, float g) {
+    return opt_update_loaded(o, i, g, o.param[i], o.s1[i], o.kind == PTR_OPT_ADAM ? o.s2[i] : 0.0f);
+}
 #endif
 
 }
diff --git a/ptranking_amd/csrc/scorer.hip b/ptranking_amd/csrc/scorer.hip
--- a/ptranking_amd/csrc/scorer.hip
+++ b/ptranking_amd/csrc/scorer.hip
@@ -864,11 +864,21 @@
 
 namespace ptr {
 int mlp_backward_impl(const char *who, const float *X, const float *params, const float *acts, const float *dpreds, int R, int F, int NL,
-                             float p_drop, uint64_t seed, float *dz, float *ws, float *grad, void *stream, const OptStep &opt);
+                             float p_drop, uint64_t seed, float *dz, float *ws, float *grad, void *stream, const OptStep &opt, const void *bimg);
 }
 extern "C" int ptr_mlp_backward(const float *X, const float *params, const float *acts, const float *dpreds, int R, int F, int NL,
                                 float p_drop, uint64_t seed, float *dz, float *ws, float *grad, void *stream) {
-    return ptr::mlp_backward_impl("ptr_mlp_backward", X, params, acts, dpreds, R, F, NL, p_drop, seed, dz, ws, grad, stream, ptr::OptStep{});
+    return ptr::mlp_backward_impl("ptr_mlp_backward", X, params, acts, dpreds, R, F, NL, p_drop, seed, dz, ws, grad, stream, ptr::OptStep{}, nullptr);
+}
+
+extern "C" int ptr_mlp_backward_x6_img(const float *X, const float *params, const float *acts, const float *dpreds, int R, int F, int NL,
+                                       float p_drop, uint64_t seed, float *dz, float *ws, float *grad, const void *bimg, void *stream) {
+    const char *who = "ptr_mlp_backward_x6_img";
+    if (bimg && (!ptr::bwd_x6_img_bytes(F, NL) || (reinterpret_cast<uintptr_t>(bimg) & 15))) {
+        ptr::set_error("%s: an image for F=%d NL=%d that the bf16x6 backward does not serve, or not 16-byte aligned", who, F, NL);
+        return PTR_ERR_INVALID_ARG;
+    }
+    return ptr::mlp_backward_impl(who, X, params, acts, dpreds, R, F, NL, p_drop, seed, dz, ws, grad, stream, ptr::OptStep{}, bimg);
 }
 
 extern "C" int ptr_mlp_backward_step(const float *X, float *params, const float *acts, const float *dpreds, int R, int F, int NL, float p_drop,
@@ -876,29 +886,30 @@
                                      float eps, float weight_decay, int step, float *state1, float *state2, const float *loss_q, int nq,
                                      float *loss_out, void *stream) {
     return ptr::mlp_backward_step_impl(X, params, acts, dpreds, R, F, NL, p_drop, seed, dz, ws, grad, opt_kind, lr, hyper1, hyper2, eps, weight_decay, step, state1,
-                                       state2, loss_q, nq, loss_out, nullptr, stream);
+                                       state2, loss_q, nq, loss_out, nullptr, nullptr, stream);
 }
 
 int ptr::mlp_backward_step_impl(const float *X, float *params, const float *acts, const float *dpreds, int R, int F, int NL, float p_drop, uint64_t seed,
                                 float *dz, float *ws, float *grad, int opt_kind, float lr, float hyper1, float hyper2, float eps, float weight_decay, int step,
-                                float *state1, float *state2, const float *loss_q, int nq, float *loss_out, void *wimg, void *stream) {
+                                float *state1, float *state2, const float *loss_q, int nq, float *loss_out, void *wimg, void *bimg, void *stream) {
     using namespace ptr;
     const char *who = "ptr_mlp_backward_step";
     OptStep o;
     if (int rc = make_opt_step(o, who, opt_kind, lr, hyper1, hyper2, eps, weight_decay, step, params, state1, state2, true, loss_q, nq, loss_out)) return rc;
     o.wimg = reinterpret_cast<uint8_t *>(wimg); o.F = F; o.NL = NL;
-    return mlp_backward_impl(who, X, params, acts, dpreds, R, F, NL, p_drop, seed, dz, ws, grad, stream, o);
+    o.bimg = reinterpret_cast<uint8_t *>(bimg);
+    return mlp_backward_impl(who, X, params, acts, dpreds, R, F, NL, p_drop, seed, dz, ws, grad, stream, o, bimg);
 }
 
 int ptr::mlp_backward_impl(const char *who, const float *X, const float *params, const float *acts, const float *dpreds, int R, int F, int NL,
-                                  float p_drop, uint64_t seed, float *dz, float *ws, float *grad, void *stream, const OptStep &opt) {
+                                  float p_drop, uint64_t seed, float *dz, float *ws, float *grad, void *stream, const OptStep &opt, const void *bimg) {
     using namespace ptr;
     if (int rc = check_mlp(who, R, F, NL, p_drop)) return rc;
     if (!X || !params || !acts || !dpreds || !ws || !grad) { set_error("%s: NULL pointer", who); return PTR_ERR_INVALID_ARG; }
     hipStream_t st = as_stream(stream);
     MlpArgs a{R, F, NL, p_drop, (uint32_t)seed, (uint32_t)(seed >> 32)};
     if (R > 0 && bwd_fused_supported(F, NL, X, acts)) {
-        if (int e = bwd_x6_supported(R, F, NL, X, acts) ? launch_bwd_x6(X, params, acts, dpreds, a, ws, st, who)
+        if (int e = bwd_x6_supported(R, F, NL, X, acts) ? launch_bwd_x6(X, params, acts, dpreds, a, ws, bimg, st, who)
                                                         : launch_bwd_fused(X, params, acts, dpreds, a, ws, st, who)) return e;
         const int nb = bwd_fused_grid(R);
         const size_t NPf = n_params(NL, F);
@@ -914,7 +925,7 @@
     if (grid_dz < 1) grid_dz = 1;
     const bool tail = R > 0 && bwd_tail_supported(NL, acts);
     if (tail) {
-        if (int e = bwd_x6_tail_supported(R, NL, acts) ? launch_bwd_x6_tail(params, acts, dpreds, a, ws, dz, st, who)
+        if (int e = bwd_x6_tail_supported(R, NL, acts) ? launch_bwd_x6_tail(params, acts, dpreds, a, ws, dz, bimg, st, who)
                                                        : launch_bwd_tail(params, acts, dpreds, a, ws, dz, st, who)) return e;
     } else {
         const size_t lds = dz_lds_floats(NL) * sizeof(float);
diff --git a/ptranking_amd/csrc/scorer_bwd_x6.hip b/ptranking_amd/csrc/scorer_bwd_x6.hip
--- a/ptranking_amd/csrc/scorer_bwd_x6.hip
+++ b/ptranking_amd/csrc/scorer_bwd_x6.hip
@@ -24,10 +24,54 @@
 }
 __device__ __forceinline__ uint32_t b6_opaque(uint32_t x) { asm volatile("" : "+s"(x)); return x; }
 
+__device__ __forceinline__ void b6_gather_wt(f32x4 *__restrict__ wt, const float *__restrict__ P, int F, int W, int j, int g) {
+#pragma unroll
+    for (int c = 0; c < 2; ++c) {
+        const float *Wl = P + off_W(2 - c, F);
+        const int ri = 16 * W + j;
+#pragma unroll
+        for (int s = 0; s < 3; ++s) {
+            float v[8];
+#pragma unroll
+            for (int e = 0; e < 8; ++e) {
+                const int k = 32 * s + 8 * g + e;
+                v[e] = ri < kH ? Wl[(size_t)k * kH + ri] : 0.0f;
+            }
+            Frag pl[3];
+#pragma unroll
+            for (int d = 0; d < 4; ++d) split_pack2(v[2 * d], v[2 * d + 1], pl[0].u[d], pl[1].u[d], pl[2].u[d]);
+#pragma unroll
+            for (int p = 0; p < 3; ++p) wt[3 * (3 * c + s) + p] = __builtin_bit_cast(f32x4, pl[p].q);
+        }
+        {
+            float v[4];
+#pragma unroll
+            for (int e = 0; e < 4; ++e) { const int k = 96 + 4 * g + e; v[e] = (ri < kH && k < kH) ? Wl[(size_t)k * kH + ri] : 0.0f; }
+            uint32_t t0[3], t1[3];
+            split_pack2(v[0], v[1], t0[0], t0[1], t0[2]);
+            split_pack2(v[2], v[3], t1[0], t1[1], t1[2]);
+#pragma unroll
+            for (int p = 0; p < 3; ++p) {
+                const int d = 2 * (3 * c + p);
+                wt[18 + d / 4][d % 4] = __uint_as_float(t0[p]);
+                wt[18 + d / 4][d % 4 + 1] = __uint_as_float(t1[p]);
+            }
+        }
+    }
+}
+
+__global__ void __launch_bounds__(448) b6_prep_kernel(const float *__restrict__ P, int F, uint8_t *__restrict__ img) {
+    const int lane = threadIdx.x & 63, W = threadIdx.x >> 6;
+    f32x4 wt[kB6ImgSlots];
+    b6_gather_wt(wt, P, F, W, lane & 15, lane >> 4);
+#pragma unroll
+    for (int s = 0; s < kB6ImgSlots; ++s) *reinterpret_cast<f32x4 *>(img + (size_t)((s * 7 + W) * 1024 + lane * 16)) = wt[s];
+}
+
 template <int NT1>
 __global__ void __launch_bounds__(512, 2)
 mlp_bwd_x6_kernel(const float *__restrict__ X, const float *__restrict__ P, const float *__restrict__ acts, const float *__restrict__ dpreds,
-                  MlpArgs a, float *__restrict__ ws, size_t np_stride, float *__restrict__ dz0) {
+                  MlpArgs a, float *__restrict__ ws, size_t np_stride, float *__restrict__ dz0, const uint8_t *__restrict__ bimg) {
     static_assert(NT1 == 9 || NT1 == 0, "the X image is laid out for nine in-feature tiles; NT1 = 0 is the TAIL form");
     constexpr bool TAIL = NT1 == 0;
     extern __shared__ __attribute__((aligned(16))) uint8_t smem_b6[];
@@ -53,38 +97,13 @@
 #pragma unroll
     for (int i = 0; i < 39; ++i) st[i] = f32x4{0.0f, 0.0f, 0.0f, 0.0f};
     if (chain) {
-#pragma unroll
-        for (int c = 0; c < 2; ++c) {
-            const float *Wl = P + off_W(2 - c, F);
-            const int ri = 16 * W + j;
-#pragma unroll
-            for (int s = 0; s < 3; ++s) {
-                float v[8];
-#pragma unroll
-                for (int e = 0; e < 8; ++e) {
-                    const int k = 32 * s + 8 * g + e;
-                    v[e] = ri < kH ? Wl[(size_t)k * kH + ri] : 0.0f;
-                }
-                Frag pl[3];
-#pragma unroll
-                for (int d = 0; d < 4; ++d) split_pack2(v[2 * d], v[2 * d + 1], pl[0].u[d], pl[1].u[d], pl[2].u[d]);
-#pragma unroll
-                for (int p = 0; p < 3; ++p) st[18 + 3 * (3 * c + s) + p] = __builtin_bit_cast(f32x4, pl[p].q);
-            }
-            {
-                float v[4];
-#pragma unroll
-                for (int e = 0; e < 4; ++e) { const int k = 96 + 4 * g + e; v[e] = (ri < kH && k < kH) ? Wl[(size_t)k * kH + ri] : 0.0f; }
-                uint32_t t0[3], t1[3];
-                split_pack2(v[0], v[1], t0[0], t0[1], t0[2]);
-                split_pack2(v[2], v[3], t1[0], t1[1], t1[2]);
-#pragma unroll
-                for (int p = 0; p < 3; ++p) {
-                    const int d = 2 * (3 * c + p);
-                    st[36 + d / 4][d % 4] = __uint_as_float(t0[p]);
-                    st[36 + d / 4][d % 4 + 1] = __uint_as_float(t1[p]);
-                }
-            }
+        if (bimg) {
+            const b6_rsrc isrd = __builtin_amdgcn_make_buffer_rsrc(const_cast<uint8_t *>(bimg), 0, kB6ImgBytes, 0x00020000);
+#pragma unroll
+            for (int s = 0; s < kB6ImgSlots; ++s)
+                st[18 + s] = __builtin_bit_cast(f32x4, __builtin_amdgcn_raw_buffer_load_b128(isrd, lane * 16, (s * 7 + W) * 1024, 0));
+        } else {
+            b6_gather_wt(&st[18], P, F, W, j, g);
         }
     }
     B6_EDGE();
@@ -162,23 +181,27 @@
     };
     uint32_t jk = (uint32_t)j * kDropRowMul + (uint32_t)g * kDropFgMul + a.seed_lo;
     asm volatile("" : "+v"(jk));
-    auto stage_x_tile = [&](int row0, int t_, const f32x4 (&x2)[2]) __attribute__((always_inline)) {
+    static_assert(TAIL || 16 * (NT1 - 1) == 128, "tiles 0..NT1 - 2 lie wholly below F only while F > 16 (NT1 - 1) = 128");
+    auto stage_x_tile = [&](auto edge_, int row0, int t_, const f32x4 (&x2)[2]) __attribute__((always_inline)) {
+        constexpr bool EDGE = decltype(edge_)::value;
         const int t = (int)b6_opaque((uint32_t)t_);
-        int col = 16 * t + 4 * g;
-        asm volatile("" : "+v"(col));
+        [[maybe_unused]] int col = 16 * t + 4 * g;
+        if constexpr (EDGE) asm volatile("" : "+v"(col));
 #pragma unroll
         for (int dt = 0; dt < 2; ++dt) {
             uint32_t w0, w1;
             drop_bits_key(jk + ((uint32_t)(row0 + 16 * dt) * kDropRowMul + (uint32_t)(4 * t) * kDropFgMul), a.seed_hi, w0, w1);
             f32x4 v = drop4(x2[dt], w0, w1, thr, scale);
-#pragma unroll
-            for (int r = 0; r < 4; ++r) v[r] = col + r < F ? v[r] : (col + r == F ? 1.0f : 0.0f);
+            if constexpr (EDGE) {
+#pragma unroll
+                for (int r = 0; r < 4; ++r) v[r] = col + r < F ? v[r] : (col + r == F ? 1.0f : 0.0f);
+            }
             split_write4(b6_opaque(lds0 + kB6_XI + (uint32_t)(32 * t)) + wr_x + (uint32_t)(16 * dt * kB6XRS), kB6XPL, v);
         }
     };
     auto stage_x = [&](int slab) __attribute__((always_inline)) {
-        if (chain) stage_x_tile(slab * kB6S, W, xr[0]);
-        else { stage_x_tile(slab * kB6S, 7, xr[0]); stage_x_tile(slab * kB6S, 8, xr[1]); }
+        if (chain) stage_x_tile(std::false_type{}, slab * kB6S, W, xr[0]);
+        else { stage_x_tile(std::false_type{}, slab * kB6S, 7, xr[0]); stage_x_tile(std::true_type{}, slab * kB6S, 8, xr[1]); }
     };
     auto prefetch = [&](int slab) __attribute__((always_inline)) {
         const int row0 = slab * kB6S;
@@ -432,13 +455,14 @@
     if ((uint64_t)NL * (uint64_t)act_layer_floats(R) * 4 >= 0xFFFFF000ull || (uint64_t)R * (uint64_t)F * 4 >= 0xFFFFF000ull) return false;
     return NL == 3 && NT1 == 9 && F % 4 == 0 && F < 16 * NT1 && (reinterpret_cast<uintptr_t>(X) & 15) == 0 && (reinterpret_cast<uintptr_t>(acts) & 15) == 0;
 }
-int launch_bwd_x6(const float *X, const float *params, const float *acts, const float *dpreds, const MlpArgs &a, float *ws, hipStream_t st,
-                  const char *who) {
+int launch_bwd_x6(const float *X, const float *params, const float *acts, const float *dpreds, const MlpArgs &a, float *ws, const void *bimg,
+                  hipStream_t st, const char *who) {
     const int grid = bwd_fused_grid(a.R);
     const size_t NP = n_params(a.NL, a.F);
     auto kern = mlp_bwd_x6_kernel<9>;
     if (int e = allow_lds(kern, kB6Lds)) return e;
-    hipLaunchKernelGGL(kern, dim3(grid), dim3(512), kB6Lds, st, X, params, acts, dpreds, a, ws, NP, (float *)nullptr);
+    hipLaunchKernelGGL(kern, dim3(grid), dim3(512), kB6Lds, st, X, params, acts, dpreds, a, ws, NP, (float *)nullptr,
+                       reinterpret_cast<const uint8_t *>(bimg));
     return check_hip(hipGetLastError(), who);
 }
 
@@ -447,14 +471,31 @@
     if ((uint64_t)NL * (uint64_t)act_layer_floats(R) * 4 >= 0xFFFFF000ull || (uint64_t)R * (kAL * 4) >= 0xFFFFF000ull) return false;
     return NL == 3 && (reinterpret_cast<uintptr_t>(acts) & 15) == 0;
 }
-int launch_bwd_x6_tail(const float *params, const float *acts, const float *dpreds, const MlpArgs &a, float *ws, float *dz0, hipStream_t st,
-                       const char *who) {
+int launch_bwd_x6_tail(const float *params, const float *acts, const float *dpreds, const MlpArgs &a, float *ws, float *dz0, const void *bimg,
+                       hipStream_t st, const char *who) {
     const int grid = bwd_fused_grid(a.R);
     const size_t NP = n_params(a.NL, a.F);
     auto kern = mlp_bwd_x6_kernel<0>;
     if (int e = allow_lds(kern, kB6Lds)) return e;
-    hipLaunchKernelGGL(kern, dim3(grid), dim3(512), kB6Lds, st, (const float *)nullptr, params, acts, dpreds, a, ws, NP, dz0);
+    hipLaunchKernelGGL(kern, dim3(grid), dim3(512), kB6Lds, st, (const float *)nullptr, params, acts, dpreds, a, ws, NP, dz0,
+                       reinterpret_cast<const uint8_t *>(bimg));
     return check_hip(hipGetLastError(), who);
 }
 
-}
+size_t bwd_x6_img_bytes(int F, int NL) { return (env_int("PTR_BWD_X6", 1) && NL == 3 && F > 0) ? (size_t)kB6ImgBytes : 0; }
+int launch_b6_prep(const float *params, int F, void *bimg, hipStream_t st, const char *who) {
+    hipLaunchKernelGGL(b6_prep_kernel, dim3(1), dim3(448), 0, st, params, F, reinterpret_cast<uint8_t *>(bimg));
+    return check_hip(hipGetLastError(), who);
+}
+
+}
+
+extern "C" size_t ptr_mlp_bwd_x6_img_bytes(int F, int NL) { return ptr::bwd_x6_img_bytes(F, NL); }
+
+extern "C" int ptr_mlp_bwd_x6_img_prep(const float *params, int F, int NL, void *bimg, void *stream) {
+    using namespace ptr;
+    const char *who = "ptr_mlp_bwd_x6_img_prep";
+    if (!bwd_x6_img_bytes(F, NL)) { set_error("%s: the bf16x6 backward does not serve F=%d NL=%d", who, F, NL); return PTR_ERR_UNSUPPORTED; }
+    if (!params || !bimg || (reinterpret_cast<uintptr_t>(bimg) & 15)) { set_error("%s: NULL or unaligned pointer", who); return PTR_ERR_INVALID_ARG; }
+    return launch_b6_prep(params, F, bimg, as_stream(stream), who);
+}
diff --git a/ptranking_amd/csrc/train_step.hip b/ptranking_amd/csrc/train_step.hip
--- a/ptranking_amd/csrc/train_step.hip
+++ b/ptranking_amd/csrc/train_step.hip
@@ -1,8 +1,7 @@
 #include "ptr_mlp.h"
 
-extern "C" int ptr_train_step(const ptr_train_step_desc *d, void *stream) {
+static int train_step_impl(const char *who, const ptr_train_step_desc *d, void *bimg, int bimg_current, void *stream) {
     using namespace ptr;
-    const char *who = "ptr_train_step";
     if (!d) { set_error("%s: NULL descriptor", who); return PTR_ERR_INVALID_ARG; }
     if (d->struct_bytes != (int32_t)sizeof(ptr_train_step_desc)) {
         set_error("%s: descriptor of %d bytes, this library expects %d (ABI v%d)", who, (int)d->struct_bytes, (int)sizeof(ptr_train_step_desc), PTR_ABI_VERSION);
@@ -11,6 +10,10 @@
     if (d->B < 0 || d->L <= 0 || (int64_t)d->B * d->L > 0x7fffffffll) { set_error("%s: bad shape B=%d L=%d", who, d->B, d->L); return PTR_ERR_INVALID_ARG; }
     if (d->loss_kind < PTR_LOSS_RANKNET || d->loss_kind > PTR_LOSS_LISTNET) { set_error("%s: unknown loss %d", who, d->loss_kind); return PTR_ERR_INVALID_ARG; }
     if (!d->loss_q || !d->dpreds || !d->preds) { set_error("%s: NULL scratch pointer", who); return PTR_ERR_INVALID_ARG; }
+    if (bimg && (!bwd_x6_img_bytes(d->F, d->NL) || (reinterpret_cast<uintptr_t>(bimg) & 15))) {
+        set_error("%s: bimg for F=%d NL=%d, which the bf16x6 backward does not serve (ptr_mlp_bwd_x6_img_bytes), or not 16-byte aligned", who, d->F, d->NL);
+        return PTR_ERR_INVALID_ARG;
+    }
     const int R = d->B * d->L;
     hipStream_t st = as_stream(stream);
     auto mark = [&](int k) -> int { return d->events[k] ? check_hip(hipEventRecord(reinterpret_cast<hipEvent_t>(d->events[k]), st), who) : 0; };
@@ -30,7 +33,14 @@
     }
     if (rc) return rc;
     if (int rc2 = mark(2)) return rc2;
+    if (bimg && !bimg_current && R > 0) { if (int rcp = launch_b6_prep(d->params, d->F, bimg, st, who)) return rcp; }
     if (int rc3 = mlp_backward_step_impl(d->X, d->params, d->acts, d->dpreds, R, d->F, d->NL, d->p_drop, d->seed, d->dz, d->ws, d->grad, d->opt_kind, d->lr, d->hyper1,
-                                         d->hyper2, d->eps, d->weight_decay, d->step, d->state1, d->state2, d->loss_q, d->B, d->loss_out, d->wimg, stream)) return rc3;
+                                         d->hyper2, d->eps, d->weight_decay, d->step, d->state1, d->state2, d->loss_q, d->B, d->loss_out, d->wimg, bimg, stream)) return rc3;
     return mark(3);
 }
+
+extern "C" int ptr_train_step(const ptr_train_step_desc *d, void *stream) { return train_step_impl("ptr_train_step", d, nullptr, 0, stream); }
+
+extern "C" int ptr_train_step_img(const ptr_train_step_desc *d, void *bimg, int bimg_current, void *stream) {
+    return train_step_impl("ptr_train_step_img", d, bimg, bimg_current, stream);
+}
diff --git a/ptranking_amd/rankers.py b/ptranking_amd/rankers.py
--- a/ptranking_amd/rankers.py
+++ b/ptranking_amd/rankers.py
@@ -85,7 +85,9 @@
             if len(cache) >= 4:
                 cache.pop(next(iter(cache)))
             ndz = _lib.query("ptr_mlp_backward_dz_floats", R, Fd, NL)
+            nbimg = _lib.query("ptr_mlp_bwd_x6_img_bytes", Fd, NL)
             buf = dict(preds=torch.empty((B, L), device=dev), acts=alloc_acts(R, NL, dev),
+                       bimg=torch.empty(nbimg, device=dev, dtype=torch.uint8) if nbimg else None, bimg_tag=None,
                        loss_q=torch.empty(max(B, 1), device=dev), dpreds=torch.empty((B, L), device=dev),
                        ws=torch.empty(_lib.query("ptr_mlp_backward_ws_floats", Fd, NL), device=dev),
                        dz=torch.empty(ndz, device=dev) if ndz else None)
@@ -156,6 +158,10 @@
         step_before = int(st_["step"]) if st_ else 0
         d.wimg_current = int(wimg is not None and self.reuse_weight_image and os.environ.get("PTR_REUSE_IMG", "1") != "0" and
                              x6_image_tag(dev, Fd, NL) == (flat.data_ptr(), flat._version, step_before, wimg.data_ptr()))
+        bimg = buf["bimg"]
+        bimg_current = int(bimg is not None and self.reuse_weight_image and os.environ.get("PTR_REUSE_IMG", "1") != "0" and
+                           buf["bimg_tag"] == (flat.data_ptr(), flat._version, step_before, bimg.data_ptr()))
+        buf["bimg_tag"], buf["bimg_current"] = None, bimg_current
         timing = _lib.TIMING
         evs = None
         if timing is not None:
@@ -179,7 +185,7 @@
             with torch.cuda.device(dev):
                 _lib.TIMING = None
                 try:
-                    _lib.call("ptr_train_step", C.addressof(d), _lib.current_stream(dev))
+                    _lib.call("ptr_train_step_img", C.addressof(d), _lib.ptr(bimg), bimg_current, _lib.current_stream(dev))
                 finally:
                     _lib.TIMING = timing
         except Exception:
@@ -187,6 +193,8 @@
             raise
         if wimg is not None:
             x6_set_image_tag(dev, Fd, NL, (flat.data_ptr(), flat._version, step, wimg.data_ptr()))
+        if bimg is not None:
+            buf["bimg_tag"] = (flat.data_ptr(), flat._version, step, bimg.data_ptr())
         if evs is not None:
             timing.setdefault("ptr_mlp_forward_x6" if wimg is not None else "ptr_mlp_forward", []).append((evs[0], evs[1]))
             timing.setdefault(spec.entry, []).append((evs[1], evs[2]))
```

New measurement: 5.549 million. No clear change (-0.1%).
